# XiaoshuiHuang/GMF

Measured on AMD Instinct MI355X. Metric: correspondences/sec (whole node), higher is better.
Workload: dtype f32 (split-fp16 MFMA operands, fp32 accumulate; the cross products of the attention's two contractions, S = K Q'^T and O = P V, on block-scaled e4m3 operands wherever the device-side score guard allows)

## Files before the change

gmf_amd/_lib.py:

```python
from __future__ import annotations

import collections
import ctypes as C
import os
import threading
from typing import Dict, Optional

_HERE = os.path.dirname(os.path.abspath(__file__))
LIB_PATH = os.path.join(_HERE, "libgmf_hip.so")

_f32p = C.POINTER(C.c_float)
_i32p = C.POINTER(C.c_int)
_vp = C.c_void_p
_ll = C.c_longlong


class EncoderWeights(C.Structure):
    _fields_ = [
        ("num_layers", C.c_int),
        ("f1_ctx_wst", _vp), ("f1_ctx_vec", _vp),
        ("f1_attn_wst", _vp), ("f1_attn_vec", _vp),
        ("f1_ff_wst", _vp), ("f1_ff_vec", _vp),
        ("ctx_wst", _vp), ("ctx_vec", _vp), ("ctx_wst_stride", C.c_int), ("ctx_vec_stride", C.c_int),
        ("attn_wst", _vp), ("attn_vec", _vp), ("attn_wst_stride", C.c_int), ("attn_vec_stride", C.c_int),
        ("ff_wst", _vp), ("ff_vec", _vp), ("ff_wst_stride", C.c_int), ("ff_vec_stride", C.c_int),
        ("front_wst", _vp), ("front_vec", _vp), ("front_wst_stride", C.c_int), ("front_vec_stride", C.c_int),
        ("tail_wst", _vp), ("tail_vec", _vp), ("tail_wst_stride", C.c_int), ("tail_vec_stride", C.c_int),
        ("head_wst", _vp), ("head_vec", _vp),
        ("sigma_d", C.c_float),
        ("front_wst_h2", _vp), ("ctx_wst_h2", _vp), ("attn_wst_h2", _vp), ("ff_wst_h2", _vp),
        ("f1_ctx_wst_h2", _vp), ("f1_attn_wst_h2", _vp), ("f1_ff_wst_h2", _vp),
        ("tail_wst_h2", _vp),
        ("pv_guard", _vp),
    ]


class Tensor(C.Structure):
    _fields_ = [("name", C.c_char_p), ("data", _vp), ("ndim", C.c_int), ("shape", _ll * 4)]


class FusionWeights(C.Structure):
    _fields_ = [("latent_dim", C.c_int), ("d_head", C.c_int), ("pe", C.c_int), ("split_fp16", C.c_int),
                ("max_abs_scaled", C.c_float),
                ("ctx_wst", _vp), ("ctx_vec", _vp), ("attn_wst", _vp), ("attn_vec", _vp), ("ff_wst", _vp), ("ff_vec", _vp),
                ("ctx_wst_h2", _vp), ("attn_wst_h2", _vp), ("ff_wst_h2", _vp)]


GMF_PACK_DEVICE_TENSORS = 1
GMF_PACK_STANDALONE_BLOCK = 2
GMF_PACK_HOST_BLOCK = 4


def tensor_list(sd):
    import torch
    keep, items = [], []
    host = {}
    dev = [(k, v) for k, v in sd.items() if torch.is_tensor(v) and v.is_floating_point() and v.device.type != "cpu" and v.dim() <= 4]
    if dev:
        flat = torch.cat([v.detach().reshape(-1).to(torch.float32) for _, v in dev]).cpu()
        o = 0
        for k, v in dev:
            host[k] = flat[o:o + v.numel()].reshape(v.shape)
            o += v.numel()
    for k, v in sd.items():
        if not (torch.is_tensor(v) and v.is_floating_point()):
            continue
        t = host[k] if k in host else v.detach().to("cpu", torch.float32).contiguous()
        if t.dim() > 4:
            continue
        name = k.encode()
        keep += [t, name]
        e = Tensor()
        e.name, e.data, e.ndim = name, t.data_ptr(), t.dim()
        for d in range(4):
            e.shape[d] = t.shape[d] if d < t.dim() else 1
        items.append(e)
    arr = (Tensor * len(items))(*items)
    return arr, keep


class PoseParams(C.Structure):
    _fields_ = [
        ("num_seeds", C.c_int), ("k", C.c_int), ("num_iterations", C.c_int), ("use_nms", C.c_int),
        ("refine_iters", C.c_int),
        ("sigma", C.c_float), ("sigma_d", C.c_float), ("inlier_threshold", C.c_float),
        ("nms_radius", C.c_float), ("refine_threshold", C.c_float),
    ]


class PoseGraphOptions(C.Structure):
    _fields_ = [("max_iteration", C.c_int), ("max_iteration_lm", C.c_int), ("reference_node", C.c_int),
                ("min_relative_increment", C.c_double), ("min_relative_residual_increment", C.c_double),
                ("min_right_term", C.c_double), ("min_residual", C.c_double),
                ("edge_prune_threshold", C.c_double), ("preference_loop_closure", C.c_double)]


SIGNATURES = {
    "gmf_abi_version": (C.c_int, []),
    "gmf_create": (C.c_int, [C.c_int, C.POINTER(_vp)]),
    "gmf_destroy": (None, [_vp]),
    "gmf_last_error_string": (C.c_char_p, [_vp]),
    "gmf_workspace_bytes": (_ll, [_vp]),
    "gmf_set_workspace": (C.c_int, [_vp, _vp, _ll]),
    "gmf_workspace_wanted": (_ll, [_vp]),
    "gmf_status_read": (C.c_int, [_vp, C.POINTER(C.c_int), C.c_int]),
    "gmf_set_tuning": (C.c_int, [_vp, C.c_char_p, C.c_int]),
    "gmf_get_tuning": (C.c_int, [_vp, C.c_char_p, C.POINTER(C.c_int)]),
    "gmf_set_sigma_device": (C.c_int, [_vp, _vp]),
    "gmf_profile_enable": (C.c_int, [_vp, C.c_int]),
    "gmf_profile_read": (C.c_int, [_vp, C.POINTER(C.c_double), C.POINTER(C.c_int)]),
    "gmf_pack_rows_p32": (C.c_int, [_vp, _vp, _ll, _ll, _ll, C.c_int, C.c_int, C.c_int, _vp, _vp]),
    "gmf_unpack_rows_p32": (C.c_int, [_vp, _vp, C.c_int, C.c_int, C.c_int, _vp, _ll, _ll, _ll, _vp]),
    "gmf_pack_pts8": (C.c_int, [_vp, _vp, _vp, C.c_int, C.c_int, _vp, _vp]),
    "gmf_front_forward": (C.c_int, [_vp, C.c_int, _vp, _vp, _vp, _vp, _vp, _vp, _vp, C.c_int, C.c_int, _vp]),
    "gmf_scattn_forward": (C.c_int, [_vp, _vp, _vp, _vp, _vp, _vp, _vp, _vp, _vp, C.c_int, C.c_int, C.c_float, _vp]),
    "gmf_scattn_forward_dense": (C.c_int, [_vp, _vp, _vp, _vp, _vp, _vp, _vp, _vp, _vp, C.c_int, C.c_int, _vp]),
# ... 294 lines not shown
```

gmf_amd/csrc/encoder_h2.hip:

```cpp
#include <algorithm>
#include <cstdlib>
#include "enc_common.hpp"
#include "enc_ff.hpp"
#include "launchers.hpp"

namespace gmf {

#ifndef GMF_H2_RING
#define GMF_H2_RING 2
#endif
constexpr int kRing = GMF_H2_RING;

template <int MODE>
GMF_DEVINL void front_h2_body(float* lds, const int bx, const int pair, const int zsel_in, const float* __restrict__ in,
                              const float* __restrict__ wst, const float* __restrict__ vecs, float* __restrict__ f_out,
                              float* __restrict__ q_out, float* __restrict__ k_out, float* __restrict__ v_out, int N, int tiles,
                              const PairTab* __restrict__ ptab = nullptr, unsigned* __restrict__ v_scale = nullptr,
                              const PvGuard guard = {}) {
  const int lane = threadIdx.x & 63, h = lane >> 5, i = lane & 31;
  const int wave = __builtin_amdgcn_readfirstlane(threadIdx.x >> 6);
  const size_t row0 = pair_row0(ptab, pair, N);
  N = pair_rows(ptab, pair, N);
  const int tiles_p = ptab ? (N + 31) >> 5 : tiles;
  if (bx * kWavesPerWG >= tiles_p) return;
// ... 512 lines not shown

__global__ void __launch_bounds__(256, 2)
k_small_front_fattn(const float* __restrict__ f_in, const float* __restrict__ front_wst, const float* __restrict__ front_vec,
                    const float* __restrict__ ctx_img, const float* __restrict__ attn_wst, const float* __restrict__ attn_vec,
                    float* __restrict__ q_out, float* __restrict__ k_out, float* __restrict__ v_out, float* __restrict__ x1_out,
                    int N, int tiles, int T, int ttiles, unsigned* __restrict__ v_scale, const PvGuard guard,
                    const PairTab* __restrict__ ptab) {
  __shared__ __attribute__((aligned(16))) float lds[kFattnTileLdsFloats];
  static_assert(kFattnTileLdsFloats >= kFattnLdsFloats, "one buffer serves both forms of the role");
  if (blockIdx.z < 3) {
    front_h2_body<2>(lds, blockIdx.x, blockIdx.y, blockIdx.z, f_in, front_wst, front_vec, nullptr, q_out, k_out, v_out, N, tiles,
                     ptab, v_scale, guard);
    return;
  }
  const int Np = pair_rows(ptab, blockIdx.y, N), tiles_p = ptab ? (Np + 31) >> 5 : tiles;
  if (gridDim.z == 4) {
    if ((int)blockIdx.x * kWavesPerWG >= tiles_p) return;
    fusion_attn_h2_body<true>(lds, blockIdx.x, blockIdx.y, f_in, ctx_img, attn_wst, attn_vec, x1_out, Np, tiles_p, T, ttiles, tiles);
  } else {
    const int tile = (int)blockIdx.x * kWavesPerWG + ((int)blockIdx.z - 3);
    if (tile < tiles_p) fusion_attn_tile_h2_body(lds, tile, blockIdx.y, f_in, ctx_img, attn_wst, attn_vec, x1_out, Np, tiles_p, T, ttiles, tiles);
  }
}

template <bool SPLIT>
__global__ void __launch_bounds__(256, 2)
k_fusion_ff_h2p(const float* __restrict__ x1, const float* __restrict__ wst, const float* __restrict__ vecs,
                float* __restrict__ x2_out, int tiles, float* __restrict__ part) {
  __shared__ __attribute__((aligned(16))) float lds[4 * kStageFloats];
  fusion_ff_h2p_body<SPLIT>(lds, blockIdx.x, blockIdx.y, gridDim.y, blockIdx.z, gridDim.z, x1, wst, vecs, x2_out, tiles, part);
}

__global__ void __launch_bounds__(256, 2)
k_pro_ctx_pts(const int n_a, const int gx_a, const int nb, const float* __restrict__ ctx, const float* __restrict__ wst,
              const float* __restrict__ vecs, float* __restrict__ out, int T, int ttiles,
              const float* __restrict__ src, const float* __restrict__ tgt, float* __restrict__ pts8, int N, int Npad, long total,
              const PairTab* __restrict__ ptab, unsigned* __restrict__ zero_words, int n_zero) {
  __shared__ __attribute__((aligned(16))) float lds[2 * kStageFloats];
  const int id = blockIdx.x;
  if (id < n_a) {
    ctx_prep_h2_body<false, true>(lds, id % gx_a, id / gx_a, 0, nb, ctx, wst, vecs, out, T, ttiles, 0, 0);
    return;
  }
  pack_pts8_body((long)(id - n_a) * 256 + threadIdx.x, src, tgt, pts8, N, Npad, total, ptab, zero_words, n_zero);
}

constexpr int kProBLdsFloats = kFattnLdsFloats > kCompatLdsFloats ? kFattnLdsFloats : kCompatLdsFloats;
__global__ void __launch_bounds__(256, 2)
k_pro_fattn_compat(const int n_a, const int gx_a, const float* __restrict__ xin, const float* __restrict__ ctx_img,
                   const float* __restrict__ wst, const float* __restrict__ vecs, float* __restrict__ x1_out, int T, int ttiles,
                   const float* __restrict__ pts8, float* __restrict__ c_dense, int N, int tiles, int gy, float inv_sig2,
                   const PairTab* __restrict__ ptab) {
  __shared__ __attribute__((aligned(16))) float lds[kProBLdsFloats];
  const int id = blockIdx.x;
  if (id < n_a) {
    fusion_attn_h2_body<false, true>(lds, id % gx_a, id / gx_a, xin, ctx_img, wst, vecs, x1_out, T, ttiles, T, ttiles);
    return;
  }
  const int j = id - n_a, I = j % tiles, rest = j / tiles;
  compat_build_body<0>(lds, I, rest % gy, rest / gy, pts8, c_dense, N, tiles, inv_sig2, ptab);
}

constexpr int kProCLdsFloats = (kRing > 4 ? kRing : 4) * kStageFloats;
template <bool SPLIT, int MINB>
__global__ void __launch_bounds__(256, MINB)
k_pro_ff_front(const int n_a, const int gx_a, const int nb, const int hs, const float* __restrict__ x1, const float* __restrict__ wst,
               const float* __restrict__ vecs, float* __restrict__ x2_out, int ttiles, float* __restrict__ part,
               const int gx_f, const float* __restrict__ in, const float* __restrict__ fwst, const float* __restrict__ fvecs,
               float* __restrict__ f_out, float* __restrict__ q_out, float* __restrict__ k_out, float* __restrict__ v_out, int N,
               int tiles, const PairTab* __restrict__ ptab, const PvGuard guard) {
  __shared__ __attribute__((aligned(16))) float lds[kProCLdsFloats];
  const int id = blockIdx.x;
  if (id < n_a) {
    const int bx = id % gx_a, r = id / gx_a;
    fusion_ff_h2p_body<SPLIT>(lds, bx, r % nb, nb, r / nb, hs, x1, wst, vecs, x2_out, ttiles, part);
    return;
  }
  const int j = id - n_a;
  front_h2_body<3>(lds, j % gx_f, j / gx_f, -1, in, fwst, fvecs, f_out, q_out, k_out, v_out, N, tiles, ptab, nullptr, guard);
}

constexpr int kLinLdsFloats = 4 * kStageFloats + 7 * C + (3 * C + 2 * FFH) + kWavesPerWG * 2 * C + 3 * C;

template <int PART, int NP = 3, bool QSKIP = false>
GMF_DEVINL void linear_h2_body(float* lds, const float* __restrict__ f_in, const float* __restrict__ front_wst,
                               const float* __restrict__ front_vec, const float* __restrict__ ctx_img,
                               const float* __restrict__ attn_wst, const float* __restrict__ attn_vec,
                               const float* __restrict__ ff_wst, const float* __restrict__ ff_vec, float* __restrict__ q_out,
                               float* __restrict__ k_out, float* __restrict__ v_out, float* __restrict__ x2_out, int N, int tiles,
                               int T, int ttiles, const PairTab* __restrict__ ptab = nullptr,
                               unsigned* __restrict__ v_scale = nullptr,
                               const PvGuard guard = {}) {
  const int lane = threadIdx.x & 63, h = lane >> 5, i = lane & 31;
  const int wave = __builtin_amdgcn_readfirstlane(threadIdx.x >> 6);
  const int pair = blockIdx.y;
  if (ptab) N = ptab[pair].n;
  const int tiles_p = ptab ? (N + 31) >> 5 : tiles;
  if ((int)blockIdx.x * kWavesPerWG >= tiles_p) return;
  const int tile_raw = blockIdx.x * kWavesPerWG + wave;
  const bool active = tile_raw < tiles_p;
  const int tile = active ? tile_raw : tiles_p - 1;
  const float* pair_base = f_in + (size_t)pair * tiles * (32 * C);
  const size_t toff = ((size_t)pair * tiles + tile) * (32 * C);

  float* const lvec_a = lds + 4 * kStageFloats;
  float* const lvec_f = lvec_a + 7 * C;
  float* const halo = lvec_f + (3 * C + 2 * FFH) + wave * (2 * C);
  float* const lvec_p = lvec_f + (3 * C + 2 * FFH) + kWavesPerWG * (2 * C);
  if (PART != 2) dma_vec(front_vec + C, lvec_p, 3 * C, wave, kWavesPerWG, lane);
  if (PART != 1) {
    dma_vec(attn_vec, lvec_a, 7 * C, wave, kWavesPerWG, lane);
    dma_vec(ff_vec, lvec_f, 3 * C + 2 * FFH, wave, kWavesPerWG, lane);
    LcpeHalo<CF>::issue(pair_base, tile, tiles_p, halo, lane);
  }
  StageRing<4> ss;
  if (PART == 0) ss.init(lds, wave, lane, front_wst + (QSKIP ? 8 : 4) * kStageFloats, QSKIP ? 8 : 12, attn_wst, 2,
                         ctx_img + (size_t)pair * ttiles * kStageFloats, ttiles, attn_wst + 2 * kStageFloats, 2);
  else if (PART == 1) ss.init(lds, wave, lane, front_wst + 4 * kStageFloats, 12);
  else ss.init(lds, wave, lane, attn_wst, 2, ctx_img + (size_t)pair * ttiles * kStageFloats, ttiles, attn_wst + 2 * kStageFloats, 2);

  float f[CF];
  if (PART != 2) {
    FragH2<8> fx;
    load_frag_p32<CF>(f, f_in + toff, lane);
    fx.set(f);
    ss.prime();
    const bool v8 = pv_planes_on(v_scale, guard, pair);
    unsigned* const sw_tile = v_scale ? v_scale + ((size_t)pair * tiles + tile) * 128 + lane : nullptr;
    unsigned ksw = 0;
#pragma unroll
    for (int which = (QSKIP ? 1 : 0); which < 2; ++which) {
      float* dst = (which == 0 ? q_out : k_out) + toff;
#pragma unroll
      for (int mb = 0; mb < 4; ++mb) {
        constexpr int kYounger[4] = {8, 12, 16, 20};
        const int sidx = 4 * (which - (QSKIP ? 1 : 0)) + mb;
        const f16x8* lw = as_h2(PART == 1 ? ss.acquire()
                                : sidx == 0 ? ss.acquire_counted<kYounger[0]>() : sidx == 1 ? ss.acquire_counted<kYounger[1]>()
                                : sidx == 2 ? ss.acquire_counted<kYounger[2]>() : ss.acquire_counted<kYounger[3]>());
        f32x16 acc = zero16();
        mma_wx_h2n<8, NP>(acc, lw, fx);
        float t[16], bb[16];
        load_vec_block(bb, lvec_p + which * C, mb, h);
#pragma unroll
        for (int r = 0; r < 16; ++r) t[r] = fmaf(acc[r], kH2Inv, bb[r]);
        if (which == 1 && v8) store_block_v8(dst, mb, t, lane, ksw);
        else store_block_h2(dst, mb, t, lane);
      }
    }
    unsigned vsw = 0;
#pragma unroll
    for (int db = 0; db < 4; ++db) {
      const f16x8* lw = as_h2(PART == 1 ? ss.acquire() : ss.acquire_counted<20>());
      f32x16 acc = zero16();
      mma_xw_h2n<8, NP>(acc, lw, fx);
      float t[16];
      const float bvd = lvec_p[2 * C + 32 * db + i];
#pragma unroll
      for (int r = 0; r < 16; ++r) t[r] = fmaf(acc[r], kH2Inv, bvd);
      if (v8) store_block_v8(v_out + toff, db, t, lane, vsw);
      else store_block_h2(v_out + toff, db, t, lane);
    }
    if (v_scale) { sw_tile[0] = vsw; sw_tile[64] = ksw; }
  }

  if (PART == 1) {
    asm volatile("s_waitcnt vmcnt(0)" ::: "memory");
    return;
  }
  if (PART == 2) ss.prime();
  f32x16 x1a[4];
  {
    FragH2<4> qx;
    {
      float xp[CF];
      if (PART == 2) load_frag_p32<CF>(xp, f_in + toff, lane);
      else {
#pragma unroll
        for (int k = 0; k < CF; ++k) xp[k] = f[k];
      }
      if (PART == 2) {
        asm volatile("s_waitcnt vmcnt(0)" ::: "memory");
        __syncthreads();
      }
      LcpeHalo<CF>::apply(xp, halo, lvec_a, tile * 32 + i, N, lane);
      {
        FragH2<8> nx;
        {
          float xn[CF];
          layernorm_frag<CF>(xn, xp, lvec_a + 4 * C, lvec_a + 5 * C, h);
          nx.set(xn);
        }
#pragma unroll
        for (int mb = 0; mb < 2; ++mb) {
          const f16x8* lw = as_h2(ss.acquire());
          f32x16 acc = zero16();
          mma_wx_h2n<8, NP>(acc, lw, nx);
          float t[16];
#pragma unroll
          for (int r = 0; r < 16; ++r) t[r] = acc[r] * kH2Inv;
          qx.set_block(mb, t);
        }
      }
#pragma unroll
      for (int mb = 0; mb < 4; ++mb) {
        float b[16];
        load_vec_block(b, lvec_a + 6 * C, mb, h);
#pragma unroll
        for (int r = 0; r < 16; ++r) x1a[mb][r] = (xp[16 * mb + r] + b[r]) * 256.0f;
      }
    }
    f32x16 oacc[2];
    oacc[0] = zero16(); oacc[1] = zero16();
    float m_run = -INFINITY, l_half = 0.f;
    for (int t = 0; t < ttiles; ++t) {
      const f16x8* lk = as_h2(ss.acquire());
      const f16x8* lv = lk + 2 * 4 * 64;
      f32x16 sc = zero16();
      mma_wx_h2n<4, NP>(sc, lk, qx);
      float x[16];
      float mx = -INFINITY;
      if (t + 1 < ttiles) {
#pragma unroll
        for (int r = 0; r < 16; ++r) { x[r] = sc[r]; mx = fmaxf(mx, sc[r]); }
      } else {
        const int jbase = t * 32 + 4 * h;
#pragma unroll
        for (int r = 0; r < 16; ++r) {
          const int jl = 8 * (r >> 2) + (r & 3);
          x[r] = (jbase + jl < T) ? sc[r] : -INFINITY;
          mx = fmaxf(mx, x[r]);
        }
      }
      mx = xhalf_max(mx);
      const float m_new = fmaxf(m_run, mx);
      const bool moved = m_new > m_run;
      const float alpha = __builtin_amdgcn_exp2f(m_run - m_new);
      m_run = m_new;
      const float m_off = m_new - 10.0f;
      float ls = 0.f;
#pragma unroll
      for (int r = 0; r < 16; ++r) { x[r] = __builtin_amdgcn_exp2f(x[r] - m_off); ls += x[r]; }
      l_half = fmaf(l_half, alpha, ls);
      if (__any(moved)) {
#pragma unroll
        for (int db = 0; db < 2; ++db)
#pragma unroll
          for (int r = 0; r < 16; ++r) oacc[db][r] *= alpha;
      }
#pragma unroll
      for (int s2 = 0; s2 < 2; ++s2) {
        f16x8 ph, pl;
        split8h(&x[8 * s2], ph, pl);
#pragma unroll
        for (int db = 0; db < 2; ++db) {
          const int slot = 2 * db + s2;
          mma_np<NP>(oacc[db], lv[(0 * 4 + slot) * 64], lv[(1 * 4 + slot) * 64], ph, pl);
        }
      }
    }
    FragH2<4> ox;
    {
      const float inv = 1.0f / xhalf_sum(l_half);
#pragma unroll
      for (int db = 0; db < 2; ++db) {
        float t[16];
#pragma unroll
        for (int r = 0; r < 16; ++r) t[r] = oacc[db][r] * inv;
        ox.set_block(db, t);
      }
    }
#pragma unroll
    for (int st = 0; st < 2; ++st) {
      const f16x8* lw = as_h2(ss.acquire());
#pragma unroll
      for (int hb = 0; hb < 2; ++hb) mma_wx_h2n<4, NP>(x1a[2 * st + hb], lw + hb * (2 * 4 * 64), ox);
    }
  }

  FragH2<8> nx;
  f32x16 y[4];
  {
    float x1[CF], xn[CF];
#pragma unroll
    for (int mb = 0; mb < 4; ++mb)
#pragma unroll
      for (int r = 0; r < 16; ++r) x1[16 * mb + r] = x1a[mb][r] * kH2Inv;
    layernorm_frag<CF>(xn, x1, lvec_f, lvec_f + C, h);
    nx.set(xn);
#pragma unroll
    for (int mb = 0; mb < 4; ++mb) {
      float b[16];
      load_vec_block(b, lvec_f + 2 * C + 2 * FFH, mb, h);
#pragma unroll
      for (int r = 0; r < 16; ++r) y[mb][r] = (x1[16 * mb + r] + b[r]) * 256.0f;
    }
  }
  __syncthreads();
  ff_chunks<NP>(nx, y, lds, ff_wst, lvec_f + 2 * C, lvec_f + 2 * C + FFH, wave, lane, h, 0, FFH / 32);
#pragma unroll
  for (int mb = 0; mb < 4; ++mb) {
    float t[16];
#pragma unroll
    for (int r = 0; r < 16; ++r) t[r] = y[mb][r] * kH2Inv;
    if (active) store_block_p32(x2_out + toff, mb, t, lane);
  }
}

template <int NP, bool QSKIP = false>
__global__ void __launch_bounds__(256, 2)
k_linear_h2(const float* __restrict__ f_in, const float* __restrict__ front_wst, const float* __restrict__ front_vec,
            const float* __restrict__ ctx_img, const float* __restrict__ attn_wst, const float* __restrict__ attn_vec,
            const float* __restrict__ ff_wst, const float* __restrict__ ff_vec, float* __restrict__ q_out,
            float* __restrict__ k_out, float* __restrict__ v_out, float* __restrict__ x2_out, int N, int tiles, int T,
            int ttiles, const PairTab* __restrict__ ptab, unsigned* __restrict__ v_scale, const PvGuard guard) {
  __shared__ __attribute__((aligned(16))) float lds[kLinLdsFloats];
  tail_priority(blockIdx.y * gridDim.x + blockIdx.x, gridDim.x * gridDim.y);
  linear_h2_body<0, NP, QSKIP>(lds, f_in, front_wst, front_vec, ctx_img, attn_wst, attn_vec, ff_wst, ff_vec, q_out, k_out, v_out, x2_out, N,
                               tiles, T, ttiles, ptab, v_scale, guard);
}

__global__ void __launch_bounds__(256, 2)
k_linear_roles(const float* __restrict__ f_in, const float* __restrict__ front_wst, const float* __restrict__ front_vec,
               const float* __restrict__ ctx_img, const float* __restrict__ attn_wst, const float* __restrict__ attn_vec,
               const float* __restrict__ ff_wst, const float* __restrict__ ff_vec, float* __restrict__ q_out,
               float* __restrict__ k_out, float* __restrict__ v_out, float* __restrict__ x2_out, int N, int tiles, int T,
               int ttiles, unsigned* __restrict__ v_scale, const PvGuard guard, const PairTab* __restrict__ ptab) {
  __shared__ __attribute__((aligned(16))) float lds[kLinLdsFloats];
  if (blockIdx.z == 0)
    linear_h2_body<1>(lds, f_in, front_wst, front_vec, ctx_img, attn_wst, attn_vec, ff_wst, ff_vec, q_out, k_out, v_out, x2_out, N,
                      tiles, T, ttiles, ptab, v_scale, guard);
  else
    linear_h2_body<2>(lds, f_in, front_wst, front_vec, ctx_img, attn_wst, attn_vec, ff_wst, ff_vec, q_out, k_out, v_out, x2_out, N,
                      tiles, T, ttiles, ptab);
}

__global__ void __launch_bounds__(256)
k_ff_reduce(const float* __restrict__ part, const float* __restrict__ x1, const float* __restrict__ vecs,
            float* __restrict__ x2_out, int tiles, int hs) {
  const int lane = threadIdx.x & 63, h = lane >> 5;
  const int tile = blockIdx.x * kWavesPerWG + (threadIdx.x >> 6);
  if (tile >= tiles) return;
  const int mb = blockIdx.z;
  const size_t n_all = (size_t)gridDim.y * tiles;
  const size_t toff = ((size_t)blockIdx.y * tiles + tile) * (32 * C);
  float b[16], xr[16], p[8][16];
  load_vec_block(b, vecs + 2 * C + 2 * FFH, mb, h);
#pragma unroll
  for (int z = 0; z < 8; ++z)
    if (z < hs) load_block_p32(p[z], part + (size_t)z * n_all * (32 * C) + toff, mb, lane);
  load_block_p32(xr, x1 + toff, mb, lane);
  float t[16];
#pragma unroll
  for (int r = 0; r < 16; ++r) t[r] = p[0][r];
#pragma unroll
  for (int z = 1; z < 8; ++z)
    if (z < hs) {
#pragma unroll
      for (int r = 0; r < 16; ++r) t[r] += p[z][r];
    }
#pragma unroll
  for (int r = 0; r < 16; ++r) t[r] = fmaf(t[r], kH2Inv, b[r]) + xr[r];
  store_block_p32(x2_out + toff, mb, t, lane);
}

static inline dim3 tgrid(int tiles, int B, int sets = 1) { return dim3((tiles + kWavesPerWG - 1) / kWavesPerWG, B, sets); }

hipError_t launch_front_h2(int mode, bool split, const float* in, const float* wst, const float* vecs, float* f, float* q, float* k,
                           float* v, int B, int N, int tiles, hipStream_t s, const PairTab* ptab, unsigned* v_scale, PvGuard guard) {
  dim3 g = tgrid(tiles, B);
  if (split) g.z = 3;
  if (mode == 3) { g.z = 1; hipLaunchKernelGGL(k_front_h2<3>, g, dim3(256), 0, s, in, wst, vecs, f, q, k, v, N, tiles, ptab, v_scale, guard); }
  else if (mode == 1) hipLaunchKernelGGL(k_front_h2<1>, g, dim3(256), 0, s, in, wst, vecs, f, q, k, v, N, tiles, ptab, v_scale, guard);
  else if (mode == 2) hipLaunchKernelGGL(k_front_h2<2>, g, dim3(256), 0, s, in, wst, vecs, f, q, k, v, N, tiles, ptab, v_scale, guard);
  else hipLaunchKernelGGL(k_front_h2<0>, g, dim3(256), 0, s, in, wst, vecs, f, q, k, v, N, tiles, ptab, v_scale, guard);
  return hipGetLastError();
}

hipError_t launch_linear_h2(bool roles, const float* f, const float* front_wst, const float* front_vec, const float* ctx_img,
                            const float* attn_wst, const float* attn_vec, const float* ff_wst, const float* ff_vec, float* q,
                            float* k, float* v, float* x2, int B, int N, int tiles, int T, int ttiles, hipStream_t s,
                            bool one_product, const PairTab* ptab, unsigned* v_scale, PvGuard guard) {
  if (roles)
    hipLaunchKernelGGL(k_linear_roles, tgrid(tiles, B, 2), dim3(256), 0, s, f, front_wst, front_vec, ctx_img, attn_wst, attn_vec,
                       ff_wst, ff_vec, q, k, v, x2, N, tiles, T, ttiles, v_scale, guard, ptab);
  else if (one_product)
    hipLaunchKernelGGL(k_linear_h2<1>, tgrid(tiles, B), dim3(256), 0, s, f, front_wst, front_vec, ctx_img, attn_wst, attn_vec, ff_wst,
                       ff_vec, q, k, v, x2, N, tiles, T, ttiles, ptab, v_scale, guard);
  else if (!q)
    hipLaunchKernelGGL((k_linear_h2<3, true>), tgrid(tiles, B), dim3(256), 0, s, f, front_wst, front_vec, ctx_img, attn_wst, attn_vec, ff_wst,
                       ff_vec, q, k, v, x2, N, tiles, T, ttiles, ptab, v_scale, guard);
  else
    hipLaunchKernelGGL(k_linear_h2<3>, tgrid(tiles, B), dim3(256), 0, s, f, front_wst, front_vec, ctx_img, attn_wst, attn_vec, ff_wst,
                       ff_vec, q, k, v, x2, N, tiles, T, ttiles, ptab, v_scale, guard);
  return hipGetLastError();
}

hipError_t launch_ctx_prep_h2(bool pe, const float* ctx, const float* wst, const float* vecs, float* out, int B, int T,
                              int ttiles, int sets, int wst_stride, int vec_stride, hipStream_t s, bool rowmajor) {
  if (pe) hipLaunchKernelGGL(k_ctx_prep_h2<true>, tgrid(ttiles, B, sets), dim3(256), 0, s, ctx, wst, vecs, out, T, ttiles, wst_stride, vec_stride);
  else if (rowmajor) hipLaunchKernelGGL((k_ctx_prep_h2<false, true>), tgrid(ttiles, B, sets), dim3(256), 0, s, ctx, wst, vecs, out, T, ttiles, wst_stride, vec_stride);
  else hipLaunchKernelGGL(k_ctx_prep_h2<false>, tgrid(ttiles, B, sets), dim3(256), 0, s, ctx, wst, vecs, out, T, ttiles, wst_stride, vec_stride);
  return hipGetLastError();
}

hipError_t launch_fusion_attn_h2(bool pe, const float* x, const float* ctx_img, const float* wst, const float* vecs,
                                 float* x1, int B, int N, int tiles, int T, int ttiles, hipStream_t s, bool rowmajor) {
  if (pe) hipLaunchKernelGGL(k_fusion_attn_h2<true>, tgrid(tiles, B), dim3(256), 0, s, x, ctx_img, wst, vecs, x1, N, tiles, T, ttiles);
  else if (rowmajor) hipLaunchKernelGGL((k_fusion_attn_h2<false, true>), tgrid(tiles, B), dim3(256), 0, s, x, ctx_img, wst, vecs, x1, N, tiles, T, ttiles);
  else hipLaunchKernelGGL(k_fusion_attn_h2<false>, tgrid(tiles, B), dim3(256), 0, s, x, ctx_img, wst, vecs, x1, N, tiles, T, ttiles);
  return hipGetLastError();
}

hipError_t launch_pro_ctx_pts(const float* p_tokens, const float* wst, const float* vecs, float* f1ctx, int B, int T, int ttiles,
                              const float* src, const float* tgt, float* pts8, int N, hipStream_t s, const PairTab* ptab,
                              unsigned* zero_words, int n_zero) {
  const dim3 ga = tgrid(ttiles, B);
  const int Npad = ((N + 31) / 32) * 32;
  const long total = (long)B * Npad;
  const int n_a = (int)(ga.x * ga.y), n_b = (int)((std::max(total, (long)n_zero) + 255) / 256);
  hipLaunchKernelGGL(k_pro_ctx_pts, dim3(n_a + n_b), dim3(256), 0, s, n_a, (int)ga.x, B, p_tokens, wst, vecs, f1ctx, T, ttiles, src, tgt,
                     pts8, N, Npad, total, ptab, zero_words, n_zero);
  return hipGetLastError();
}

hipError_t launch_pro_fattn_compat(const float* q_tokens, const float* f1ctx, const float* wst, const float* vecs, float* x1t, int B,
                                   int T, int ttiles, const float* pts8, float* c_dense, int N, int tiles, float sigma_d,
                                   hipStream_t s, const PairTab* ptab) {
  const dim3 ga = tgrid(ttiles, B);
  const int gy = (tiles + 4 * kJPerWave - 1) / (4 * kJPerWave);
  const int n_a = (int)(ga.x * ga.y);
  const long n_b = (long)tiles * gy * B;
  hipLaunchKernelGGL(k_pro_fattn_compat, dim3((unsigned)(n_a + n_b)), dim3(256), 0, s, n_a, (int)ga.x, q_tokens, f1ctx, wst, vecs, x1t, T,
                     ttiles, pts8, c_dense, N, tiles, gy, 1.0f / (sigma_d * sigma_d), ptab);
  return hipGetLastError();
}

hipError_t launch_pro_ff_front(const float* x1t, const float* wst, const float* vecs, float* imgfeat, int B, int ttiles, float* part,
                               int hs, const float* corr_pos, const float* fwst, const float* fvecs, float* f, float* q, float* k,
                               float* v, int N, int tiles, hipStream_t s, const PairTab* ptab, PvGuard guard) {
  const dim3 ga = tgrid(ttiles, B), gf = tgrid(tiles, B);
  const int n_a = (int)(ga.x * B) * hs, n_b = (int)(gf.x * B);
#define GMF_PRO_C(SPLIT, MINB, HS, PART)                                                                                              \
  hipLaunchKernelGGL((k_pro_ff_front<SPLIT, MINB>), dim3(n_a + n_b), dim3(256), 0, s, n_a, (int)ga.x, B, HS, x1t, wst, vecs, imgfeat, ttiles, \
                     PART, (int)gf.x, corr_pos, fwst, fvecs, f, q, k, v, N, tiles, ptab, guard)
  const bool one_per_cu = n_a + n_b <= 256;
  if (hs > 1) { if (one_per_cu) GMF_PRO_C(true, 1, hs, part); else GMF_PRO_C(true, 2, hs, part); }
  else { if (one_per_cu) GMF_PRO_C(false, 1, 1, (float*)nullptr); else GMF_PRO_C(false, 2, 1, (float*)nullptr); }
#undef GMF_PRO_C
  return hipGetLastError();
}

hipError_t launch_ff_reduce_h2(const float* part, const float* x1, const float* vecs, float* x2, int B, int tiles, int hs, hipStream_t s) {
  const dim3 g = tgrid(tiles, B);
  hipLaunchKernelGGL(k_ff_reduce, dim3(g.x, g.y, 4), dim3(256), 0, s, part, x1, vecs, x2, tiles, hs);
  return hipGetLastError();
}

hipError_t launch_small_front_fattn(const float* f, const float* front_wst, const float* front_vec, const float* ctx_img,
                                    const float* attn_wst, const float* attn_vec, float* q, float* k, float* v, float* x1, int B,
                                    int N, int tiles, int T, int ttiles, hipStream_t s, unsigned* v_scale, PvGuard guard, bool tile_role,
                                    const PairTab* ptab) {
  const bool per_tile = tile_role && ttiles >= 2 && (long)tiles * B <= 256;
  hipLaunchKernelGGL(k_small_front_fattn, tgrid(tiles, B, per_tile ? 7 : 4), dim3(256), 0, s, f, front_wst, front_vec, ctx_img, attn_wst, attn_vec,
                     q, k, v, x1, N, tiles, T, ttiles, v_scale, guard, ptab);
  return hipGetLastError();
}

hipError_t launch_fusion_ff_h2(const float* x1, const float* wst, const float* vecs, float* x2, int B, int tiles, hipStream_t s,
                               float* part, int hs) {
  const dim3 g = tgrid(tiles, B);
  if (hs > 1) {
    hipLaunchKernelGGL(k_fusion_ff_h2p<true>, dim3(g.x, g.y, hs), dim3(256), 0, s, x1, wst, vecs, x2, tiles, part);
    hipLaunchKernelGGL(k_ff_reduce, dim3(g.x, g.y, 4), dim3(256), 0, s, part, x1, vecs, x2, tiles, hs);
  }
  else hipLaunchKernelGGL(k_fusion_ff_h2p<false>, g, dim3(256), 0, s, x1, wst, vecs, x2, tiles, (float*)nullptr);
  return hipGetLastError();
// ... 4 lines not shown
```

gmf_amd/csrc/encoder_kernels.hip:

```cpp
#include <algorithm>
#include <type_traits>
#include "enc_common.hpp"
#include "enc_ff.hpp"

namespace gmf {

template <int MODE>
__global__ void __launch_bounds__(256, 2)
k_front(const float* __restrict__ in, const float* __restrict__ wst, const float* __restrict__ vecs,
        float* __restrict__ f_out, float* __restrict__ q_out, float* __restrict__ k_out,
        float* __restrict__ v_out, int N, int tiles) {
  __shared__ __attribute__((aligned(16))) float lds[2 * kStageFloats];
  const int lane = threadIdx.x & 63, wave = threadIdx.x >> 6, h = lane >> 5, i = lane & 31;
  const int pair = blockIdx.y;
  const int tile_raw = blockIdx.x * kWavesPerWG + wave;
  const bool active = tile_raw < tiles;
  const int tile = active ? tile_raw : tiles - 1;
  const size_t toff = ((size_t)pair * tiles + tile) * (32 * C);

  constexpr bool FIRST = (MODE == 1);
  StageStream ss;
  if (MODE == 2) ss.init(lds, lds + kStageFloats, wave, kWavesPerWG, lane, wst + 4 * kStageFloats, 12);
  else ss.init(lds, lds + kStageFloats, wave, kWavesPerWG, lane, wst, 16);
  ss.prime();
// ... 456 lines not shown

template <bool NEXT_PCN, class Stages, class Fus>
GMF_DEVINL void scattn_epilogue_h2(const float (&o)[CF], const bool active, Stages& ss, const float* __restrict__ vecs,
                                   const Fus& fus_tile, float* __restrict__ out_tile, const int lane, const int h,
                                   const float* __restrict__ next_bias = nullptr,
                                   unsigned* __restrict__ stat_next = nullptr, const int pair = 0, const bool row_valid = false) {
    FragH2<8> ox, featx;
    FragH2<4> m1x, m2x;
    if (active) ox.set(o);
#pragma unroll
    for (int mb = 0; mb < 2; ++mb) {
      const f16x8* lw = as_h2(ss.acquire());
      if (!active) continue;
      f32x16 acc = zero16();
      mma_wx_h2<8>(acc, lw, ox);
      float b[16], t1[16];
      load_vec_block(b, vecs, mb, h);
#pragma unroll
      for (int r = 0; r < 16; ++r) t1[r] = relu_nan(fmaf(acc[r], kH2Inv, b[r]));
      m1x.set_block(mb, t1);
    }
    {
      const f16x8* lw = as_h2(ss.acquire());
#pragma unroll
      for (int mb = 0; mb < 2; ++mb) {
        if (!active) continue;
        f32x16 acc = zero16();
        mma_wx_h2<4>(acc, lw + mb * (2 * 4 * 64), m1x);
        float b[16], t2[16];
        load_vec_block(b, vecs + 64, mb, h);
#pragma unroll
        for (int r = 0; r < 16; ++r) t2[r] = relu_nan(fmaf(acc[r], kH2Inv, b[r]));
        m2x.set_block(mb, t2);
      }
    }
#pragma unroll
    for (int st = 0; st < 2; ++st) {
      const f16x8* lw = as_h2(ss.acquire());
#pragma unroll
      for (int hb = 0; hb < 2; ++hb) {
        if (!active) continue;
        const int mb = 2 * st + hb;
        f32x16 acc = zero16();
        mma_wx_h2<4>(acc, lw + hb * (2 * 4 * 64), m2x);
        float b[16], fz[16], tt[16];
        load_vec_block(b, vecs + 128, mb, h);
        fus_tile.load(fz, mb, lane, h);
#pragma unroll
        for (int r = 0; r < 16; ++r) tt[r] = fmaf(acc[r], kH2Inv, b[r]) + fz[r];
        if (NEXT_PCN) featx.set_block(mb, tt);
        else if (active) store_block_p32(out_tile, mb, tt, lane);
      }
    }
    if (NEXT_PCN) {
      float ssq = 0.f;
#pragma unroll
      for (int mb = 0; mb < 4; ++mb) {
        const f16x8* lw = as_h2(ss.acquire());
        if (!active) continue;
        f32x16 acc = zero16();
        mma_wx_h2<8>(acc, lw, featx);
        float b[16], tt[16];
        load_vec_block(b, next_bias, mb, h);
#pragma unroll
        for (int r = 0; r < 16; ++r) { tt[r] = relu_nan(fmaf(acc[r], kH2Inv, b[r])); ssq = fmaf(tt[r], tt[r], ssq); }
        store_block_p32(out_tile, mb, tt, lane);
      }
      if (stat_next && active) pv_stat_raise(stat_next, pair, ssq, row_valid, lane);
    }
}

struct AttnItem { int item, ks; bool split, valid; };
GMF_DEVINL AttnItem attn_item(int L, int n_items, int n_full, int ksplits) {
  const int chunk = n_items >> 3, rem = n_items & 7, xcd = L & 7, kth = L >> 3;
  const int start = (xcd < rem) ? xcd * (chunk + 1) : rem * (chunk + 1) + (xcd - rem) * chunk;
  const int items = chunk + (xcd < rem ? 1 : 0);
  const int nf = min(n_full, items);
  if (kth < nf) return AttnItem{start + kth, 0, false, true};
  const int j = kth - nf, r = j / ksplits;
  return AttnItem{start + nf + r, j - r * ksplits, true, nf + r < items};
}

constexpr float kInvU16 = 1.0f / 65535.0f;
template <int NPROD = 3, int CFMT = 0, int WAVES = 4, bool PVF8 = false>
GMF_DEVINL void scattn_h2p_body(float* lds, const int bid, const float* __restrict__ q_img, const float* __restrict__ k_img,
                                const float* __restrict__ v_img, const float* __restrict__ fus, const float* __restrict__ wst,
                                const float* __restrict__ vecs, float* out, int N, int tiles, int wgs_per_pair,
                                const float* __restrict__ c_dense, int n_items, int n_full, int ksplits,
                                float* __restrict__ part_o, float* __restrict__ part_ml, const float* __restrict__ next_wst,
                                const float* __restrict__ next_bias, const PairTab* __restrict__ ptab = nullptr,
                                const unsigned* __restrict__ v_scale = nullptr,
                                const float* qf_img = nullptr, const float* __restrict__ qw_wst = nullptr,
                                const float* __restrict__ qw_bias = nullptr,
                                unsigned* __restrict__ stat_next = nullptr) {
  static_assert(!PVF8 || NPROD == 3, "the fp8 cross products belong to the three-product form");
  float* const ldsK = lds;
  float* const ldsV = lds + 2 * kStageFloats;
  const int lane = threadIdx.x & 63, h = lane >> 5;
  const int wave = __builtin_amdgcn_readfirstlane(threadIdx.x >> 6);
  const unsigned lane_off16 = lane * 16;
  const AttnItem it = attn_item(bid, n_items, n_full, ksplits);
  if (!it.valid) return;
  const bool split = it.split;
  const int ks = it.ks;
  const int slot = it.item / wgs_per_pair, qblock = it.item - slot * wgs_per_pair;
  const int pair = ptab ? ptab[slot].ord : slot;
  if (ptab) N = ptab[pair].n;
  const int tiles_p = ptab ? (N + 31) >> 5 : tiles;
  if (qblock * WAVES >= tiles_p) return;
  const int t_begin = split ? (tiles_p * ks) / ksplits : 0;
  const int t_end = split ? (tiles_p * (ks + 1)) / ksplits : tiles_p;
  const int tile_raw = qblock * WAVES + wave;
  const bool active = tile_raw < tiles_p;
  const int tile = active ? tile_raw : tiles_p - 1;
  const size_t pbase = (size_t)pair * tiles;
  const size_t toff = (pbase + tile) * (32 * C);

  f16x8 qh[8], ql[8];
  if (NPROD == 3 && WAVES == 4 && qf_img) {
    FragH2<8> fx;
    {
      float fq[CF];
      load_frag_p32<CF>(fq, qf_img + toff, lane);
      fx.set(fq);
    }
#pragma unroll
    for (int st = 0; st < 4; ++st) dma_4k_s(qw_wst + st * kStageFloats + wave * 1024, lds + st * kStageFloats + wave * 1024, lane_off16);
    asm volatile("s_waitcnt vmcnt(0)" ::: "memory");
    __syncthreads();
#pragma unroll
    for (int mb = 0; mb < 4; ++mb) {
      const f16x8* lw = reinterpret_cast<const f16x8*>(lds + mb * kStageFloats) + lane;
      f32x16 acc = zero16();
      mma_wx_h2n<8, 3>(acc, lw, fx);
      float t[16], bq[16];
      load_vec_block(bq, qw_bias, mb, h);
#pragma unroll
      for (int r = 0; r < 16; ++r) t[r] = fmaf(acc[r], kH2Inv, bq[r]);
      split8h(&t[0], qh[2 * mb], ql[2 * mb]);
      split8h(&t[8], qh[2 * mb + 1], ql[2 * mb + 1]);
    }
    __syncthreads();
  } else {
    const f16x8* qp = reinterpret_cast<const f16x8*>(q_img + (pbase + tile) * (size_t)kStageFloats) + lane;
#pragma unroll
    for (int s = 0; s < 8; ++s) {
      qh[s] = qp[(0 * 8 + s) * 64];
      if (NPROD == 3) ql[s] = qp[(1 * 8 + s) * 64];
    }
  }
  i32x8 qb[4];
  unsigned qsw = 0;
  if (PVF8) {
#pragma unroll
    for (int cb = 0; cb < 4; ++cb) q_planes8(qh[2 * cb], ql[2 * cb], qh[2 * cb + 1], ql[2 * cb + 1], cb, lane, qb[cb], qsw);
  }
  constexpr int kCTile16 = CFMT ? 128 : 256;
  const f32x4* const crow = reinterpret_cast<const f32x4*>(c_dense) + ((pbase + tile) * (size_t)tiles) * kCTile16 + lane;
  float c[16];
  unsigned cw[8];
  const unsigned* const vsrow = PVF8 ? v_scale + pbase * 128 + lane : nullptr;
  unsigned vsw_next = 0, vsw = 0, ksw_next = 0, ksw = 0;
  const int psc = (lane & 32) ? 117 : 129;
  auto fetch_c = [&](int t) {
    const f32x4* ct = crow + (size_t)t * kCTile16;
    if (PVF8) {
      vsw_next = __builtin_nontemporal_load(vsrow + (size_t)t * 128);
      ksw_next = __builtin_nontemporal_load(vsrow + (size_t)min(t + 1, tiles_p - 1) * 128 + 64);
    }
    if (CFMT == 1) {
#pragma unroll
      for (int q2 = 0; q2 < 2; ++q2) {
        const f16x8 hv = __builtin_bit_cast(f16x8, __builtin_nontemporal_load(ct + q2 * 64));
#pragma unroll
        for (int e = 0; e < 8; ++e) c[8 * q2 + e] = (float)hv[e];
      }
    } else if (CFMT >= 2) {
#pragma unroll
      for (int q2 = 0; q2 < 2; ++q2) {
        const f32x4 v = __builtin_nontemporal_load(ct + q2 * 64);
#pragma unroll
        for (int e = 0; e < 4; ++e) cw[4 * q2 + e] = __float_as_uint(v[e]);
      }
    } else {
#pragma unroll
      for (int q = 0; q < 4; ++q) {
        const f32x4 v = __builtin_nontemporal_load(ct + q * 64);
        c[4 * q + 0] = v[0]; c[4 * q + 1] = v[1]; c[4 * q + 2] = v[2]; c[4 * q + 3] = v[3];
      }
    }
  };
  auto score = [&](int r, float sv) -> float {
    if (CFMT == 2) return (float)((r & 1) ? (cw[r >> 1] >> 16) : (cw[r >> 1] & 0xffffu)) * sv;
    return c[r] * sv;
  };
  auto expo = [&](float xv, float m_off) -> float {
    return __builtin_amdgcn_exp2f(CFMT == 2 ? fmaf(xv, kInvU16, -m_off) : xv - m_off);
  };
  auto mma_n = [&](f32x16& acc, f16x8 ah, f16x8 al, f16x8 bh, f16x8 bl) {
    if (NPROD == 3) mma3(acc, ah, al, bh, bl);
    else acc = mfma_h16(ah, bh, acc);
  };
  auto to_planes2 = [&](float x0, float x1, f16x8& hi, f16x8& lo, int j) {
    if (NPROD == 3) split2h(x0, x1, hi, lo, j);
    else { const f32x2 xx = {x0, x1}; const f16x2 hh = __builtin_convertvector(xx, f16x2); hi[j] = hh[0]; hi[j + 1] = hh[1]; }
  };
  auto planes_f8 = [&](const f16x8& hi, const f16x8& lo, const int j, const int kp, i32x8& pb, float& ls_h, float& ls_l) {
    const f16x2 hh = {hi[j], hi[j + 1]}, ll = {lo[j], lo[j + 1]};
    const f16x2 ones = {(_Float16)1.0f, (_Float16)1.0f};
    const int w = kp >> 1;
    if (kp & 1) {
      pb[w] = cvt2_fp8_f16<true>(pb[w], hh, 4.0f);
      pb[4 + w] = cvt2_fp8_f16<true>(pb[4 + w], ll, 0x1p-10f);
      ls_l = __builtin_amdgcn_fdot2(dec2_fp8_f16<true>(pb[4 + w], 0x1p-10f), ones, ls_l, false);
    } else {
      int d0, d1;
      asm("" : "=v"(d0), "=v"(d1));
      pb[w] = cvt2_fp8_f16<false>(d0, hh, 4.0f);
      pb[4 + w] = cvt2_fp8_f16<false>(d1, ll, 0x1p-10f);
      ls_l = __builtin_amdgcn_fdot2(dec2_fp8_f16<false>(pb[4 + w], 0x1p-10f), ones, ls_l, false);
    }
    ls_h = __builtin_amdgcn_fdot2(hh, ones, ls_h, false);
    asm volatile("" : "+v"(ls_h), "+v"(ls_l));
  };
  const float* gk = k_img + pbase * (size_t)kStageFloats;
  const float* gv = v_img + pbase * (size_t)kStageFloats;
  constexpr int kPiecesPerWave = ((NPROD == 3) ? 16 : 8) / WAVES;
  auto issue16k = [&](const float* g, float* l) {
#pragma unroll
    for (int q = 0; q < kPiecesPerWave; ++q) dma_piece_1k_s(g + (wave + WAVES * q) * 256, l + (wave + WAVES * q) * 256, lane_off16);
  };
  auto issueK = [&](int t) { issue16k(gk + (size_t)t * kStageFloats, ldsK + (t & 1) * kStageFloats); };
  auto issueV = [&](int t) { issue16k(gv + (size_t)t * kStageFloats, ldsV + (t & 1) * kStageFloats); };

  f32x16 oacc[4];
#pragma unroll
  for (int db = 0; db < 4; ++db) oacc[db] = zero16();
  float m_run = -INFINITY, l_half = 0.f;

  issueK(t_begin);
  if (t_begin + 1 < t_end) issueK(t_begin + 1);
  issueV(t_begin);
  fetch_c(t_begin);
  asm volatile("s_waitcnt vmcnt(0)" ::: "memory");
  __syncthreads();
  f32x16 s_a = zero16(), s_b;
  auto s_cross8 = [&](f32x16 acc, const f16x8* lkt, const int cb, const unsigned kscale) -> f32x16 {
    const i32x4* l8 = reinterpret_cast<const i32x4*>(lkt);
    const i32x4 a_lo = l8[(1 * 8 + 2 * cb) * 64], a_hi = l8[(1 * 8 + 2 * cb + 1) * 64];
    const i32x8 ka = {a_lo[0], a_lo[1], a_lo[2], a_lo[3], a_hi[0], a_hi[1], a_hi[2], a_hi[3]};
    return mfma_f8s2(ka, qb[cb], acc, cb, (int)kscale, (int)qsw);
  };
  if (active) {
    const f16x8* lk = reinterpret_cast<const f16x8*>(ldsK + (t_begin & 1) * kStageFloats) + lane;
    if (PVF8) {
      const unsigned ks0 = vsrow[(size_t)t_begin * 128 + 64];
#pragma unroll
      for (int s = 0; s < 8; ++s) s_a = mfma_h16(lk[(0 * 8 + s) * 64], qh[s], s_a);
#pragma unroll
      for (int cb = 0; cb < 4; ++cb) s_a = s_cross8(s_a, lk, cb, ks0);
    } else {
#pragma unroll
      for (int s = 0; s < 8; ++s) mma_n(s_a, lk[(0 * 8 + s) * 64], lk[(1 * 8 + s) * 64], qh[s], ql[s]);
    }
  }

  auto tile_top = [&](const int t, const f32x16& s_cur, float (&x)[16], float& mx) {
    asm volatile("s_waitcnt vmcnt(0)" ::: "memory");
    __syncthreads();
    if (PVF8) vsw = vsw_next;
#pragma unroll
    for (int r = 0; r < 16; r += 2) {
      x[r] = score(r, s_cur[r]);
      x[r + 1] = score(r + 1, s_cur[r + 1]);
      mx = __builtin_fmaxf(mx, __builtin_fmaxf(x[r], x[r + 1]));
    }
    __builtin_amdgcn_sched_barrier(0);
    if (t + 1 < t_end) fetch_c(t + 1);
    __builtin_amdgcn_sched_barrier(0);
  };
  auto issue_piece = [&](const int t, const int q) {
    if ((q & 3) >= kPiecesPerWave) return;
    if (q < 4) {
      if (t + 2 < t_end) dma_piece_1k_s(gk + (size_t)(t + 2) * kStageFloats + (wave + WAVES * q) * 256,
                                        ldsK + (t & 1) * kStageFloats + (wave + WAVES * q) * 256, lane_off16);
    } else {
      dma_piece_1k_s(gv + (size_t)(t + 1) * kStageFloats + (wave + WAVES * (q - 4)) * 256,
                     ldsV + ((t + 1) & 1) * kStageFloats + (wave + WAVES * (q - 4)) * 256, lane_off16);
    }
  };
  auto issue_k4 = [&](const int t) {
    if (WAVES == 4 && t + 2 < t_end && (NPROD == 3 || wave < 2))
      dma_4k_s(gk + (size_t)(t + 2) * kStageFloats + wave * 1024, ldsK + (t & 1) * kStageFloats + wave * 1024, lane_off16);
  };
  auto issue_v4 = [&](const int t) {
    if (WAVES == 4 && (NPROD == 3 || wave < 2))
      dma_4k_s(gv + (size_t)(t + 1) * kStageFloats + wave * 1024, ldsV + ((t + 1) & 1) * kStageFloats + wave * 1024, lane_off16);
  };
  auto rescale = [&](const bool moved, const float alpha) {
    if (__any(moved)) {
#pragma unroll
      for (int db = 0; db < 4; ++db)
#pragma unroll
        for (int r = 0; r < 16; ++r) oacc[db][r] *= alpha;
    }
  };
  auto tile_step = [&](const int t, const f32x16& s_cur, f32x16& s_next) {
    float x[16];
    float mx = -INFINITY, m_off = 0.f, alpha = 1.f, ls = 0.f;
    tile_top(t, s_cur, x, mx);
    const f16x8* lv = reinterpret_cast<const f16x8*>(ldsV + (t & 1) * kStageFloats) + lane;
    const f16x8* lk = reinterpret_cast<const f16x8*>(ldsK + ((t + 1) & 1) * kStageFloats) + lane;
    bool moved = false;
    f16x8 ph0, pl0, ph1, pl1;
    {
      mx = xhalf_max_swap(mx);
      if (CFMT == 2) mx *= kInvU16;
      const float m_new = __builtin_fmaxf(m_run, mx);
      moved = m_new > m_run;
      alpha = __builtin_amdgcn_exp2f(m_run - m_new);
      m_run = m_new;
      m_off = m_new - 10.0f;
      rescale(moved, alpha);
    }
    s_next = zero16();
    {
      f16x8 kh = lk[0], kl = kh;
      if (NPROD == 3) kl = lk[8 * 64];
      f16x8 kh_n = kh, kl_n = kl;
#pragma unroll
      for (int u = 0; u < 24; ++u) {
        const int s = u / 3, pr = u % 3;
        if (pr == 0 && s < 7) { kh_n = lk[(0 * 8 + s + 1) * 64]; if (NPROD == 3) kl_n = lk[(1 * 8 + s + 1) * 64]; }
        if (NPROD == 3 || pr == 2) s_next = mma3_part(pr, s_next, kh, kl, qh[s], ql[s]);
        if (pr == 2) { kh = kh_n; kl = kl_n; }
        if (u < 2) {
        } else if (u <= 11) {
          const int r = u - 2;
          x[r] = expo(x[r], m_off);
          ls += x[r];
        } else if (u <= 15) {
          const int j = 2 * (u - 12);
          to_planes2(x[j], x[j + 1], ph0, pl0, j);
        } else if (u <= 21) {
          const int r = u - 6;
          x[r] = expo(x[r], m_off);
          ls += x[r];
        } else {
          const int j = 2 * (u - 22);
          to_planes2(x[8 + j], x[8 + j + 1], ph1, pl1, j);
        }
        __builtin_amdgcn_sched_barrier(0);
      }
    }
    {
      f16x8 vh = lv[0], vl = vh;
      if (NPROD == 3) vl = lv[8 * 64];
      f16x8 vh_n = vh, vl_n = vl;
#pragma unroll
      for (int u = 0; u < 24; ++u) {
        const int s2 = u / 12, db = (u % 12) / 3, pr = u % 3;
        if (pr == 0 && u < 21) {
          const int un = u + 3, slot = 2 * ((un % 12) / 3) + un / 12;
          vh_n = lv[(0 * 8 + slot) * 64]; if (NPROD == 3) vl_n = lv[(1 * 8 + slot) * 64];
        }
        if (NPROD == 3 || pr == 2) oacc[db] = mma3_part(pr, oacc[db], vh, vl, s2 ? ph1 : ph0, s2 ? pl1 : pl0);
        if (pr == 2) { vh = vh_n; vl = vl_n; }
        if (u < 2) {
          const int j = 4 + 2 * u;
          to_planes2(x[8 + j], x[8 + j + 1], ph1, pl1, j);
        }
        if (u >= 3 && u < 11) issue_piece(t, u - 3);
        __builtin_amdgcn_sched_barrier(0);
      }
    }
    l_half = fmaf(l_half, alpha, ls);
  };
  constexpr float kLazy = 5.0f;
  auto tile_step_f8 = [&](const int t, const f32x16& s_cur, f32x16& s_next) {
    float x[16];
    float mx = -INFINITY, m_off = 0.f, alpha = 1.f, ls = 0.f, ls_l = 0.f;
    asm volatile("s_waitcnt vmcnt(0)" ::: "memory");
    __syncthreads();
    vsw = vsw_next;
    ksw = ksw_next;
    const f16x8* lv = reinterpret_cast<const f16x8*>(ldsV + (t & 1) * kStageFloats) + lane;
    const f16x8* lk = reinterpret_cast<const f16x8*>(ldsK + ((t + 1) & 1) * kStageFloats) + lane;
    f16x8 ph0, pl0, ph1, pl1;
    i32x8 pb;
    f16x8 vr[3];
    auto hslot = [](int u) { return (0 * 8 + 2 * (u & 3) + (u >> 2)) * 64; };
    s_next = zero16();
    {
      const i32x4* lk8 = reinterpret_cast<const i32x4*>(lk);
      f16x8 kh = lk[0];
      f16x8 kh_n = kh;
      i32x4 k8a = lk8[(1 * 8) * 64], k8b = lk8[(1 * 8 + 1) * 64];
#pragma unroll
      for (int u = 0; u < 24; ++u) {
        const int s = u / 3, pr = u % 3;
        if (pr == 0 && s < 7) kh_n = lk[(0 * 8 + s + 1) * 64];
        if (pr == 2) s_next = mfma_h16(kh, qh[s], s_next);
        if (pr == 0 && (s & 1)) {
          const int cb = s >> 1;
          const i32x8 ka = {k8a[0], k8a[1], k8a[2], k8a[3], k8b[0], k8b[1], k8b[2], k8b[3]};
          s_next = mfma_f8s2(ka, qb[cb], s_next, cb, (int)ksw, (int)qsw);
          if (cb < 3) { k8a = lk8[(1 * 8 + 2 * cb + 2) * 64]; k8b = lk8[(1 * 8 + 2 * cb + 3) * 64]; }
        }
        if (pr == 2) kh = kh_n;
        if (u < 4) {
#pragma unroll
          for (int r = 4 * u; r < 4 * u + 4; r += 2) {
            x[r] = score(r, s_cur[r]);
            x[r + 1] = score(r + 1, s_cur[r + 1]);
            mx = __builtin_fmaxf(mx, __builtin_fmaxf(x[r], x[r + 1]));
          }
        }
        if (u == 3) {
          __builtin_amdgcn_sched_barrier(0);
          if (t + 1 < t_end) fetch_c(t + 1);
          __builtin_amdgcn_sched_barrier(0);
          mx = xhalf_max_swap(mx);
          if (CFMT == 2) mx *= kInvU16;
          const bool moved = mx > m_run + kLazy;
          const float m_new = moved ? mx : m_run;
          alpha = __builtin_amdgcn_exp2f(m_run - m_new);
          m_run = m_new;
          m_off = m_new - (10.0f - kLazy);
          rescale(moved, alpha);
        }
        if (u >= 4 && u < 20) x[u - 4] = expo(x[u - 4], m_off);
        if (u >= 6 && u <= 18 && (u & 1) == 0) {
          const int k = (u - 6) >> 1;
          if (k < 4) split2h(x[2 * k], x[2 * k + 1], ph0, pl0, 2 * k);
          else split2h(x[2 * k], x[2 * k + 1], ph1, pl1, 2 * k - 8);
        }
        if (u == 20) split2h(x[14], x[15], ph1, pl1, 6);
        if (u == 16) issue_k4(t);
        if (u == 23) issue_v4(t);
        if (u >= 21) vr[u - 21] = lv[hslot(u - 21)];
        __builtin_amdgcn_sched_barrier(0);
      }
    }
    {
      const i32x4* lv8 = reinterpret_cast<const i32x4*>(lv);
      i32x4 fa[2][2];
#pragma unroll
      for (int u = 0; u < 12; ++u) {
        if (u < 8) {
          const int s2 = u >> 2, db = u & 3;
          oacc[db] = mfma_h16(vr[u % 3], s2 ? ph1 : ph0, oacc[db]);
          if (u + 3 < 8) vr[u % 3] = lv[hslot(u + 3)];
          if (u == 4 || u == 6) { const int fd = (u - 4) >> 1; fa[fd][0] = lv8[(1 * 8 + 2 * fd) * 64]; fa[fd][1] = lv8[(1 * 8 + 2 * fd + 1) * 64]; }
          planes_f8(u < 4 ? ph0 : ph1, u < 4 ? pl0 : pl1, 2 * (u & 3), u, pb, ls, ls_l);
        } else {
          const int db = u - 8;
          const i32x4 a_lo = fa[db & 1][0], a_hi = fa[db & 1][1];
          const i32x8 va = {a_lo[0], a_lo[1], a_lo[2], a_lo[3], a_hi[0], a_hi[1], a_hi[2], a_hi[3]};
          oacc[db] = mfma_f8s(va, pb, oacc[db], db, (int)vsw, psc);
          if (db < 2) { fa[db & 1][0] = lv8[(1 * 8 + 2 * db + 4) * 64]; fa[db & 1][1] = lv8[(1 * 8 + 2 * db + 5) * 64]; }
        }
        __builtin_amdgcn_sched_barrier(0);
      }
    }
    l_half = fmaf(l_half, alpha, ls + ls_l);
  };
  auto tile_last = [&](const int t, const f32x16& s_cur) {
    float x[16];
    float mx = -INFINITY, ls = 0.f;
    tile_top(t, s_cur, x, mx);
    const f16x8* lv = reinterpret_cast<const f16x8*>(ldsV + (t & 1) * kStageFloats) + lane;
    const int jbase = t * 32 + 4 * h;
    mx = -INFINITY;
#pragma unroll
    for (int r = 0; r < 16; ++r) {
// ... 39 lines not shown
#pragma unroll
      for (int db = 0; db < 4; ++db) {
        const int slot = 2 * db + s2;
        mma_n(oacc[db], lv[(0 * 8 + slot) * 64], lv[(1 * 8 + slot) * 64], ph, pl);
      }
    }
    }
    l_half = fmaf(l_half, alpha, ls);
  };
  if (!active) {
    for (int t = t_begin; t < t_end; ++t) {
      asm volatile("s_waitcnt vmcnt(0)" ::: "memory");
      __syncthreads();
      if (t + 1 < t_end) {
        if (PVF8) { issue_k4(t); issue_v4(t); }
        else {
#pragma unroll
          for (int q = 0; q < 8; ++q) issue_piece(t, q);
        }
      }
    }
  } else {
    int t = t_begin;
    if (PVF8) {
      for (; t + 2 < t_end; t += 2) {
        tile_step_f8(t, s_a, s_b);
        tile_step_f8(t + 1, s_b, s_a);
      }
      if (t + 1 < t_end) { tile_step_f8(t, s_a, s_b); tile_last(t + 1, s_b); }
      else tile_last(t, s_a);
    } else {
    for (; t + 2 < t_end; t += 2) {
      tile_step(t, s_a, s_b);
      tile_step(t + 1, s_b, s_a);
    }
    if (t + 1 < t_end) { tile_step(t, s_a, s_b); tile_last(t + 1, s_b); }
    else tile_last(t, s_a);
    }
  }
  if (split) {
    if (active) {
      float of[CF];
#pragma unroll
      for (int db = 0; db < 4; ++db)
#pragma unroll
        for (int r = 0; r < 16; ++r) of[16 * db + r] = oacc[db][r];
      const size_t n_tiles_all = (size_t)(n_items / wgs_per_pair) * tiles;
      const size_t pt = (size_t)ks * n_tiles_all + pbase + tile;
      store_frag_p32<CF>(part_o + pt * (32 * C), of, lane);
      const float lsum = xhalf_sum(l_half);
      if (h == 0) { part_ml[(pt * 32 + (lane & 31)) * 2] = m_run; part_ml[(pt * 32 + (lane & 31)) * 2 + 1] = lsum; }
    }
    return;
  }

  float o[CF];
  {
    const float inv = 1.0f / xhalf_sum(l_half);
#pragma unroll
    for (int db = 0; db < 4; ++db)
#pragma unroll
      for (int r = 0; r < 16; ++r) o[16 * db + r] = oacc[db][r] * inv;
  }
  __syncthreads();
  float* const lvec = lds + 2 * kStageFloats;
  stage_tail_vecs(lvec, vecs, next_wst ? next_bias : nullptr, wave, lane);
  StageStream ss;
  ss.init(lds, lds + kStageFloats, wave, WAVES, lane, wst, 5, next_wst, next_wst ? 4 : 0);
  ss.prime();
  const FusTile ft{fus + toff};
  if (next_wst) scattn_epilogue_h2<true>(o, active, ss, lvec, ft, out + toff, lane, h, lvec + 2 * C, stat_next, pair,
                                         tile_raw * 32 + (lane & 31) < N);
  else scattn_epilogue_h2<false>(o, active, ss, lvec, ft, out + toff, lane, h);
}

GMF_DEVINL bool attn_pv_on(const unsigned* __restrict__ v_scale, const PvGuard& guard, int bid, int n_items, int n_full, int ksplits,
                           int wgs_per_pair, const PairTab* __restrict__ ptab = nullptr) {
  if (!guard.stat) return v_scale != nullptr;
  const AttnItem it = attn_item(bid, n_items, n_full, ksplits);
  const int slot = it.valid ? it.item / wgs_per_pair : 0;
  return pv_planes_on(v_scale, guard, ptab ? ptab[slot].ord : slot);
}

template <int NPROD, int CFMT, bool PVF8 = false>
__global__ void __launch_bounds__(256, 2)
k_scattn_h2p(const float* __restrict__ q_img, const float* __restrict__ k_img, const float* __restrict__ v_img,
             const float* __restrict__ fus, const float* __restrict__ wst, const float* __restrict__ vecs,
             float* out, int N, int tiles, int wgs_per_pair, const float* __restrict__ c_dense,
             int n_items, int n_full, int ksplits, float* __restrict__ part_o, float* __restrict__ part_ml,
             const float* __restrict__ next_wst, const float* __restrict__ next_bias, const PairTab* __restrict__ ptab,
             const unsigned* __restrict__ v_scale, const float* qf_img, const float* __restrict__ qw_wst,
             const float* __restrict__ qw_bias, const PvGuard guard) {
  __shared__ __attribute__((aligned(16))) float lds[4 * kStageFloats];
  tail_priority(blockIdx.x, gridDim.x);
  if (!PVF8 || attn_pv_on(v_scale, guard, blockIdx.x, n_items, n_full, ksplits, wgs_per_pair, ptab))
    scattn_h2p_body<NPROD, CFMT, 4, PVF8>(lds, blockIdx.x, q_img, k_img, v_img, fus, wst, vecs, out, N, tiles, wgs_per_pair, c_dense, n_items,
                                          n_full, ksplits, part_o, part_ml, next_wst, next_bias, ptab, v_scale, qf_img, qw_wst, qw_bias,
                                          guard.stat_next);
  else
    scattn_h2p_body<NPROD, CFMT, 4, false>(lds, blockIdx.x, q_img, k_img, v_img, fus, wst, vecs, out, N, tiles, wgs_per_pair, c_dense, n_items,
                                           n_full, ksplits, part_o, part_ml, next_wst, next_bias, ptab, nullptr, qf_img, qw_wst, qw_bias,
                                           guard.stat_next);
}

__global__ void __launch_bounds__(256, 2)
k_scattn_fast(const float* __restrict__ q_img, const float* __restrict__ k_img, const float* __restrict__ v_img,
              const float* __restrict__ fus, const float* __restrict__ wst, const float* __restrict__ vecs,
              float* __restrict__ out, int N, int tiles, int wgs_per_pair, const float* __restrict__ c_half, int n_items,
              const float* __restrict__ next_wst, const float* __restrict__ next_bias) {
  constexpr int WAVES = 4;
  constexpr int kHiFloats = kStageFloats / 2;
  constexpr int kCFloats = 512;
  __shared__ __attribute__((aligned(16))) float lds[6 * kHiFloats + WAVES * 3 * kCFloats];
  float* const ldsK = lds;
  float* const ldsV = lds + 3 * kHiFloats;
  const int lane = threadIdx.x & 63, h = lane >> 5;
  const int wave = __builtin_amdgcn_readfirstlane(threadIdx.x >> 6);
  float* const ldsC = lds + 6 * kHiFloats + wave * 3 * kCFloats;
  const unsigned lane_off16 = lane * 16;
  const AttnItem it = attn_item(blockIdx.x, n_items, 0x7fffffff, 1);
  if (!it.valid) return;
  const int pair = it.item / wgs_per_pair, qblock = it.item - pair * wgs_per_pair;
  const int tile_raw = qblock * WAVES + wave;
  const bool active = tile_raw < tiles;
  const int tile = active ? tile_raw : tiles - 1;
  const size_t pbase = (size_t)pair * tiles;
  const size_t toff = (pbase + tile) * (32 * C);

  f16x8 qh[8];
  {
    const f16x8* qp = reinterpret_cast<const f16x8*>(q_img + (pbase + tile) * (size_t)kStageFloats) + lane;
#pragma unroll
    for (int s = 0; s < 8; ++s) qh[s] = qp[s * 64];
  }
  const float* gc = c_half + ((pbase + tile) * (size_t)tiles) * kCFloats;
  const float* gk = k_img + pbase * (size_t)kStageFloats;
  const float* gv = v_img + pbase * (size_t)kStageFloats;
  auto issue_tile = [&](int t, const int slot) {
    t = min(t, tiles - 1);
#pragma unroll
    for (int q = 0; q < 2; ++q)
      dma_piece_1k_s(gk + (size_t)t * kStageFloats + (wave + WAVES * q) * 256, ldsK + slot * kHiFloats + (wave + WAVES * q) * 256, lane_off16);
#pragma unroll
    for (int q = 0; q < 2; ++q)
      dma_piece_1k_s(gv + (size_t)t * kStageFloats + (wave + WAVES * q) * 256, ldsV + slot * kHiFloats + (wave + WAVES * q) * 256, lane_off16);
#pragma unroll
    for (int q = 0; q < 2; ++q)
      dma_piece_1k_s(gc + (size_t)t * kCFloats + q * 256, ldsC + slot * kCFloats + q * 256, lane_off16);
  };
  auto cfma = [&](const float cdw, const float sv, const float neg_m_off, const bool hi) {
    const f16x2 hv = __builtin_bit_cast(f16x2, cdw);
    return __builtin_fmaf((float)(hi ? hv[1] : hv[0]), sv, neg_m_off);
  };

  f32x16 oacc[4];
#pragma unroll
  for (int db = 0; db < 4; ++db) oacc[db] = zero16();
  float l_half = 0.f;

  constexpr float kSlack = 15.0f;
  float m_off = 0.f;
  auto tile_step = [&](auto last_tag, auto first_tag, const int t, const int slot) {
    constexpr bool LAST = decltype(last_tag)::value;
    constexpr bool FIRST = decltype(first_tag)::value;
    asm volatile("s_waitcnt vmcnt(6)" ::: "memory");
    __syncthreads();
    issue_tile(t + 2, slot == 0 ? 2 : slot - 1);
    if (!active) return;
    const f16x8* lk = reinterpret_cast<const f16x8*>(ldsK + slot * kHiFloats) + lane;
    const f16x8* lv = reinterpret_cast<const f16x8*>(ldsV + slot * kHiFloats) + lane;
    const f32x4* lc = reinterpret_cast<const f32x4*>(ldsC + slot * kCFloats) + lane;
    const f32x4 c0a = lc[0], c0b = lc[64];
    f32x16 sc = zero16();
#pragma unroll
    for (int s = 0; s < 8; ++s) sc = mfma_h16(lk[s * 64], qh[s], sc);
    float x[16];
    const float nm = FIRST ? 0.f : -m_off;
    const int jbase = t * 32 + 4 * h;
#pragma unroll
    for (int r = 0; r < 16; ++r) {
      const float cdw = (r < 8) ? c0a[r >> 1] : c0b[(r - 8) >> 1];
      x[r] = cfma(cdw, sc[r], nm, (r & 1) != 0);
      if (LAST) {
        const int jl = 8 * (r >> 2) + (r & 3);
        x[r] = (jbase + jl < N) ? x[r] : -INFINITY;
// ... 777 lines not shown

__global__ void k_pack_pts8(const float* __restrict__ src, const float* __restrict__ tgt, float* __restrict__ dst,
                            int N, int Npad, long total, const PairTab* __restrict__ ptab, unsigned* __restrict__ zero_words,
                            int n_zero) {
  pack_pts8_body((long)blockIdx.x * blockDim.x + threadIdx.x, src, tgt, dst, N, Npad, total, ptab, zero_words, n_zero);
}

}


#include "launchers.hpp"

namespace gmf {

static inline dim3 tile_grid(int tiles, int B, int sets = 1) { return dim3((tiles + kWavesPerWG - 1) / kWavesPerWG, B, sets); }

hipError_t launch_front(int mode, const float* in, const float* wst, const float* vecs, float* f, float* q, float* k,
                        float* v, int B, int N, int tiles, hipStream_t s) {
  const dim3 g = tile_grid(tiles, B);
  if (mode == 1) hipLaunchKernelGGL(k_front<1>, g, dim3(256), 0, s, in, wst, vecs, f, q, k, v, N, tiles);
  else if (mode == 2) hipLaunchKernelGGL(k_front<2>, g, dim3(256), 0, s, in, wst, vecs, f, q, k, v, N, tiles);
  else hipLaunchKernelGGL(k_front<0>, g, dim3(256), 0, s, in, wst, vecs, f, q, k, v, N, tiles);
  return hipGetLastError();
}

hipError_t launch_compat_build(const float* pts8, float* c_dense, int B, int N, int tiles, float sigma_d, int fmt, hipStream_t s,
                               const PairTab* ptab) {
  const dim3 grid(tiles, (tiles + 4 * kJPerWave - 1) / (4 * kJPerWave), B);
  const float inv = 1.0f / (sigma_d * sigma_d);
  if (fmt == 1) hipLaunchKernelGGL(k_compat_build<1>, grid, dim3(256), 0, s, pts8, c_dense, N, tiles, inv, ptab);
  else if (fmt == 2) hipLaunchKernelGGL(k_compat_build<2>, grid, dim3(256), 0, s, pts8, c_dense, N, tiles, inv, ptab);
  else hipLaunchKernelGGL(k_compat_build<0>, grid, dim3(256), 0, s, pts8, c_dense, N, tiles, inv, ptab);
  return hipGetLastError();
}

hipError_t launch_scattn_fp32(const float* q, const float* k, const float* v, const float* pts8, const float* fus,
                              const float* wst, const float* vecs, float* out, int B, int N, int tiles, float sigma_d,
                              hipStream_t s) {
  hipLaunchKernelGGL(k_scattn<false>, tile_grid(tiles, B), dim3(256), 0, s, q, k, v, pts8, fus, wst, vecs, out, N, tiles,
                     1.0f / (sigma_d * sigma_d));
  return hipGetLastError();
}

hipError_t launch_small_attn_ff_merge(const float* q, const float* k, const float* v, const float* x1, const float* ff_wst,
                                      const float* ff_vecs, float* ff_part, int ff_hs, const float* tail_vecs, float* out, int B,
                                      int N, int tiles, int ksplits, hipStream_t s, const CompatCache* cc, bool tile_merge) {
  const int wpp = (tiles + 3) / 4, W = wpp * B;
  const int per_xcd = (W >> 3) + ((W & 7) ? 1 : 0);
  const int n_attn = 8 * per_xcd * ksplits, n_ff = W * ff_hs;
  if (cc->fmt == 2 && cc->v_scale)
    hipLaunchKernelGGL((k_small_attn_ff<2, true>), dim3(n_attn + n_ff), dim3(256), 0, s, n_attn, q, k, v, cc->tail_wst_h2, tail_vecs, N, tiles, wpp,
                       cc->dense, W, ksplits, cc->part_o, cc->part_ml, x1, ff_wst, ff_vecs, ff_part, B, ff_hs, cc->v_scale, cc->guard, cc->ptab);
  else if (cc->fmt == 2)
    hipLaunchKernelGGL(k_small_attn_ff<2>, dim3(n_attn + n_ff), dim3(256), 0, s, n_attn, q, k, v, cc->tail_wst_h2, tail_vecs, N, tiles, wpp,
                       cc->dense, W, ksplits, cc->part_o, cc->part_ml, x1, ff_wst, ff_vecs, ff_part, B, ff_hs, (const unsigned*)nullptr, PvGuard{}, cc->ptab);
  else if (cc->v_scale)
    hipLaunchKernelGGL((k_small_attn_ff<0, true>), dim3(n_attn + n_ff), dim3(256), 0, s, n_attn, q, k, v, cc->tail_wst_h2, tail_vecs, N, tiles, wpp,
                       cc->dense, W, ksplits, cc->part_o, cc->part_ml, x1, ff_wst, ff_vecs, ff_part, B, ff_hs, cc->v_scale, cc->guard, cc->ptab);
  else
    hipLaunchKernelGGL(k_small_attn_ff<0>, dim3(n_attn + n_ff), dim3(256), 0, s, n_attn, q, k, v, cc->tail_wst_h2, tail_vecs, N, tiles, wpp,
                       cc->dense, W, ksplits, cc->part_o, cc->part_ml, x1, ff_wst, ff_vecs, ff_part, B, ff_hs, (const unsigned*)nullptr, PvGuard{}, cc->ptab);
  if (tile_merge)
    hipLaunchKernelGGL(k_scattn_merge_tile, dim3(tiles, B), dim3(256), 0, s, cc->part_o, cc->part_ml, cc->tail_wst_h2, tail_vecs, out,
                       tiles, ksplits, cc->next_wst_h2, cc->next_bias, (const float*)ff_part, ff_hs, x1, ff_vecs + 2 * C + 2 * FFH,
                       cc->guard.stat_next, N, cc->ptab);
  else
    hipLaunchKernelGGL(k_scattn_merge, dim3(8 * per_xcd), dim3(256), 0, s, cc->part_o, cc->part_ml, x1, cc->tail_wst_h2, tail_vecs, out,
                       tiles, wpp, W, 0, ksplits, cc->next_wst_h2, cc->next_bias, (const float*)ff_part, ff_hs, x1,
                       ff_vecs + 2 * C + 2 * FFH, cc->guard.stat_next, N, cc->ptab);
  return hipGetLastError();
}

hipError_t launch_scattn_h2p(const float* q, const float* k, const float* v, const float* fus, const float* vecs, float* out, int B,
                             int N, int tiles, hipStream_t s, const CompatCache& cc, int n_full, int ksplits) {
  const int wpp = (tiles + 3) / 4, W = wpp * B;
  const int per_xcd = (W >> 3) + ((W & 7) ? 1 : 0);
  const int max_tail = std::max(0, per_xcd - n_full);
  const dim3 grid(8 * (std::min(n_full, per_xcd) + max_tail * ksplits));
  if (cc.half && max_tail == 0)
    hipLaunchKernelGGL(k_scattn_fast, dim3(8 * per_xcd), dim3(256), 0, s, q, k, v, fus, cc.tail_wst_h2, vecs, out, N, tiles, wpp, cc.dense, W,
                       cc.next_wst_h2, cc.next_bias);
  else if (cc.half)
    hipLaunchKernelGGL((k_scattn_h2p<1, 1>), grid, dim3(256), 0, s, q, k, v, fus, cc.tail_wst_h2, vecs, out, N, tiles, wpp, cc.dense, W,
                       n_full, ksplits, cc.part_o, cc.part_ml, cc.next_wst_h2, cc.next_bias, cc.ptab, (const unsigned*)nullptr, (const float*)nullptr, (const float*)nullptr, (const float*)nullptr, PvGuard{});
  else if (cc.fmt == 2 && cc.v_scale)
    hipLaunchKernelGGL((k_scattn_h2p<3, 2, true>), grid, dim3(256), 0, s, q, k, v, fus, cc.tail_wst_h2, vecs, out, N, tiles, wpp, cc.dense,
                       W, n_full, ksplits, cc.part_o, cc.part_ml, cc.next_wst_h2, cc.next_bias, cc.ptab, cc.v_scale, cc.qf_img, cc.qw_wst, cc.qw_bias, cc.guard);
  else if (cc.fmt == 2)
    hipLaunchKernelGGL((k_scattn_h2p<3, 2>), grid, dim3(256), 0, s, q, k, v, fus, cc.tail_wst_h2, vecs, out, N, tiles, wpp, cc.dense,
                       W, n_full, ksplits, cc.part_o, cc.part_ml, cc.next_wst_h2, cc.next_bias, cc.ptab, (const unsigned*)nullptr, cc.qf_img, cc.qw_wst, cc.qw_bias, PvGuard{});
  else if (cc.v_scale)
    hipLaunchKernelGGL((k_scattn_h2p<3, 0, true>), grid, dim3(256), 0, s, q, k, v, fus, cc.tail_wst_h2, vecs, out, N, tiles, wpp, cc.dense,
                       W, n_full, ksplits, cc.part_o, cc.part_ml, cc.next_wst_h2, cc.next_bias, cc.ptab, cc.v_scale, cc.qf_img, cc.qw_wst, cc.qw_bias, cc.guard);
  else
    hipLaunchKernelGGL((k_scattn_h2p<3, 0>), grid, dim3(256), 0, s, q, k, v, fus, cc.tail_wst_h2, vecs, out, N, tiles, wpp, cc.dense,
                       W, n_full, ksplits, cc.part_o, cc.part_ml, cc.next_wst_h2, cc.next_bias, cc.ptab, (const unsigned*)nullptr, cc.qf_img, cc.qw_wst, cc.qw_bias, PvGuard{});
  if (max_tail > 0)
    hipLaunchKernelGGL(k_scattn_merge, dim3(8 * max_tail), dim3(256), 0, s, cc.part_o, cc.part_ml, fus, cc.tail_wst_h2, vecs, out,
                       tiles, wpp, W, n_full, ksplits, cc.next_wst_h2, cc.next_bias, (const float*)nullptr, 0,
                       (const float*)nullptr, (const float*)nullptr, cc.guard.stat_next, N, cc.ptab);
  return hipGetLastError();
}

hipError_t launch_scattn_h2(const float* q, const float* k, const float* v, const float* pts8, const float* fus, const float* wst,
                            const float* vecs, float* out, int B, int N, int tiles, float sigma_d, hipStream_t s, const float* c_dense) {
  const float inv = 1.0f / (sigma_d * sigma_d);
  const int wpp = (tiles + 3) / 4;
  if (c_dense) hipLaunchKernelGGL(k_scattn_h2<true>, dim3(wpp * B), dim3(256), 0, s, q, k, v, pts8, fus, wst, vecs, out, N, tiles, inv, wpp, c_dense);
  else hipLaunchKernelGGL(k_scattn_h2<false>, dim3(wpp * B), dim3(256), 0, s, q, k, v, pts8, fus, wst, vecs, out, N, tiles, inv, wpp, c_dense);
  return hipGetLastError();
}

hipError_t launch_scattn_dense(const float* q, const float* k, const float* v, const float* compat, const float* fus,
                               const float* wst, const float* vecs, float* out, int B, int N, int tiles, hipStream_t s) {
  hipLaunchKernelGGL(k_scattn<true>, tile_grid(tiles, B), dim3(256), 0, s, q, k, v, compat, fus, wst, vecs, out, N, tiles, 0.f);
  return hipGetLastError();
}

hipError_t launch_ctx_prep(bool pe, const float* ctx, const float* wst, const float* vecs, float* out, int B, int T,
                           int ttiles, int sets, int wst_stride, int vec_stride, hipStream_t s) {
  if (pe) hipLaunchKernelGGL(k_ctx_prep<true>, tile_grid(ttiles, B, sets), dim3(256), 0, s, ctx, wst, vecs, out, T, ttiles, wst_stride, vec_stride);
  else hipLaunchKernelGGL(k_ctx_prep<false>, tile_grid(ttiles, B, sets), dim3(256), 0, s, ctx, wst, vecs, out, T, ttiles, wst_stride, vec_stride);
  return hipGetLastError();
}

hipError_t launch_fusion_attn(bool pe, const float* x, const float* ctx_img, const float* wst, const float* vecs,
                              float* x1, int B, int N, int tiles, int T, int ttiles, hipStream_t s) {
  if (pe) hipLaunchKernelGGL(k_fusion_attn<true>, tile_grid(tiles, B), dim3(256), 0, s, x, ctx_img, wst, vecs, x1, N, tiles, T, ttiles);
  else hipLaunchKernelGGL(k_fusion_attn<false>, tile_grid(tiles, B), dim3(256), 0, s, x, ctx_img, wst, vecs, x1, N, tiles, T, ttiles);
  return hipGetLastError();
}

hipError_t launch_fusion_ff(const float* x1, const float* wst, const float* vecs, float* x2, int B, int tiles, hipStream_t s) {
  hipLaunchKernelGGL(k_fusion_ff, tile_grid(tiles, B), dim3(256), 0, s, x1, wst, vecs, x2, tiles);
  return hipGetLastError();
}

hipError_t launch_head(const float* feat_img, const float* wst, const float* vecs, float* logits, float* feat_n,
                       float* feat_rm, int B, int N, int tiles, hipStream_t s, int* status, const PairTab* ptab, const unsigned* pv_stat,
                       const float* pv_thr2, int n_layers) {
  hipLaunchKernelGGL(k_head, tile_grid(tiles, B), dim3(256), 0, s, feat_img, wst, vecs, logits, feat_n, feat_rm, N, tiles, status, ptab,
                     pv_stat, pv_thr2, n_layers);
  return hipGetLastError();
}

hipError_t launch_seed_dist(const float* featn_img, const int* seeds, float* dist, int B, int N, int S, hipStream_t s, const PairTab* ptab) {
  const int tiles = (N + 31) / 32;
  const int sblocks = (S + 127) / 128;
  int chunks = 1;
  while (chunks < 16 && sblocks * B * chunks < 1024 && tiles / (2 * chunks) >= 4) chunks *= 2;
  hipLaunchKernelGGL(k_seed_dist, dim3(sblocks, B * chunks), dim3(256), 0, s, featn_img, seeds, dist, N, tiles, S, chunks, ptab);
  return hipGetLastError();
}

hipError_t launch_pack_p32(const float* src, float* dst, int B, int n_rows, int K, long sb, long sr, long sk, hipStream_t s, const PairTab* ptab) {
  const int tiles = (n_rows + 31) / 32;
  const long total4 = (long)B * tiles * (K / 8) * 64;
  hipLaunchKernelGGL(k_pack_p32, dim3((unsigned)((total4 + 255) / 256)), dim3(256), 0, s, src, dst, n_rows, tiles, K, sb, sr, sk, total4, ptab);
  return hipGetLastError();
}

hipError_t launch_pack_rows_h2(const float* src, float* dst, int B, int n_rows, hipStream_t s, const PairTab* ptab, const float* copy_src,
                               float* copy_dst, long n_copy) {
  const int tiles = (n_rows + 31) / 32;
  const long total = (long)B * tiles * 8 * 64;
  if (!copy_src || !copy_dst) n_copy = 0;
  if (n_copy > total) return hipErrorInvalidValue;
  hipLaunchKernelGGL(k_pack_rows_h2, dim3((unsigned)((total + 255) / 256)), dim3(256), 0, s, src, dst, n_rows, tiles, total, ptab, copy_src,
                     copy_dst, n_copy);
  return hipGetLastError();
}

hipError_t launch_unpack_p32(const float* src, float* dst, int B, int n_rows, int K, long sb, long sr, long sk, hipStream_t s, int* status) {
  const int tiles = (n_rows + 31) / 32;
  const long total4 = (long)B * tiles * (K / 8) * 64;
  hipLaunchKernelGGL(k_unpack_p32, dim3((unsigned)((total4 + 255) / 256)), dim3(256), 0, s, src, dst, n_rows, tiles, K, sb, sr, sk, total4, status);
  return hipGetLastError();
}

// ... 11 lines not shown
```

gmf_amd/csrc/gmf_api.cpp:

```cpp
#include "../../include/gmf_hip.h"

#include <hip/hip_runtime.h>

#include <cmath>
#include <cstdint>
#include <cstdio>
#include <algorithm>
#include <cstring>
#include <new>
#include <string>
#include <utility>
#include <vector>

#include "api_common.hpp"
#include "launchers_pose.hpp"
#include "launchers_solvers.hpp"
#include "launchers_spectral.hpp"
#include "launchers_pointcloud.hpp"
#include "launchers_sparse.hpp"
#include "launchers_dgr_input.hpp"
#include "launchers_correspondence.hpp"
#include "launchers_posegraph.hpp"
#include "launchers_clique.hpp"
#include "launchers_tsdf.hpp"
// ... 190 lines not shown
    return GMF_OK;
  }
  if (std::strcmp(name, "ff_hidden_splits") == 0) {
    GMF_REQUIRE(value == 0 || value == 1 || value == 2 || value == 4 || value == 8, GMF_ERR_BAD_ARG,
                "set_tuning: ff_hidden_splits must be 0, 1, 2, 4 or 8");
    t.ff_split = value;
    return GMF_OK;
  }
  if (std::strcmp(name, "attn_key_splits") == 0) {
    GMF_REQUIRE(value >= 0 && value <= 8, GMF_ERR_BAD_ARG, "set_tuning: attn_key_splits out of range (0..8)");
    t.key_splits = value;
    return GMF_OK;
  }
  if (std::strcmp(name, "attn_tail_split") == 0) {
    GMF_REQUIRE(value == 0 || value == 1, GMF_ERR_BAD_ARG, "set_tuning: attn_tail_split must be 0 or 1");
    t.tail_split = value != 0;
    return GMF_OK;
  }
  if (std::strcmp(name, "small_grid_roles") == 0) {
    GMF_REQUIRE(value == 0 || value == 1, GMF_ERR_BAD_ARG, "set_tuning: small_grid_roles must be 0 or 1");
    t.small_roles = value != 0;
    return GMF_OK;
  }
  if (std::strcmp(name, "fused_linear") == 0) {
    GMF_REQUIRE(value == 0 || value == 1, GMF_ERR_BAD_ARG, "set_tuning: fused_linear must be 0 or 1");
    t.fused_linear = value != 0;
    return GMF_OK;
  }
  if (std::strcmp(name, "compat_cache") == 0) {
    GMF_REQUIRE(value == 0 || value == 1, GMF_ERR_BAD_ARG, "set_tuning: compat_cache must be 0 or 1");
    t.use_cache = value != 0;
    return GMF_OK;
  }
  if (std::strcmp(name, "conv_lds_patch") == 0) {
    GMF_REQUIRE(value >= 0 && value <= 2, GMF_ERR_BAD_ARG, "set_tuning: conv_lds_patch must be 0, 1 or 2");
    t.conv_patch = value;
    return GMF_OK;
  }
  if (std::strcmp(name, "small_fattn_tile") == 0) {
    GMF_REQUIRE(value == 0 || value == 1, GMF_ERR_BAD_ARG, "set_tuning: small_fattn_tile must be 0 or 1");
    t.small_fattn_tile = value != 0;
    return GMF_OK;
  }
  if (std::strcmp(name, "small_prologue_roles") == 0) {
    GMF_REQUIRE(value == 0 || value == 1, GMF_ERR_BAD_ARG, "set_tuning: small_prologue_roles must be 0 or 1");
    t.small_prologue = value != 0;
    return GMF_OK;
  }
  if (std::strcmp(name, "conv_small_grid") == 0) {
    GMF_REQUIRE(value == 0 || value == 1, GMF_ERR_BAD_ARG, "set_tuning: conv_small_grid must be 0 or 1");
    t.conv_small = value != 0;
    return GMF_OK;
  }
  if (std::strcmp(name, "nms_binned") == 0) {
    GMF_REQUIRE(value >= 0 && value <= 2, GMF_ERR_BAD_ARG, "set_tuning: nms_binned must be 0, 1 or 2");
    t.nms_binned = value;
    return GMF_OK;
  }
  if (std::strcmp(name, "topk_select") == 0) {
    GMF_REQUIRE(value == 0 || value == 1, GMF_ERR_BAD_ARG, "set_tuning: topk_select must be 0 or 1");
    t.topk_select = value != 0;
    return GMF_OK;
  }
  if (std::strcmp(name, "wide_attn_tile") == 0) {
    GMF_REQUIRE(value == 0 || value == 1, GMF_ERR_BAD_ARG, "set_tuning: wide_attn_tile must be 0 or 1");
    t.wide_attn_tile = value != 0;
    return GMF_OK;
  }
  if (std::strcmp(name, "small_merge_tile") == 0) {
    GMF_REQUIRE(value == 0 || value == 1, GMF_ERR_BAD_ARG, "set_tuning: small_merge_tile must be 0 or 1");
    t.small_merge_tile = value != 0;
    return GMF_OK;
  }
  if (std::strcmp(name, "mid_grid_roles") == 0) {
    GMF_REQUIRE(value >= 0 && value <= 4096, GMF_ERR_BAD_ARG, "set_tuning: mid_grid_roles out of range (0..4096)");
    t.mid_grid_roles = value;
    return GMF_OK;
  }
  if (std::strcmp(name, "q_in_attention") == 0) {
    GMF_REQUIRE(value == 0 || value == 1, GMF_ERR_BAD_ARG, "set_tuning: q_in_attention must be 0 or 1");
    t.q_in_attention = value != 0;
    return GMF_OK;
  }
  if (std::strcmp(name, "pv_fp8") == 0) {
    GMF_REQUIRE(value >= 0 && value <= 2, GMF_ERR_BAD_ARG, "set_tuning: pv_fp8 must be 0 (three f16 products), 1 (guarded, default) or 2 (always)");
    t.pv_fp8 = value;
    return GMF_OK;
  }
  if (std::strcmp(name, "compat_format") == 0) {
    GMF_REQUIRE(value == 0 || value == 2, GMF_ERR_BAD_ARG, "set_tuning: compat_format must be 0 (fp32) or 2 (16-bit fixed point of c)");
    t.compat_format = value;
    return GMF_OK;
  }
  if (std::strcmp(name, "precision") == 0) {
    GMF_REQUIRE(value >= 0 && value <= 2, GMF_ERR_BAD_ARG, "set_tuning: precision must be 0 (parity), 1 or 2 (throughput numerics)");
    t.precision = value;
    return GMF_OK;
  }
  if (std::strcmp(name, "spectral_col_splits") == 0) {
    GMF_REQUIRE(value >= 0 && value <= gmf::kSmMaxSplits, GMF_ERR_BAD_ARG, "set_tuning: spectral_col_splits out of range (0..32)");
    t.spectral_col_splits = value;
    return GMF_OK;
  }
  if (std::strcmp(name, "clique_local_rows") == 0) {
    GMF_REQUIRE(value >= 0 && value <= gmf::kPmcLocal, GMF_ERR_BAD_ARG, "set_tuning: clique_local_rows out of range (0..384)");
    t.clique_local_rows = value;
    return GMF_OK;
  }
  return fail(h, GMF_ERR_BAD_ARG, std::string("gmf: set_tuning: unknown knob ") + name);
}

int gmf_get_tuning(gmf_handle* h, const char* name, int* value) {
  GMF_REQUIRE(h && name && value, GMF_ERR_BAD_ARG, "get_tuning: null pointer");
  std::lock_guard<std::mutex> lock(h->mu);
  const gmf::Tuning& t = h->tune;
  const struct { const char* name; int v; } tab[] = {
      {"scattn_variant", t.scattn_variant}, {"front_output_split", t.front_split ? 1 : 0}, {"ff_hidden_splits", t.ff_split},
      {"attn_key_splits", t.key_splits}, {"attn_tail_split", t.tail_split ? 1 : 0}, {"small_grid_roles", t.small_roles ? 1 : 0},
      {"fused_linear", t.fused_linear ? 1 : 0}, {"compat_cache", t.use_cache ? 1 : 0}, {"conv_lds_patch", t.conv_patch}, {"conv_small_grid", t.conv_small ? 1 : 0}, {"small_prologue_roles", t.small_prologue ? 1 : 0}, {"small_fattn_tile", t.small_fattn_tile ? 1 : 0},
      {"nms_binned", t.nms_binned}, {"topk_select", t.topk_select ? 1 : 0}, {"wide_attn_tile", t.wide_attn_tile ? 1 : 0},
      {"small_merge_tile", t.small_merge_tile ? 1 : 0}, {"mid_grid_roles", t.mid_grid_roles}, {"pv_fp8", t.pv_fp8}, {"q_in_attention", t.q_in_attention ? 1 : 0},
      {"compat_format", t.compat_format}, {"precision", t.precision}, {"spectral_col_splits", t.spectral_col_splits},
      {"clique_local_rows", t.clique_local_rows}};
  for (const auto& e : tab) {
    if (std::strcmp(name, e.name) == 0) { *value = e.v; return GMF_OK; }
  }
  return fail(h, GMF_ERR_BAD_ARG, std::string("gmf: get_tuning: unknown knob ") + name);
}

int gmf_profile_enable(gmf_handle* h, int on) {
  GMF_REQUIRE(h, GMF_ERR_BAD_ARG, "profile_enable: null handle");
  h->profile = (on != 0);
  h->prof_used = 0;
  return GMF_OK;
}

int gmf_profile_read(gmf_handle* h, double* scattn_ms_total, int* scattn_launches) {
  GMF_REQUIRE(h && scattn_ms_total && scattn_launches, GMF_ERR_BAD_ARG, "profile_read: null pointer");
  SetDevice sd(h);
  double total = 0.0;
  for (size_t i = 0; i < h->prof_used; ++i) {
    GMF_HIP(hipEventSynchronize(h->prof_events[i].second));
    float ms = 0.f;
    GMF_HIP(hipEventElapsedTime(&ms, h->prof_events[i].first, h->prof_events[i].second));
    total += ms;
  }
  *scattn_ms_total = total;
  *scattn_launches = (int)h->prof_used;
  h->prof_used = 0;
  return GMF_OK;
}

void gmf_destroy(gmf_handle* h) {
  if (!h) return;
  for (auto& e : h->prof_events) { (void)hipEventDestroy(e.first); (void)hipEventDestroy(e.second); }
  int prev = -1;
  (void)hipGetDevice(&prev);
  (void)hipSetDevice(h->device);
  if (h->arena && !h->arena_external) (void)hipFree(h->arena);
  if (h->xs_event) (void)hipEventDestroy(h->xs_event);
  for (auto& sl : h->ptab_ring) {
    if (sl.ev) (void)hipEventDestroy(sl.ev);
    if (sl.host) (void)hipHostFree(sl.host);
  }
  for (void* p : h->graph_tables) (void)hipHostFree(p);
  if (h->status_host) (void)hipHostFree(h->status_host);
  if (prev >= 0 && prev != h->device) (void)hipSetDevice(prev);
  delete h;
}

const char* gmf_last_error_string(gmf_handle* h) { return h ? h->err.c_str() : "gmf: null handle"; }

long long gmf_workspace_bytes(gmf_handle* h) { return h ? (long long)h->arena_bytes : 0; }

int gmf_pack_rows_p32(gmf_handle* h, const float* src, long long sb, long long sr, long long sk, int B, int n_rows,
                      int K, float* dst, gmf_stream_t stream) {
  GMF_REQUIRE(h && src && dst, GMF_ERR_BAD_ARG, "pack_rows_p32: null pointer");
  GMF_REQUIRE(B > 0 && n_rows > 0 && K > 0 && K % 8 == 0, GMF_ERR_UNSUPPORTED_SHAPE, "pack_rows_p32: K must be a positive multiple of 8");
  SetDevice sd(h, stream);
  GMF_HIP(gmf::launch_pack_p32(src, dst, B, n_rows, K, sb, sr, sk, S(stream)));
  return GMF_OK;
}

int gmf_unpack_rows_p32(gmf_handle* h, const float* src_img, int B, int n_rows, int K, float* dst, long long sb,
                        long long sr, long long sk, gmf_stream_t stream) {
  GMF_REQUIRE(h && src_img && dst, GMF_ERR_BAD_ARG, "unpack_rows_p32: null pointer");
  GMF_REQUIRE(B > 0 && n_rows > 0 && K > 0 && K % 8 == 0, GMF_ERR_UNSUPPORTED_SHAPE, "unpack_rows_p32: K must be a positive multiple of 8");
  SetDevice sd(h, stream);
  GMF_HIP(gmf::launch_unpack_p32(src_img, dst, B, n_rows, K, sb, sr, sk, S(stream)));
  return GMF_OK;
}

int gmf_pack_pts8(gmf_handle* h, const float* src, const float* tgt, int B, int N, float* dst, gmf_stream_t stream) {
  GMF_REQUIRE(h && src && tgt && dst, GMF_ERR_BAD_ARG, "pack_pts8: null pointer");
  GMF_REQUIRE(B > 0 && N > 0, GMF_ERR_UNSUPPORTED_SHAPE, "pack_pts8: empty input");
  SetDevice sd(h, stream);
  GMF_HIP(gmf::launch_pack_pts8(src, tgt, dst, B, N, S(stream)));
  return GMF_OK;
}

int gmf_front_forward(gmf_handle* h, int first, const float* in, const float* wst, const float* vecs, float* f,
                      float* q, float* k, float* v, int B, int N, gmf_stream_t stream) {
  GMF_REQUIRE(h && in && wst && vecs && f && q && k && v, GMF_ERR_BAD_ARG, "front_forward: null pointer");
  GMF_REQUIRE(B > 0 && N > 0, GMF_ERR_UNSUPPORTED_SHAPE, "front_forward: empty input");
  SetDevice sd(h, stream);
// ... 52 lines not shown
int gmf_classifier_forward(gmf_handle* h, const float* feat_img, const float* wst, const float* vecs, float* logits,
                           float* feat_n, float* feat, int B, int N, gmf_stream_t stream) {
  GMF_REQUIRE(h && feat_img && wst && vecs && logits && feat_n, GMF_ERR_BAD_ARG, "classifier_forward: null pointer");
  GMF_REQUIRE(B > 0 && N > 0, GMF_ERR_UNSUPPORTED_SHAPE, "classifier_forward: empty input");
  SetDevice sd(h, stream);
  GMF_HIP(gmf::launch_head(feat_img, wst, vecs, logits, feat_n, feat, B, N, tiles_of(N), S(stream), h->status_dev));
  return GMF_OK;
}

static int check_weights(gmf_handle* h, const gmf_encoder_weights* w) {
  GMF_REQUIRE(w, GMF_ERR_BAD_ARG, "encoder weights: null");
  GMF_REQUIRE(w->num_layers >= 0 && w->num_layers <= 64, GMF_ERR_BAD_ARG, "encoder weights: bad num_layers");
  GMF_REQUIRE(w->sigma_d > 0.f, GMF_ERR_BAD_ARG, "encoder weights: sigma_d must be positive");
  return GMF_OK;
}

static int cu_count() {
  int dev = 0;
  if (hipGetDevice(&dev) != hipSuccess) return 256;
  static int cached[16] = {0};
  if (dev >= 0 && dev < 16 && cached[dev] > 0) return cached[dev];
  int n = 0;
  if (hipDeviceGetAttribute(&n, hipDeviceAttributeMultiprocessorCount, dev) != hipSuccess || n <= 0) n = 256;
  if (dev >= 0 && dev < 16) cached[dev] = n;
  return n;
}

static void plan_attn_split(const gmf::Tuning& tune, int cus, int W, int tiles, int max_splits, bool ragged, int* n_full_out,
                            int* ksplits_out) {
  const int slots = 2 * cus;
  const int per_xcd = (W >> 3) + ((W & 7) ? 1 : 0);
  int n_full = per_xcd, ksplits = 1;
  if (max_splits > 1 && tiles >= 8) {
    const int cap = std::min(max_splits, std::max(1, tiles / 4));
    if (tune.key_splits > 1) { n_full = 0; ksplits = std::min(tune.key_splits, cap); }
    else if (tune.key_splits == 0) {
      if (W < slots / 2) { n_full = 0; ksplits = std::min(std::max(2, (slots / 2) / W), cap); }
      else if (W < 3 * slots / 4 && tiles >= 64) { n_full = 0; ksplits = std::min(2, cap); }
      else if (W > slots && tune.tail_split && !ragged) {
        const int full = (W / slots) * slots, rest = W - full;
        if (rest > 0 && 2 * rest <= slots && tiles >= 16) { n_full = full / 8; ksplits = std::min(std::min(slots / rest, 4), cap); }
      }
    }
    if (ksplits <= 1) { n_full = per_xcd; ksplits = 1; }
  }
  *n_full_out = n_full;
  *ksplits_out = ksplits;
}

static int plan_ff_split(const gmf::Tuning& tune, int base, int max_parts) {
  int hs = 1;
  if (max_parts >= 2) {
    if (tune.ff_split > 0) hs = tune.ff_split;
    else if (base < 256) hs = base <= 32 ? 8 : base <= 64 ? 4 : 2;
    hs = std::min(hs, max_parts);
    if (hs != 2 && hs != 4 && hs != 8) hs = 1;
  }
  return hs;
}

struct EncoderPlan {
  enum Form {
    kFp32,
    kStages,
    kFusedStages,
    kLinear,
    kSmall3,
  };
  Form form = kFp32;
  bool fused() const { return form >= kFusedStages; }
  bool f1_h2 = false;
  bool prologue = false;
  bool cache = false;
  bool pipelined = false;
  int fmt = 0;
  bool half = false;
  bool one_product = false;
  bool front_split = false;
  int max_splits = 0;
  int attn_nf = 0, attn_ks = 1;
  int ff_hs = 1, f1_ff_hs = 1;
  bool roles = false;
  bool q_in_attn = false;
  bool v_fp8 = false;
  bool guard = false;
  bool clear_stats = false;
  size_t act = 0, tok = 0, cache_floats = 0;
};

static EncoderPlan plan_encoder(const gmf::Tuning& t, const gmf_encoder_weights* w, int B, int N, int T, int L, int min_tiles, int cus,
                                bool dense = false) {
  EncoderPlan p;
  const int tiles = tiles_of(N), tt = tiles_of(T);
  const int W = ((tiles + 3) / 4) * B;
  const bool ragged = min_tiles > 0;
  p.act = (size_t)B * tiles * kTileFloats;
  p.tok = (size_t)B * tt * kTileFloats;
  const bool h2 = !dense && t.scattn_variant >= 9 && w->front_wst_h2 && w->ctx_wst_h2 && w->attn_wst_h2 && w->ff_wst_h2 && w->tail_wst_h2;
  const bool fusable = h2 && t.fused_linear && t.scattn_variant == 18;
  const bool half = t.precision >= 1 && fusable && W >= 256 && !ragged;
  const int fmt = half ? 1 : t.scattn_variant == 18 ? t.compat_format : 0;
  const size_t cache_floats = (size_t)B * tiles * tiles * (fmt ? 512 : 1024);
  p.cache = h2 && L > 1 && t.use_cache && cache_floats * 4 <= ((size_t)96 << 30);
  const bool fused = fusable && p.cache;
  if (p.cache) { p.cache_floats = cache_floats; p.fmt = fmt; p.half = half; }
  p.one_product = p.half && t.precision == 2;
  p.pipelined = p.cache && t.scattn_variant == 18;
  p.front_split = t.front_split && W < 128;
  p.max_splits = (p.cache && tiles >= 8) ? (W < 384 ? 8 : 4) : 0;
  plan_attn_split(t, cus, W, ragged ? min_tiles : tiles, p.max_splits, ragged, &p.attn_nf, &p.attn_ks);
  p.ff_hs = plan_ff_split(t, W, p.max_splits);
  p.f1_ff_hs = tt <= tiles ? plan_ff_split(t, ((tt + 3) / 4) * B, p.max_splits) : 1;
  if (!h2) p.form = EncoderPlan::kFp32;
  else if (!fused) p.form = EncoderPlan::kStages;
  else if (W < 256 && t.small_roles && p.attn_nf == 0 && p.attn_ks > 1 && p.ff_hs > 1 && p.max_splits == 8) p.form = EncoderPlan::kSmall3;
  else p.form = (W >= 256 || ragged) ? EncoderPlan::kLinear : EncoderPlan::kFusedStages;
  p.roles = p.form == EncoderPlan::kLinear && t.mid_grid_roles > 0 && W < t.mid_grid_roles;
  p.q_in_attn = p.form == EncoderPlan::kLinear && t.q_in_attention && !p.half && !p.roles;
  p.v_fp8 = fused && !p.half && (t.pv_fp8 == 2 || (t.pv_fp8 == 1 && w->pv_guard));
  p.clear_stats = fused && t.pv_fp8 == 1 && w->pv_guard;
  p.guard = p.clear_stats && !p.half;
  p.f1_h2 = h2 && w->f1_ctx_wst_h2 && w->f1_attn_wst_h2 && w->f1_ff_wst_h2;
  p.prologue = t.small_prologue && fused && p.f1_h2 && p.fmt == 0 && W < 256;
  return p;
}

static int prof_begin(gmf_handle* h, hipStream_t st, hipEvent_t* ev0, hipEvent_t* ev1) {
  *ev0 = *ev1 = nullptr;
  if (!h->profile) return GMF_OK;
  if (h->prof_used == h->prof_events.size()) {
    hipEvent_t a, b;
    GMF_HIP(hipEventCreate(&a));
    GMF_HIP(hipEventCreate(&b));
    h->prof_events.emplace_back(a, b);
  }
  *ev0 = h->prof_events[h->prof_used].first;
  *ev1 = h->prof_events[h->prof_used].second;
  ++h->prof_used;
  GMF_HIP(hipEventRecord(*ev0, st));
  return GMF_OK;
}

static int run_scattn(gmf_handle* h, const gmf_encoder_weights* w, const EncoderPlan& p, int l, const float* q, const float* k,
                      const float* v, const float* pts8, const float* x2, float* out, int B, int N, hipStream_t st,
                      const float* dense_compat, const gmf::CompatCache& cc) {
  const int tiles = tiles_of(N);
  const float* wst = w->tail_wst + (size_t)l * w->tail_wst_stride;
  const float* vecs = w->tail_vec + (size_t)l * w->tail_vec_stride;
  hipEvent_t ev0 = nullptr, ev1 = nullptr;
  if (int rc = prof_begin(h, st, &ev0, &ev1)) return rc;
  if (dense_compat) GMF_HIP(gmf::launch_scattn_dense(q, k, v, dense_compat, x2, wst, vecs, out, B, N, tiles, st));
  else if (p.pipelined) GMF_HIP(gmf::launch_scattn_h2p(q, k, v, x2, vecs, out, B, N, tiles, st, cc, p.attn_nf, p.attn_ks));
  else if (p.form == EncoderPlan::kStages)
    GMF_HIP(gmf::launch_scattn_h2(q, k, v, pts8, x2, wst, vecs, out, B, N, tiles, w->sigma_d, st, cc.dense));
  else GMF_HIP(gmf::launch_scattn_fp32(q, k, v, pts8, x2, wst, vecs, out, B, N, tiles, w->sigma_d, st));
  if (ev1) GMF_HIP(hipEventRecord(ev1, st));
  return GMF_OK;
}

static int run_block_tail(gmf_handle* h, const gmf_encoder_weights* w, const EncoderPlan& p, int l, const float* f, const float* q,
                          const float* k, const float* v, const float* pts8, const float* ctx_l, float* x1, float* x2,
                          float* out, int B, int N, int T, hipStream_t st, const float* dense_compat, const gmf::CompatCache& cc) {
  const int tiles = tiles_of(N), tt = tiles_of(T);
  if (p.form == EncoderPlan::kStages) {
    GMF_HIP(gmf::launch_fusion_attn_h2(true, f, ctx_l, w->attn_wst_h2 + (size_t)l * w->attn_wst_stride,
                                       w->attn_vec + (size_t)l * w->attn_vec_stride, x1, B, N, tiles, T, tt, st));
    GMF_HIP(gmf::launch_fusion_ff_h2(x1, w->ff_wst_h2 + (size_t)l * w->ff_wst_stride, w->ff_vec + (size_t)l * w->ff_vec_stride, x2, B,
                                     tiles, st, cc.part_o, p.ff_hs));
  } else {
    GMF_HIP(gmf::launch_fusion_attn(true, f, ctx_l, w->attn_wst + (size_t)l * w->attn_wst_stride,
                                    w->attn_vec + (size_t)l * w->attn_vec_stride, x1, B, N, tiles, T, tt, st));
    GMF_HIP(gmf::launch_fusion_ff(x1, w->ff_wst + (size_t)l * w->ff_wst_stride, w->ff_vec + (size_t)l * w->ff_vec_stride,
                                  x2, B, tiles, st));
  }
  return run_scattn(h, w, p, l, q, k, v, pts8, x2, out, B, N, st, dense_compat, cc);
}

static int check_ragged_sizes(gmf_handle* h, const int* n_points, int B) {
  const gmf::PairPlanStatus bad = gmf::check_pair_sizes(n_points, B);
  GMF_REQUIRE(bad != gmf::kPairPlanEmptyPair, GMF_ERR_UNSUPPORTED_SHAPE, "ragged batch: every pair needs at least one correspondence");
  GMF_REQUIRE(bad != gmf::kPairPlanTooManyRows, GMF_ERR_UNSUPPORTED_SHAPE, "ragged batch: more than 2^31 rows");
  return GMF_OK;
}

static int encoder_forward_impl(gmf_handle* h, const gmf_encoder_weights* w, const float* corr_pos, const float* src_keypts,
                                const float* tgt_keypts, const float* p_tokens, const float* q_tokens, int B, int N, int T,
                                float* logits, float* feat_n, float* feat, gmf_stream_t stream, const int* n_points);

int gmf_encoder_forward(gmf_handle* h, const gmf_encoder_weights* w, const float* corr_pos, const float* src_keypts,
                        const float* tgt_keypts, const float* p_tokens, const float* q_tokens, int B, int N, int T,
                        float* logits, float* feat_n, float* feat, gmf_stream_t stream) {
  GMF_REQUIRE(h, GMF_ERR_BAD_ARG, "encoder_forward: null handle");
  GMF_REQUIRE(B > 0 && N > 0 && T > 0, GMF_ERR_UNSUPPORTED_SHAPE, "encoder_forward: empty input");
  return encoder_forward_impl(h, w, corr_pos, src_keypts, tgt_keypts, p_tokens, q_tokens, B, N, T, logits, feat_n, feat, stream, nullptr);
}

int gmf_encoder_forward_ragged(gmf_handle* h, const gmf_encoder_weights* w, const float* corr_pos, const float* src_keypts,
                               const float* tgt_keypts, const float* p_tokens, const float* q_tokens, const int* n_points, int B,
                               int T, float* logits, float* feat_n, float* feat, gmf_stream_t stream) {
  GMF_REQUIRE(h, GMF_ERR_BAD_ARG, "encoder_forward_ragged: null handle");
  GMF_REQUIRE(n_points, GMF_ERR_BAD_ARG, "encoder_forward_ragged: null n_points");
  GMF_REQUIRE(B > 0 && T > 0, GMF_ERR_UNSUPPORTED_SHAPE, "encoder_forward_ragged: empty input");
  return encoder_forward_impl(h, w, corr_pos, src_keypts, tgt_keypts, p_tokens, q_tokens, B, 0, T, logits, feat_n, feat, stream, n_points);
}

static int encoder_forward_impl(gmf_handle* h, const gmf_encoder_weights* w, const float* corr_pos, const float* src_keypts,
                                const float* tgt_keypts, const float* p_tokens, const float* q_tokens, int B, int N, int T,
                                float* logits, float* feat_n, float* feat, gmf_stream_t stream, const int* n_points) {
  if (int rc = check_weights(h, w)) return rc;
  GMF_REQUIRE(corr_pos && src_keypts && tgt_keypts && p_tokens && q_tokens && logits && feat_n, GMF_ERR_BAD_ARG,
              "encoder_forward: null pointer");
  SetDevice sd(h, stream);
  hipStream_t st = S(stream);
  const bool ragged = n_points != nullptr;
  int min_tiles = 0;
  HostTable tab;
  const HostPart<gmf::PairTab> pairs = tab.add<gmf::PairTab>(ragged ? (size_t)B : 0);
  RingTaken ring;
  if (ragged) {
    long long n_sum = 0;
    if (int rc = check_ragged_sizes(h, n_points, B)) return rc;
    if (int rc = ring_take(h, tab, &ring)) return rc;
    gmf::plan_pair_table(n_points, B, -1.0, 0, pairs.host(ring.host), &N, &n_sum, nullptr);
    min_tiles = tiles_of(*std::min_element(n_points, n_points + B));
  }
  const int L = w->num_layers;
  const int tiles = tiles_of(N), tt = tiles_of(T);
  const EncoderPlan p = plan_encoder(h->tune, w, B, N, T, L, min_tiles, cu_count());
  GMF_REQUIRE(p.fused() || !ragged, GMF_ERR_UNSUPPORTED_SHAPE,
              "encoder_forward_ragged: ragged batches run on the default path only (split-fp16 weight images, at least two layers, the "
              "compat cache, \"fused_linear\" = 1, \"scattn_variant\" = 18)");
  const size_t act = p.act, tok = p.tok;
  char* dtab;
  float *featA, *featB, *f, *q, *k, *v, *x1, *x2, *pts8, *pimg, *qimg, *f1ctx, *x1t, *imgfeat, *ctxall, *c_dense, *ff_part, *part_o,
      *part_ml;
  unsigned *v_scale, *fstat;
  if (int rc = arena_carve(h, {arena_buf(dtab, tab.bytes()), arena_buf(featA, act), arena_buf(featB, act), arena_buf(f, act),
                               arena_buf(q, act), arena_buf(k, act), arena_buf(v, act), arena_buf(x1, act), arena_buf(x2, act),
                               arena_buf(pts8, (size_t)B * tiles * 32 * 8), arena_buf(pimg, tok), arena_buf(qimg, tok),
                               arena_buf(f1ctx, tok), arena_buf(x1t, tok), arena_buf(imgfeat, tok),
                               arena_buf(ctxall, (size_t)(L > 0 ? L : 1) * tok),
                               arena_buf(v_scale, (size_t)B * tiles * 128),
                               arena_buf(fstat, (size_t)(L + 1) * B * gmf::kPvStatStride),
                               arena_buf(c_dense, p.cache_floats),
                               arena_buf(ff_part, p.max_splits == 8 ? 8 * act : 0),
                               arena_buf(part_o, p.max_splits * act),
                               arena_buf(part_ml, (size_t)p.max_splits * B * tiles * 64)}))
    return rc;
  if (int rc = ragged ? ring_upload(h, ring, dtab, st) : GMF_OK) return rc;
  const gmf::PairTab* const ptab = ragged ? pairs.dev(dtab) : nullptr;
  gmf::CompatCache cc{c_dense, nullptr, part_o, part_ml};
  cc.half = p.half;
  cc.fmt = p.fmt;
  cc.ptab = ptab;
  cc.v_scale = p.v_fp8 ? v_scale : nullptr;
  unsigned* const zero_words = p.clear_stats ? fstat : nullptr;
  const int n_zero = p.clear_stats ? (L + 1) * B * gmf::kPvStatStride : 0;
  if (p.prologue) {
    GMF_HIP(gmf::launch_pro_ctx_pts(p_tokens, w->f1_ctx_wst_h2, w->f1_ctx_vec, f1ctx, B, T, tt, src_keypts, tgt_keypts, pts8, N, st, ptab,
                                    zero_words, n_zero));
    GMF_HIP(gmf::launch_pro_fattn_compat(q_tokens, f1ctx, w->f1_attn_wst_h2, w->f1_attn_vec, x1t, B, T, tt, pts8, c_dense, N, tiles,
                                         w->sigma_d, st, ptab));
    gmf::PvGuard g0;
    if (p.guard) g0.stat_next = fstat;
    GMF_HIP(gmf::launch_pro_ff_front(x1t, w->f1_ff_wst_h2, w->f1_ff_vec, imgfeat, B, tt, part_o, p.f1_ff_hs, corr_pos, w->front_wst_h2,
                                     w->front_vec, f, q, k, v, N, tiles, st, ptab, g0));
    if (p.f1_ff_hs > 1) GMF_HIP(gmf::launch_ff_reduce_h2(part_o, x1t, w->f1_ff_vec, imgfeat, B, tt, p.f1_ff_hs, st));
    GMF_HIP(gmf::launch_ctx_prep_h2(true, imgfeat, w->ctx_wst_h2, w->ctx_vec, ctxall, B, T, tt, L, w->ctx_wst_stride, w->ctx_vec_stride, st));
  } else {
    if (p.f1_h2) {
      GMF_HIP(gmf::launch_ctx_prep_h2(false, p_tokens, w->f1_ctx_wst_h2, w->f1_ctx_vec, f1ctx, B, T, tt, 1, 0, 0, st, true));
      GMF_HIP(gmf::launch_fusion_attn_h2(false, q_tokens, f1ctx, w->f1_attn_wst_h2, w->f1_attn_vec, x1t, B, T, tt, T, tt, st, true));
      GMF_HIP(gmf::launch_fusion_ff_h2(x1t, w->f1_ff_wst_h2, w->f1_ff_vec, imgfeat, B, tt, st, part_o, p.f1_ff_hs));
    } else {
      GMF_HIP(gmf::launch_pack_p32(p_tokens, pimg, B, T, kC, (long)T * kC, kC, 1, st));
      GMF_HIP(gmf::launch_pack_p32(q_tokens, qimg, B, T, kC, (long)T * kC, kC, 1, st));
      GMF_HIP(gmf::launch_ctx_prep(false, pimg, w->f1_ctx_wst, w->f1_ctx_vec, f1ctx, B, T, tt, 1, 0, 0, st));
      GMF_HIP(gmf::launch_fusion_attn(false, qimg, f1ctx, w->f1_attn_wst, w->f1_attn_vec, x1t, B, T, tt, T, tt, st));
      GMF_HIP(gmf::launch_fusion_ff(x1t, w->f1_ff_wst, w->f1_ff_vec, imgfeat, B, tt, st));
    }
    if (L > 0) {
      if (p.form != EncoderPlan::kFp32) GMF_HIP(gmf::launch_ctx_prep_h2(true, imgfeat, w->ctx_wst_h2, w->ctx_vec, ctxall, B, T, tt, L,
                                                                         w->ctx_wst_stride, w->ctx_vec_stride, st));
      else GMF_HIP(gmf::launch_ctx_prep(true, imgfeat, w->ctx_wst, w->ctx_vec, ctxall, B, T, tt, L, w->ctx_wst_stride,
                                        w->ctx_vec_stride, st));
    }
    GMF_HIP(gmf::launch_pack_pts8(src_keypts, tgt_keypts, pts8, B, N, st, ptab, zero_words, n_zero));
    if (p.cache) GMF_HIP(gmf::launch_compat_build(pts8, c_dense, B, N, tiles, w->sigma_d, p.fmt, st, ptab));
  }

  float* cur = featA;
  float* nxt = featB;
  if (p.fused()) {
    if (!p.prologue) {
      gmf::PvGuard g0;
      if (p.guard) g0.stat_next = fstat;
      GMF_HIP(gmf::launch_front_h2(3, p.front_split, corr_pos, w->front_wst_h2, w->front_vec, f, q, k, v, B, N, tiles, st, ptab, nullptr, g0));
    }
    for (int l = 0; l < L; ++l) {
      cc.guard = gmf::PvGuard{};
      if (p.guard) cc.guard = gmf::PvGuard{fstat + (size_t)l * B * gmf::kPvStatStride, w->pv_guard + l, fstat + (size_t)(l + 1) * B * gmf::kPvStatStride};
      const float* fw = w->front_wst_h2 + (size_t)l * w->front_wst_stride;
      const float* fv = w->front_vec + (size_t)l * w->front_vec_stride;
      const float* aw = w->attn_wst_h2 + (size_t)l * w->attn_wst_stride;
      const float* av = w->attn_vec + (size_t)l * w->attn_vec_stride;
      const float* ffw = w->ff_wst_h2 + (size_t)l * w->ff_wst_stride;
      const float* ffv = w->ff_vec + (size_t)l * w->ff_vec_stride;
      const float* ctx_l = ctxall + (size_t)l * tok;
      const bool last = (l + 1 == L);
      cc.tail_wst_h2 = w->tail_wst_h2 + (size_t)l * w->tail_wst_stride;
      cc.next_wst_h2 = last ? nullptr : w->front_wst_h2 + (size_t)(l + 1) * w->front_wst_stride;
      cc.next_bias = last ? nullptr : w->front_vec + (size_t)(l + 1) * w->front_vec_stride;
      if (p.form == EncoderPlan::kLinear) {
        cc.qf_img = p.q_in_attn ? f : nullptr;
        cc.qw_wst = p.q_in_attn ? fw + 4 * kTileFloats : nullptr;
        cc.qw_bias = p.q_in_attn ? fv + kC : nullptr;
        GMF_HIP(gmf::launch_linear_h2(p.roles, f, fw, fv, ctx_l, aw, av, ffw, ffv, p.q_in_attn ? nullptr : q, k, v, x2, B, N, tiles, T, tt,
                                      st, p.one_product, ptab, cc.v_scale, cc.guard));
      } else if (p.form == EncoderPlan::kSmall3) {
        GMF_HIP(gmf::launch_small_front_fattn(f, fw, fv, ctx_l, aw, av, q, k, v, x1, B, N, tiles, T, tt, st, cc.v_scale, cc.guard,
                                              h->tune.small_fattn_tile, ptab));
        hipEvent_t e0 = nullptr, e1 = nullptr;
        if (int rc = prof_begin(h, st, &e0, &e1)) return rc;
        GMF_HIP(gmf::launch_small_attn_ff_merge(q, k, v, x1, ffw, ffv, ff_part, p.ff_hs, w->tail_vec + (size_t)l * w->tail_vec_stride,
                                                last ? cur : f, B, N, tiles, p.attn_ks, st, &cc, h->tune.small_merge_tile));
        if (e1) GMF_HIP(hipEventRecord(e1, st));
        continue;
      } else {
        GMF_HIP(gmf::launch_front_h2(2, p.front_split, f, fw, fv, f, q, k, v, B, N, tiles, st, nullptr, cc.v_scale, cc.guard));
        GMF_HIP(gmf::launch_fusion_attn_h2(true, f, ctx_l, aw, av, x1, B, N, tiles, T, tt, st));
        GMF_HIP(gmf::launch_fusion_ff_h2(x1, ffw, ffv, x2, B, tiles, st, part_o, p.ff_hs));
      }
      if (int rc = run_scattn(h, w, p, l, q, k, v, pts8, x2, last ? cur : f, B, N, st, nullptr, cc)) return rc;
    }
    GMF_HIP(gmf::launch_head(cur, w->head_wst, w->head_vec, logits, feat_n, feat, B, N, tiles, st, h->status_dev, ptab,
                             p.guard ? fstat : nullptr, p.guard ? w->pv_guard : nullptr, L));
    return GMF_OK;
  }
  if (L == 0) {
    GMF_HIP(gmf::launch_front(1, corr_pos, w->front_wst, w->front_vec, cur, q, k, v, B, N, tiles, st));
  }
  for (int l = 0; l < L; ++l) {
    const float* in = (l == 0) ? corr_pos : cur;
    if (p.form == EncoderPlan::kStages)
      GMF_HIP(gmf::launch_front_h2(l == 0 ? 1 : 0, p.front_split, in, w->front_wst_h2 + (size_t)l * w->front_wst_stride,
                                   w->front_vec + (size_t)l * w->front_vec_stride, f, q, k, v, B, N, tiles, st));
    else GMF_HIP(gmf::launch_front(l == 0 ? 1 : 0, in, w->front_wst + (size_t)l * w->front_wst_stride,
                                   w->front_vec + (size_t)l * w->front_vec_stride, f, q, k, v, B, N, tiles, st));
    cc.tail_wst_h2 = w->tail_wst_h2 ? w->tail_wst_h2 + (size_t)l * w->tail_wst_stride : nullptr;
    if (int rc = run_block_tail(h, w, p, l, f, q, k, v, pts8, ctxall + (size_t)l * tok, x1, x2, nxt, B, N, T, st, nullptr, cc)) return rc;
    float* t = cur; cur = nxt; nxt = t;
  }
  GMF_HIP(gmf::launch_head(cur, w->head_wst, w->head_vec, logits, feat_n, feat, B, N, tiles, st, h->status_dev));
  return GMF_OK;
}

int gmf_nonlocal_block_forward(gmf_handle* h, const gmf_encoder_weights* w, int layer, int apply_pointcn,
                               const float* feat_img, const float* pts8, const float* attention,
                               const float* image_feat_img, float* out_img, int B, int N, int T, gmf_stream_t stream) {
  GMF_REQUIRE(h, GMF_ERR_BAD_ARG, "nonlocal_block_forward: null handle");
  if (int rc = check_weights(h, w)) return rc;
  GMF_REQUIRE(feat_img && image_feat_img && out_img, GMF_ERR_BAD_ARG, "nonlocal_block_forward: null pointer");
  GMF_REQUIRE((pts8 != nullptr) != (attention != nullptr), GMF_ERR_BAD_ARG, "nonlocal_block_forward: pass exactly one of pts8 / attention");
  GMF_REQUIRE(layer >= 0 && layer < w->num_layers, GMF_ERR_BAD_ARG, "nonlocal_block_forward: layer out of range");
  GMF_REQUIRE(B > 0 && N > 0 && T > 0, GMF_ERR_UNSUPPORTED_SHAPE, "nonlocal_block_forward: empty input");
  GMF_REQUIRE(apply_pointcn == 0 || apply_pointcn == 1, GMF_ERR_BAD_ARG, "nonlocal_block_forward: bad flag");
  SetDevice sd(h, stream);
  hipStream_t st = S(stream);
  const int tiles = tiles_of(N), tt = tiles_of(T);
  const EncoderPlan p = plan_encoder(h->tune, w, B, N, T, 1, 0, cu_count(), attention != nullptr);
  float *f, *q, *k, *v, *x1, *x2, *ctx;
  if (int rc = arena_carve(h, {arena_buf(f, p.act), arena_buf(q, p.act), arena_buf(k, p.act), arena_buf(v, p.act), arena_buf(x1, p.act),
                               arena_buf(x2, p.act), arena_buf(ctx, p.tok)}))
    return rc;
  if (p.form == EncoderPlan::kStages) {
    GMF_HIP(gmf::launch_front_h2(apply_pointcn ? 0 : 2, p.front_split, feat_img, w->front_wst_h2 + (size_t)layer * w->front_wst_stride,
                                 w->front_vec + (size_t)layer * w->front_vec_stride, f, q, k, v, B, N, tiles, st));
    GMF_HIP(gmf::launch_ctx_prep_h2(true, image_feat_img, w->ctx_wst_h2 + (size_t)layer * w->ctx_wst_stride,
                                    w->ctx_vec + (size_t)layer * w->ctx_vec_stride, ctx, B, T, tt, 1, 0, 0, st));
  } else {
    GMF_HIP(gmf::launch_front(apply_pointcn ? 0 : 2, feat_img, w->front_wst + (size_t)layer * w->front_wst_stride,
                              w->front_vec + (size_t)layer * w->front_vec_stride, f, q, k, v, B, N, tiles, st));
    GMF_HIP(gmf::launch_ctx_prep(true, image_feat_img, w->ctx_wst + (size_t)layer * w->ctx_wst_stride,
                                 w->ctx_vec + (size_t)layer * w->ctx_vec_stride, ctx, B, T, tt, 1, 0, 0, st));
  }
  gmf::CompatCache cc{nullptr, w->tail_wst_h2 ? w->tail_wst_h2 + (size_t)layer * w->tail_wst_stride : nullptr, nullptr, nullptr};
  return run_block_tail(h, w, p, layer, f, q, k, v, pts8, ctx, x1, x2, out_img, B, N, T, st, attention, cc);
}

int gmf_fusion_layer_forward(gmf_handle* h, int pe, int latent_dim, int d_head, const float* ctx_wst, const float* ctx_vec,
                             const float* attn_wst, const float* attn_vec, const float* ff_wst, const float* ff_vec,
                             const float* data, const float* queries, long long q_sb, long long q_sr, long long q_sk,
                             float* out, long long o_sb, long long o_sr, long long o_sk, int B, int N, int T,
                             gmf_stream_t stream, const float* ff_wst_h2, const float* ctx_wst_h2, const float* attn_wst_h2) {
  GMF_REQUIRE(h && ctx_wst && ctx_vec && attn_wst && attn_vec && ff_wst && ff_vec && data && queries && out,
              GMF_ERR_BAD_ARG, "fusion_layer_forward: null pointer");
  GMF_REQUIRE((ctx_wst_h2 == nullptr) == (attn_wst_h2 == nullptr), GMF_ERR_BAD_ARG,
              "fusion_layer_forward: ctx_wst_h2 and attn_wst_h2 go together (the attention reads the context image the "
              "context kernel of the same kind writes)");
  GMF_REQUIRE(B > 0 && N > 0 && T > 0, GMF_ERR_UNSUPPORTED_SHAPE, "fusion_layer_forward: empty input");
  const bool narrow = (latent_dim == 128 && d_head == 64), wide = (latent_dim == 256 && d_head == 128);
  GMF_REQUIRE(narrow || wide, GMF_ERR_UNSUPPORTED_SHAPE,
              "fusion_layer_forward: kernels exist for (latent_dim, d_head) = (128, 64) and (256, 128), context dim 128");
  SetDevice sd(h, stream);
  hipStream_t st = S(stream);
  const int tiles = tiles_of(N), tt = tiles_of(T);
  const size_t act = (size_t)B * tiles * 32 * latent_dim;
  const size_t tok = (size_t)B * tt * kTileFloats;
  const size_t ctxsz = wide ? 2 * tok : tok;
  const int ff_hs_w = (wide && ff_wst_h2 && h->tune.ff_split != 1) ?
                          (h->tune.ff_split > 1 ? h->tune.ff_split : gmf::plan_ff_split_w(((tiles + 3) / 4) * B)) : 1;
  float *xin, *x1, *x2, *cimg, *ctx, *ff_part_w;
  if (int rc = arena_carve(h, {arena_buf(xin, act), arena_buf(x1, act), arena_buf(x2, act), arena_buf(cimg, tok), arena_buf(ctx, ctxsz),
                               arena_buf(ff_part_w, ff_hs_w > 1 ? (size_t)ff_hs_w * act : 0)}))
    return rc;
  const bool wide_direct = wide && attn_wst_h2 != nullptr;
// ... 1215 lines not shown
```

gmf_amd/csrc/gmf_pack.cpp:

```cpp
#include "../../include/gmf_hip.h"

#include <hip/hip_runtime.h>

#include <algorithm>
#include <cmath>
#include <cstdint>
#include <cstring>
#include <map>
#include <new>
#include <string>
#include <vector>

#include "api_common.hpp"

#pragma clang fp contract(off)

namespace {

constexpr int kCw = 128;
constexpr double kLog2e = 1.4426950408889634;
constexpr float kFp16Max = 65504.0f;

struct Mat {
  int M = 0, K = 0;
// ... 197 lines not shown
  const Mat Wk = mat_of(sd, n + "projection_k.weight", kCw, kCw), Wv = mat_of(sd, n + "projection_v.weight", kCw, kCw);
  cx.img(wst, Wp, kind);
  cx.img(wst, Wq, kind);
  cx.img(wst, Wk, kind);
  cx.img(wst, Wv, kind);
  if (!vec) return;
  append(*vec, bp);
  append(*vec, bq);
  append(*vec, vec_of(sd, n + "projection_k.bias", kCw));
  append(*vec, vec_of(sd, n + "projection_v.bias", kCw));
  if (with_layer0) {
    const Mat W0 = mat_of(sd, "encoder.layer0.weight", kCw);
    if (W0.K > 8) throw PackError{GMF_ERR_UNSUPPORTED_SHAPE, "gmf: pack: in_dim > 8 is not supported by the layer0 MFMA prologue"};
    Mat W0p(kCw, 8);
    for (int r = 0; r < kCw; ++r)
      for (int c = 0; c < W0.K; ++c) W0p.at(r, c) = W0.at(r, c);
    append(*vec, vec_of(sd, "encoder.layer0.bias", kCw));
    p32(*vec, W0p);
  } else {
    append_zeros(*vec, kCw + 1024);
  }
}

constexpr double kPvGuardScore = 1024.0;
double spectral_norm(const Mat& W) {
  std::vector<double> x((size_t)W.K), y((size_t)W.M);
  for (int c = 0; c < W.K; ++c) x[c] = 1.0 + 0.01 * ((c * 37) % 17);
  double sigma = 0.0;
  for (int it = 0; it < 96; ++it) {
    double nx = 0.0;
    for (int c = 0; c < W.K; ++c) nx += x[c] * x[c];
    nx = std::sqrt(nx);
    if (!(nx > 0.0) || !std::isfinite(nx)) return nx > 0.0 ? nx : 0.0;
    for (int c = 0; c < W.K; ++c) x[c] /= nx;
    double ny = 0.0;
    for (int r = 0; r < W.M; ++r) {
      double a = 0.0;
      for (int c = 0; c < W.K; ++c) a += (double)W.at(r, c) * x[c];
      y[r] = a;
      ny += a * a;
    }
    sigma = std::sqrt(ny);
    for (int c = 0; c < W.K; ++c) {
      double a = 0.0;
      for (int r = 0; r < W.M; ++r) a += (double)W.at(r, c) * y[r];
      x[c] = a;
    }
  }
  return sigma * 1.02;
}
float pv_guard_threshold(const StateDict& sd, int layer) {
  const std::string n = "encoder.blocks.NonLocal_layer_" + std::to_string(layer) + ".";
  const Mat Wq = mat_of(sd, n + "projection_q.weight", kCw, kCw), Wk = mat_of(sd, n + "projection_k.weight", kCw, kCw);
  const std::vector<float> bq = vec_of(sd, n + "projection_q.bias", kCw), bk = vec_of(sd, n + "projection_k.bias", kCw);
  double nq = 0.0, nk = 0.0;
  for (float v : bq) nq += (double)v * v;
  for (float v : bk) nk += (double)v * v;
  nq = std::sqrt(nq); nk = std::sqrt(nk);
  const double sq = spectral_norm(Wq), sk = spectral_norm(Wk), Z = kPvGuardScore * std::sqrt((double)kCw);
  if (!std::isfinite(sq) || !std::isfinite(sk) || !std::isfinite(nq) || !std::isfinite(nk)) return -1.0f;
  const double a = sq * sk, b = sq * nk + sk * nq, c = nq * nk - Z;
  if (c >= 0.0) return -1.0f;
  if (!(a > 0.0)) return b > 0.0 ? (float)std::min(1e30, (-c / b) * (-c / b)) : 1e30f;
  const double F = (-b + std::sqrt(b * b - 4.0 * a * c)) / (2.0 * a);
  return (float)std::min(1e30, F * F);
}

void pack_tail(const StateDict& sd, int layer, Img kind, Ctx& cx, std::vector<float>& wst, std::vector<float>* vec) {
  const std::string p = "encoder.blocks.NonLocal_layer_" + std::to_string(layer) + ".fc_message.";
  Mat Wa = mat_of(sd, p + "0.weight", 64, kCw), Wb = mat_of(sd, p + "3.weight", 64, 64);
  const Mat Wc = mat_of(sd, p + "6.weight", kCw, 64);
  std::vector<float> ba = vec_of(sd, p + "0.bias", 64), bb = vec_of(sd, p + "3.bias", 64);
  fold_bn(Wa, ba, sd, p + "1.");
  fold_bn(Wb, bb, sd, p + "4.");
  cx.img(wst, Wa, kind);
  cx.img(wst, Wb, kind);
  cx.img(wst, Wc, kind);
  if (!vec) return;
  append(*vec, ba);
  append(*vec, bb);
  append(*vec, vec_of(sd, p + "6.bias", kCw));
}

void pack_head(const StateDict& sd, std::vector<float>& wst, std::vector<float>& vec) {
  p32(wst, mat_of(sd, "classification.0.weight", 32, kCw));
  p32(wst, mat_of(sd, "classification.2.weight", 32, 32));
  append_zeros(wst, 8192 - 4096 - 1024);
  append(vec, vec_of(sd, "classification.0.bias", 32));
  append(vec, vec_of(sd, "classification.2.bias", 32));
  append(vec, vec_of(sd, "classification.4.weight", 32));
  append(vec, vec_of(sd, "classification.4.bias", 1));
  append_zeros(vec, 128 - 97);
}

int read_state(gmf_handle* h, const gmf_tensor* ts, int n, int on_device, StateDict& sd, std::string& err) {
  for (int i = 0; i < n; ++i) {
    const gmf_tensor& t = ts[i];
    if (!t.name || !t.data || t.ndim < 0 || t.ndim > 4) { err = "gmf: pack: tensor " + std::to_string(i) + " has no name / data or a bad rank"; return GMF_ERR_BAD_ARG; }
    Tensor e{t.data, t.ndim, {1, 1, 1, 1}, 1};
    for (int d = 0; d < t.ndim; ++d) {
      if (t.shape[d] < 0) { err = std::string("gmf: pack: negative extent in `") + t.name + "`"; return GMF_ERR_BAD_ARG; }
      e.shape[d] = t.shape[d];
      e.numel *= t.shape[d];
    }
    if (on_device) {
      if (!h) { err = "gmf: pack: device tensors need a handle"; return GMF_ERR_BAD_ARG; }
      SetDevice sdv(h);
      sd.staged.emplace_back((size_t)e.numel);
      hipError_t rc = hipMemcpy(sd.staged.back().data(), t.data, (size_t)e.numel * sizeof(float), hipMemcpyDeviceToHost);
      if (rc != hipSuccess) { err = std::string("gmf: pack: hipMemcpy(`") + t.name + "`): " + hipGetErrorString(rc); return GMF_ERR_HIP; }
      e.data = sd.staged.back().data();
    }
    sd.t[t.name] = e;
  }
  return GMF_OK;
}

struct Block {
  std::vector<float> host;
  size_t add(const std::vector<float>& v) {
    const size_t off = (host.size() + 63) / 64 * 64;
    host.resize(off);
    host.insert(host.end(), v.begin(), v.end());
    return off;
  }
};

}

struct gmf_packed_encoder {
  gmf_encoder_weights w{};
  float sigma = 1.0f;
  int split_fp16 = 0;
  float amax = 0.f;
  float* device_block = nullptr;
  int device = -1;
  std::vector<float> host_block;
  const float* placed = nullptr;
};

struct gmf_packed_fusion {
  gmf_fusion_weights w{};
  float* device_block = nullptr;
  int device = -1;
  std::vector<float> host_block;
  const float* placed = nullptr;
};

namespace {

int place(gmf_handle* h, Block& blk, std::vector<float>& host_keep, float** device_block, int* device, const float** base, std::string& err,
          bool host_only = false) {
  if (!h || host_only) {
    host_keep.swap(blk.host);
    *base = host_keep.data();
    return GMF_OK;
  }
  SetDevice sd(h);
  void* d = nullptr;
  hipError_t rc = hipMalloc(&d, blk.host.size() * sizeof(float));
  if (rc != hipSuccess) { err = std::string("gmf: pack: hipMalloc: ") + hipGetErrorString(rc); return GMF_ERR_OOM; }
  rc = hipMemcpy(d, blk.host.data(), blk.host.size() * sizeof(float), hipMemcpyHostToDevice);
  if (rc != hipSuccess) { (void)hipFree(d); err = std::string("gmf: pack: hipMemcpy: ") + hipGetErrorString(rc); return GMF_ERR_HIP; }
  *device_block = static_cast<float*>(d);
  *device = h->device;
  *base = *device_block;
  return GMF_OK;
}

}

extern "C" {

int gmf_encoder_pack_weights(gmf_handle* h, const gmf_tensor* tensors, int n_tensors, int num_layers, int flags,
                             gmf_packed_encoder** out) {
  if (!out) return GMF_ERR_BAD_ARG;
  *out = nullptr;
  std::string err;
  auto bail = [&](int code, const std::string& m) { if (h) h->err = m; return code; };
  if (!tensors || n_tensors <= 0 || num_layers < 0 || num_layers > 64) return bail(GMF_ERR_BAD_ARG, "gmf: encoder_pack_weights: bad arguments");
  const bool on_device = (flags & GMF_PACK_DEVICE_TENSORS) != 0, standalone = (flags & GMF_PACK_STANDALONE_BLOCK) != 0;
  gmf_packed_encoder* p = new (std::nothrow) gmf_packed_encoder();
  if (!p) return GMF_ERR_OOM;
  try {
    StateDict sd;
    if (int rc = read_state(h, tensors, n_tensors, on_device, sd, err)) { delete p; return bail(rc, err); }
    const int L = num_layers;
    const bool has_f1 = sd.has("encoder.fusion_layer_1.cross_attend_blocks.0.fn.to_q.weight");
    const bool has_l0 = sd.has("encoder.layer0.weight");
    const bool has_head = sd.has("classification.0.weight");
    Block blk;
    struct Off { size_t v = 0; bool set = false; };
    auto put = [&](Off& o, const std::vector<float>& v) { o.v = blk.add(v); o.set = true; };
    Off f1[6], f1h[3], ctx[2], attn[2], ff[2], front[2], tail[2], head[2], ctxh, attnh, ffh, fronth, tailh, pvgo;
    Ctx c32, ch2;
    if (has_f1) {
      FusionBlobs b = pack_fusion(sd, "encoder.fusion_layer_1.", false, Img::F32, c32);
      if (b.lat != 128) throw PackError{GMF_ERR_UNSUPPORTED_SHAPE, "gmf: pack: fusion_layer_1 must be 128 wide"};
      put(f1[0], b.ctx_wst); put(f1[1], b.ctx_vec); put(f1[2], b.attn_wst); put(f1[3], b.attn_vec); put(f1[4], b.ff_wst); put(f1[5], b.ff_vec);
      FusionBlobs bh = pack_fusion(sd, "encoder.fusion_layer_1.", false, Img::H2S, ch2);
      put(f1h[0], bh.ctx_wst); put(f1h[1], bh.attn_wst); put(f1h[2], bh.ff_wst);
    }
    if (L > 0) {
      std::vector<float> cw, cv, aw, av, fw, fv, cwh, awh, fwh, frw, frv, frwh, tw, tv, twh, pvg;
      for (int l = 0; l < L; ++l) {
        const std::string pre = "encoder.blocks.NonLocal_layer_" + std::to_string(l) + ".fusion_layer_2.";
        FusionBlobs b = pack_fusion(sd, pre, true, Img::F32, c32);
        if (b.lat != 128) throw PackError{GMF_ERR_UNSUPPORTED_SHAPE, "gmf: pack: fusion_layer_2 must be 128 wide"};
        append(cw, b.ctx_wst); append(cv, b.ctx_vec); append(aw, b.attn_wst); append(av, b.attn_vec); append(fw, b.ff_wst); append(fv, b.ff_vec);
        FusionBlobs bh = pack_fusion(sd, pre, true, Img::H2S, ch2);
        append(cwh, bh.ctx_wst); append(awh, bh.attn_wst); append(fwh, bh.ff_wst);
        pack_front(sd, l, l == 0 && has_l0, standalone, Img::F32, c32, frw, &frv);
        pack_front(sd, l, l == 0 && has_l0, standalone, Img::H2S, ch2, frwh, nullptr);
        pack_tail(sd, l, Img::F32, c32, tw, &tv);
        pack_tail(sd, l, Img::H2S, ch2, twh, nullptr);
        pvg.push_back(pv_guard_threshold(sd, l));
      }
      put(ctx[0], cw); put(ctx[1], cv); put(attn[0], aw); put(attn[1], av); put(ff[0], fw); put(ff[1], fv);
      put(front[0], frw); put(front[1], frv); put(tail[0], tw); put(tail[1], tv);
      put(ctxh, cwh); put(attnh, awh); put(ffh, fwh); put(fronth, frwh); put(tailh, twh); put(pvgo, pvg);
    }
    if (has_head) {
      std::vector<float> hw, hv;
      pack_head(sd, hw, hv);
      put(head[0], hw); put(head[1], hv);
    }
    p->split_fp16 = ch2.ok ? 1 : 0;
    p->amax = ch2.amax;
    p->sigma = sd.has("sigma") ? need(sd, "sigma").data[0] : 1.0f;
    const float sigma_d = sd.has("sigma_spat") ? need(sd, "sigma_spat").data[0] : 0.1f;
    const float* base = nullptr;
    if (int rc = place(h, blk, p->host_block, &p->device_block, &p->device, &base, err, (flags & GMF_PACK_HOST_BLOCK) != 0)) { delete p; return bail(rc, err); }
    auto at = [&](const Off& o) -> const float* { return o.set ? base + o.v : nullptr; };
    gmf_encoder_weights& w = p->w;
    w.num_layers = L;
    w.f1_ctx_wst = at(f1[0]); w.f1_ctx_vec = at(f1[1]); w.f1_attn_wst = at(f1[2]); w.f1_attn_vec = at(f1[3]);
    w.f1_ff_wst = at(f1[4]); w.f1_ff_vec = at(f1[5]);
    w.ctx_wst = at(ctx[0]); w.ctx_vec = at(ctx[1]); w.ctx_wst_stride = 16384; w.ctx_vec_stride = 768;
    w.attn_wst = at(attn[0]); w.attn_vec = at(attn[1]); w.attn_wst_stride = 16384; w.attn_vec_stride = 896;
    w.ff_wst = at(ff[0]); w.ff_vec = at(ff[1]); w.ff_wst_stride = 196608; w.ff_vec_stride = 1408;
    w.front_wst = at(front[0]); w.front_vec = at(front[1]); w.front_wst_stride = 65536; w.front_vec_stride = 1664;
    w.tail_wst = at(tail[0]); w.tail_vec = at(tail[1]); w.tail_wst_stride = 20480; w.tail_vec_stride = 256;
    w.head_wst = at(head[0]); w.head_vec = at(head[1]);
    w.sigma_d = sigma_d;
    w.pv_guard = at(pvgo);
    if (ch2.ok) {
      w.front_wst_h2 = at(fronth); w.ctx_wst_h2 = at(ctxh); w.attn_wst_h2 = at(attnh); w.ff_wst_h2 = at(ffh);
      w.f1_ctx_wst_h2 = at(f1h[0]); w.f1_attn_wst_h2 = at(f1h[1]); w.f1_ff_wst_h2 = at(f1h[2]);
      w.tail_wst_h2 = at(tailh);
    }
  } catch (const PackError& e) {
    delete p;
    return bail(e.code, e.msg);
  } catch (const std::bad_alloc&) {
    delete p;
    return bail(GMF_ERR_OOM, "gmf: pack: out of host memory");
  }
  *out = p;
  return GMF_OK;
}

const gmf_encoder_weights* gmf_packed_encoder_weights(const gmf_packed_encoder* p) { return p ? &p->w : nullptr; }

int gmf_packed_encoder_info(const gmf_packed_encoder* p, float* sigma, float* sigma_d, int* split_fp16, float* max_abs_scaled) {
  if (!p) return GMF_ERR_BAD_ARG;
  if (sigma) *sigma = p->sigma;
  if (sigma_d) *sigma_d = p->w.sigma_d;
  if (split_fp16) *split_fp16 = p->split_fp16;
  if (max_abs_scaled) *max_abs_scaled = p->amax;
  return GMF_OK;
}

void gmf_packed_encoder_free(gmf_packed_encoder* p) {
  if (!p) return;
  if (p->device_block) {
    int prev = -1;
    (void)hipGetDevice(&prev);
    (void)hipSetDevice(p->device);
    (void)hipFree(p->device_block);
    if (prev >= 0 && prev != p->device) (void)hipSetDevice(prev);
  }
  delete p;
}

int gmf_fusion_pack_weights(gmf_handle* h, const gmf_tensor* tensors, int n_tensors, const char* prefix, int pe, int flags,
                            gmf_packed_fusion** out) {
  if (!out) return GMF_ERR_BAD_ARG;
  *out = nullptr;
  std::string err;
  auto bail = [&](int code, const std::string& m) { if (h) h->err = m; return code; };
  if (!tensors || n_tensors <= 0) return bail(GMF_ERR_BAD_ARG, "gmf: fusion_pack_weights: bad arguments");
  gmf_packed_fusion* p = new (std::nothrow) gmf_packed_fusion();
  if (!p) return GMF_ERR_OOM;
  try {
    StateDict sd;
    if (int rc = read_state(h, tensors, n_tensors, (flags & GMF_PACK_DEVICE_TENSORS) != 0, sd, err)) { delete p; return bail(rc, err); }
    const std::string pre = prefix ? prefix : "";
    Ctx c32, ch2;
    FusionBlobs b = pack_fusion(sd, pre, pe != 0, Img::F32, c32);
    FusionBlobs bh = pack_fusion(sd, pre, pe != 0, Img::H2S, ch2);
    Block blk;
    const size_t o0 = blk.add(b.ctx_wst), o1 = blk.add(b.ctx_vec), o2 = blk.add(b.attn_wst), o3 = blk.add(b.attn_vec), o4 = blk.add(b.ff_wst),
                 o5 = blk.add(b.ff_vec), o6 = blk.add(bh.ctx_wst), o7 = blk.add(bh.attn_wst), o8 = blk.add(bh.ff_wst);
    const float* base = nullptr;
    if (int rc = place(h, blk, p->host_block, &p->device_block, &p->device, &base, err, (flags & GMF_PACK_HOST_BLOCK) != 0)) { delete p; return bail(rc, err); }
    gmf_fusion_weights& w = p->w;
    w.latent_dim = b.lat; w.d_head = b.dh; w.pe = pe != 0;
    w.ctx_wst = base + o0; w.ctx_vec = base + o1; w.attn_wst = base + o2; w.attn_vec = base + o3; w.ff_wst = base + o4; w.ff_vec = base + o5;
    if (ch2.ok) { w.ctx_wst_h2 = base + o6; w.attn_wst_h2 = base + o7; w.ff_wst_h2 = base + o8; }
    w.split_fp16 = ch2.ok ? 1 : 0;
    w.max_abs_scaled = ch2.amax;
  } catch (const PackError& e) {
    delete p;
    return bail(e.code, e.msg);
  } catch (const std::bad_alloc&) {
    delete p;
    return bail(GMF_ERR_OOM, "gmf: pack: out of host memory");
  }
  *out = p;
  return GMF_OK;
}

const gmf_fusion_weights* gmf_packed_fusion_weights(const gmf_packed_fusion* p) { return p ? &p->w : nullptr; }

void gmf_packed_fusion_free(gmf_packed_fusion* p) {
  if (!p) return;
  if (p->device_block) {
    int prev = -1;
    (void)hipGetDevice(&prev);
    (void)hipSetDevice(p->device);
    (void)hipFree(p->device_block);
    if (prev >= 0 && prev != p->device) (void)hipSetDevice(prev);
  }
  delete p;
}

}

namespace {
inline void rebase_ptr(const float*& ptr, const float* from, size_t n, const float* to) {
  if (ptr && ptr >= from && ptr < from + n) ptr = to + (ptr - from);
}
int place_into(gmf_handle* h, const std::vector<float>& host_block, void* device_dst, long long bytes, gmf_stream_t stream, const char* what) {
  if (!h || !device_dst) return GMF_ERR_BAD_ARG;
  if (host_block.empty()) { h->err = std::string("gmf: ") + what + ": the object was not packed with a NULL handle (its block is not in host memory)"; return GMF_ERR_BAD_ARG; }
  if ((size_t)bytes < host_block.size() * sizeof(float) || ((uintptr_t)device_dst & 255u)) {
    h->err = std::string("gmf: ") + what + ": the destination must be 256-byte aligned and hold " + std::to_string(host_block.size() * sizeof(float)) + " B";
    return GMF_ERR_BAD_ARG;
  }
  SetDevice sd(h, stream);
  hipStream_t st = reinterpret_cast<hipStream_t>(stream);
  hipError_t rc = hipMemcpyAsync(device_dst, host_block.data(), host_block.size() * sizeof(float), hipMemcpyHostToDevice, st);
  if (rc == hipSuccess) rc = hipStreamSynchronize(st);
  if (rc != hipSuccess) { h->err = std::string("gmf: ") + what + ": copy to the device: " + hipGetErrorString(rc); return GMF_ERR_HIP; }
  return GMF_OK;
}
}

extern "C" {

long long gmf_packed_encoder_bytes(const gmf_packed_encoder* p) {
  return p ? (long long)(p->host_block.size() * sizeof(float)) : 0;
}

int gmf_packed_encoder_place(gmf_handle* h, gmf_packed_encoder* p, void* device_dst, long long bytes, gmf_stream_t stream) {
  if (!h || !p) return GMF_ERR_BAD_ARG;
  if (int rc = place_into(h, p->host_block, device_dst, bytes, stream, "packed_encoder_place")) return rc;
  const float* from = p->placed ? p->placed : p->host_block.data();
  const float* to = static_cast<const float*>(device_dst);
  const size_t n = p->host_block.size();
  gmf_encoder_weights& w = p->w;
  const float** ptrs[] = {&w.f1_ctx_wst, &w.f1_ctx_vec, &w.f1_attn_wst, &w.f1_attn_vec, &w.f1_ff_wst, &w.f1_ff_vec, &w.ctx_wst, &w.ctx_vec,
                          &w.attn_wst, &w.attn_vec, &w.ff_wst, &w.ff_vec, &w.front_wst, &w.front_vec, &w.tail_wst, &w.tail_vec, &w.head_wst,
                          &w.head_vec, &w.front_wst_h2, &w.ctx_wst_h2, &w.attn_wst_h2, &w.ff_wst_h2, &w.f1_ctx_wst_h2, &w.f1_attn_wst_h2,
                          &w.f1_ff_wst_h2, &w.tail_wst_h2, &w.pv_guard};
  for (const float** q : ptrs) rebase_ptr(*q, from, n, to);
  p->placed = to;
  return GMF_OK;
}

long long gmf_packed_fusion_bytes(const gmf_packed_fusion* p) {
  return p ? (long long)(p->host_block.size() * sizeof(float)) : 0;
}

int gmf_packed_fusion_place(gmf_handle* h, gmf_packed_fusion* p, void* device_dst, long long bytes, gmf_stream_t stream) {
  if (!h || !p) return GMF_ERR_BAD_ARG;
  if (int rc = place_into(h, p->host_block, device_dst, bytes, stream, "packed_fusion_place")) return rc;
  const float* from = p->placed ? p->placed : p->host_block.data();
  const float* to = static_cast<const float*>(device_dst);
  const size_t n = p->host_block.size();
  gmf_fusion_weights& w = p->w;
  const float** ptrs[] = {&w.ctx_wst, &w.ctx_vec, &w.attn_wst, &w.attn_vec, &w.ff_wst, &w.ff_vec, &w.ctx_wst_h2, &w.attn_wst_h2, &w.ff_wst_h2};
  for (const float** q : ptrs) rebase_ptr(*q, from, n, to);
  p->placed = to;
  return GMF_OK;
}

}
```

gmf_amd/csrc/launchers.hpp:

```cpp
#pragma once
#include <hip/hip_runtime.h>

#include "pair_plan.hpp"

namespace gmf {


constexpr int kPvStatStride = 32;
struct PvGuard {
  const unsigned* stat = nullptr;
  const float* thr2 = nullptr;
  unsigned* stat_next = nullptr;
};

struct CompatCache {
  const float* dense;
  const float* tail_wst_h2;
  float* part_o;
  float* part_ml;
  const float* next_wst_h2 = nullptr;
  const float* next_bias = nullptr;
  bool half = false;
  const PairTab* ptab = nullptr;
  int fmt = 0;
  unsigned* v_scale = nullptr;
  const float* qf_img = nullptr;
  const float* qw_wst = nullptr;
  const float* qw_bias = nullptr;
  PvGuard guard;
};

struct Tuning {
  int scattn_variant = 18;
  bool use_cache = true;
  int key_splits = 0;
  bool tail_split = false;
  int ff_split = 0;
  bool front_split = true;
  bool wide_attn_tile = true;
  bool small_merge_tile = true;
  bool small_fattn_tile = true;
  bool small_roles = true;
  bool fused_linear = true;
  int conv_patch = 1;
  bool small_prologue = true;
  bool conv_small = true;
  int nms_binned = 1;
  bool topk_select = true;
  int mid_grid_roles = 512;
  bool q_in_attention = true;
  int pv_fp8 = 1;
  int compat_format = 0;
  int precision = 0;
  int spectral_col_splits = 0;
  int clique_local_rows = 384;
};

hipError_t launch_compat_build(const float* pts8, float* c_dense, int B, int N, int tiles, float sigma_d, int fmt, hipStream_t s,
                               const PairTab* ptab = nullptr);
hipError_t launch_front(int mode, const float* in, const float* wst, const float* vecs, float* f, float* q, float* k,
                        float* v, int B, int N, int tiles, hipStream_t s);
hipError_t launch_scattn_fp32(const float* q, const float* k, const float* v, const float* pts8, const float* fus,
                              const float* wst, const float* vecs, float* out, int B, int N, int tiles, float sigma_d,
                              hipStream_t s);
hipError_t launch_scattn_h2(const float* q, const float* k, const float* v, const float* pts8, const float* fus, const float* wst,
                            const float* vecs, float* out, int B, int N, int tiles, float sigma_d, hipStream_t s, const float* c_dense);
hipError_t launch_scattn_h2p(const float* q, const float* k, const float* v, const float* fus, const float* vecs, float* out, int B,
                             int N, int tiles, hipStream_t s, const CompatCache& cc, int n_full, int ksplits);
hipError_t launch_scattn_dense(const float* q, const float* k, const float* v, const float* compat, const float* fus,
                               const float* wst, const float* vecs, float* out, int B, int N, int tiles, hipStream_t s);
hipError_t launch_ctx_prep(bool pe, const float* ctx, const float* wst, const float* vecs, float* out, int B, int T,
                           int ttiles, int sets, int wst_stride, int vec_stride, hipStream_t s);
hipError_t launch_fusion_attn(bool pe, const float* x, const float* ctx_img, const float* wst, const float* vecs,
                              float* x1, int B, int N, int tiles, int T, int ttiles, hipStream_t s);
hipError_t launch_fusion_ff(const float* x1, const float* wst, const float* vecs, float* x2, int B, int tiles, hipStream_t s);
hipError_t launch_head(const float* feat_img, const float* wst, const float* vecs, float* logits, float* feat_n,
                       float* feat_rm, int B, int N, int tiles, hipStream_t s, int* status = nullptr, const PairTab* ptab = nullptr,
                       const unsigned* pv_stat = nullptr, const float* pv_thr2 = nullptr, int n_layers = 0);
hipError_t launch_ctx_prep_w(bool pe, const float* ctx, const float* wst, const float* vecs, float* out, int B, int T,
                             int ttiles, hipStream_t s);
hipError_t launch_fusion_attn_w(bool pe, const float* x, const float* ctx_img, const float* wst, const float* vecs,
                                float* x1, int B, int N, int tiles, int T, int ttiles, hipStream_t s);
hipError_t launch_fusion_ff_w(const float* x1, const float* wst, const float* vecs, float* x2, int B, int tiles, hipStream_t s);
hipError_t launch_ctx_prep_w_h2(bool pe, const float* ctx, const float* wst_h2, const float* vecs, float* out, int B, int T,
                                int ttiles, hipStream_t s, bool rowmajor = false);
hipError_t launch_fusion_attn_w_h2(bool pe, const float* x, const float* ctx_img, const float* wst_h2, const float* vecs,
                                   float* x1, int B, int N, int tiles, int T, int ttiles, hipStream_t s, bool tile_form = true);
hipError_t launch_fusion_ff_w_h2(const float* x1, const float* wst_h2, const float* vecs, float* x2, int B, int tiles, hipStream_t s,
                                 float* part = nullptr, int hs = 1, float* out_rm = nullptr, long o_sb = 0, long o_sr = 0,
                                 long o_sk = 0, int n_rows = 0, int* status = nullptr);
int plan_ff_split_w(int base_wgs);
hipError_t launch_front_h2(int mode, bool split, const float* in, const float* wst, const float* vecs, float* f, float* q, float* k,
                           float* v, int B, int N, int tiles, hipStream_t s, const PairTab* ptab = nullptr, unsigned* v_scale = nullptr,
                           PvGuard guard = {});
hipError_t launch_linear_h2(bool roles, const float* f, const float* front_wst, const float* front_vec, const float* ctx_img,
                            const float* attn_wst, const float* attn_vec, const float* ff_wst, const float* ff_vec, float* q,
                            float* k, float* v, float* x2, int B, int N, int tiles, int T, int ttiles, hipStream_t s, bool one_product = false,
                            const PairTab* ptab = nullptr, unsigned* v_scale = nullptr, PvGuard guard = {});
hipError_t launch_small_front_fattn(const float* f, const float* front_wst, const float* front_vec, const float* ctx_img,
                                    const float* attn_wst, const float* attn_vec, float* q, float* k, float* v, float* x1, int B,
                                    int N, int tiles, int T, int ttiles, hipStream_t s, unsigned* v_scale = nullptr, PvGuard guard = {},
                                    bool tile_role = true, const PairTab* ptab = nullptr);
hipError_t launch_small_attn_ff_merge(const float* q, const float* k, const float* v, const float* x1, const float* ff_wst,
                                      const float* ff_vecs, float* ff_part, int ff_hs, const float* tail_vecs, float* out, int B,
                                      int N, int tiles, int ksplits, hipStream_t s, const CompatCache* cc, bool tile_merge = true);
hipError_t launch_ctx_prep_h2(bool pe, const float* ctx, const float* wst, const float* vecs, float* out, int B, int T,
                              int ttiles, int sets, int wst_stride, int vec_stride, hipStream_t s, bool rowmajor = false);
hipError_t launch_fusion_attn_h2(bool pe, const float* x, const float* ctx_img, const float* wst, const float* vecs,
                                 float* x1, int B, int N, int tiles, int T, int ttiles, hipStream_t s, bool rowmajor = false);
hipError_t launch_pro_ctx_pts(const float* p_tokens, const float* wst, const float* vecs, float* f1ctx, int B, int T, int ttiles,
                              const float* src, const float* tgt, float* pts8, int N, hipStream_t s, const PairTab* ptab,
                              unsigned* zero_words, int n_zero);
hipError_t launch_pro_fattn_compat(const float* q_tokens, const float* f1ctx, const float* wst, const float* vecs, float* x1t, int B,
                                   int T, int ttiles, const float* pts8, float* c_dense, int N, int tiles, float sigma_d,
                                   hipStream_t s, const PairTab* ptab);
hipError_t launch_pro_ff_front(const float* x1t, const float* wst, const float* vecs, float* imgfeat, int B, int ttiles, float* part,
                               int hs, const float* corr_pos, const float* fwst, const float* fvecs, float* f, float* q, float* k,
                               float* v, int N, int tiles, hipStream_t s, const PairTab* ptab, PvGuard guard);
hipError_t launch_ff_reduce_h2(const float* part, const float* x1, const float* vecs, float* x2, int B, int tiles, int hs, hipStream_t s);
hipError_t launch_fusion_ff_h2(const float* x1, const float* wst, const float* vecs, float* x2, int B, int tiles, hipStream_t s,
                               float* part = nullptr, int hs = 1);
int padded_desc_width(int d);
hipError_t launch_nn_match(const float* F0, const float* F1, float* f0_img, float* f1_img, float* norm2, unsigned long long* best, int* idx,
                           float* dist, int N0, int N1, int d, int mode, hipStream_t s);
struct MatchPair { int row0, n0, key0, n1, tile0, stage0, stages, wg0, wgx, ks, pad0, pad1; };
static_assert(sizeof(MatchPair) == 48, "tests/abi_cpp/host_table_host.cpp lays the correspondence table out with a 48-byte stand-in");
struct MatchTotals { long tiles0, stages, wgs, rows0; int tps; };
bool plan_nn_match_batched(const int* off0, const int* off1, int B, int K, MatchPair* tab, MatchTotals* tot);
hipError_t launch_nn_match_batched(const float* F0, const float* F1, float* f0_img, float* f1_img, float* norm2, unsigned long long* best,
                                   const MatchPair* tab, int B, const MatchTotals& tot, int d, int mode, int global_index, int* idx,
                                   float* dist, hipStream_t s);
hipError_t launch_seed_dist(const float* featn_img, const int* seeds, float* dist, int B, int N, int S, hipStream_t s, const PairTab* ptab = nullptr);
hipError_t launch_pack_p32(const float* src, float* dst, int B, int n_rows, int K, long sb, long sr, long sk, hipStream_t s, const PairTab* ptab = nullptr);
hipError_t launch_pack_rows_h2(const float* src, float* dst, int B, int n_rows, hipStream_t s, const PairTab* ptab = nullptr,
                               const float* copy_src = nullptr, float* copy_dst = nullptr, long n_copy = 0);
hipError_t launch_unpack_p32(const float* src, float* dst, int B, int n_rows, int K, long sb, long sr, long sk, hipStream_t s, int* status = nullptr);
hipError_t launch_pack_pts8(const float* src, const float* tgt, float* dst, int B, int N, hipStream_t s, const PairTab* ptab = nullptr,
                            unsigned* zero_words = nullptr, int n_zero = 0);

size_t similarity_image_floats(int B, int N);
int sm_fused_parts_per_pair(int B, int N);
int sm_parts_per_pair(int B, int N);
int classification_parts(int B, int N);
int transformation_slices(int B, int N);
hipError_t launch_similarity_matrix(const float* feat_n, float* img, float* M, int B, int N, int ldm, float sigma,
                                    hipStream_t s, const float* sigma_dev = nullptr);
hipError_t launch_sm_loss_fused(const float* feat_n, const float* gt, float* img, double* part, double* pair_loss, int B,
                                int N, float sigma, int balanced, float* out, hipStream_t s, const float* sigma_dev = nullptr);
hipError_t launch_sm_loss(const float* M, int ldm, const float* gt, double* part, double* pair_loss, int B, int N,
                          int balanced, float* out, hipStream_t s);
int sm_backward_parts(int B, int N);
hipError_t launch_sm_backward(const float* feat_n, const float* gt, float* img, float* timg, float* consts, double* dsig_part,
                              int B, int N, float sigma, int balanced, float* dF, float* dsigma, hipStream_t s,
                              const float* sigma_dev = nullptr);
hipError_t launch_classification_loss(const float* pred, const float* gt, const float* weight, double* part, int B, int N,
                                      int balanced, float* out, hipStream_t s);
hipError_t launch_transformation_loss(const float* trans, const float* gt_trans, const float* src, const float* tgt,
                                      const float* probs, double* part, int B, int N, float re_thre, float te_thre,
                                      float* out, hipStream_t s);

int gemm_ksplits(bool ta, bool tb, const float* A, const float* B, int M, int N, int K, long lda, long ldb, long sA, long sB,
                 int batch);
hipError_t launch_gemm_f32(bool ta, bool tb, const float* A, const float* B, float* C, const float* bias, const float* R, int M, int N,
                           int K, long lda, long ldb, long ldc, long sA, long sB, long sC, int batch, float alpha, float* part,
                           int ksplits, int relu, hipStream_t s);
hipError_t launch_lcpe(bool backward, const float* x, const float* w, const float* bias, float* y, int rows, int L, int C, hipStream_t s);
hipError_t launch_ln_fwd(const float* x, const float* gamma, const float* beta, float* y, float* mean, float* rstd, long rows, int C,
                         hipStream_t s);
hipError_t launch_ln_bwd(const float* dy, const float* x, const float* gamma, const float* mean, const float* rstd, const float* dx_add,
                         float* dx, long rows, int C, hipStream_t s);
hipError_t launch_softmax(bool backward, const float* a, const float* b, const float* mul, float* out, long rows, int T, float scale,
                          hipStream_t s);
hipError_t launch_geglu(bool backward, const float* hdn, const float* dg, float* out, long rows, int H, hipStream_t s);
int colsum_chunks(long rows);
hipError_t launch_colsum(const float* x, const float* y, const float* mean, const float* rstd, const float* cmean, const float* crstd,
                         int center_x, int shift, int L, long rows, int C, float* part, float* out, hipStream_t s,
                         const float* relu_y = nullptr, bool dual = false, float* out2 = nullptr);
hipError_t launch_bn_finish(const float* sum, const float* sumsq, float* mean, float* rstd, float* run_mean, float* run_var, int C,
                            long rows, float eps, float momentum, hipStream_t s);
hipError_t launch_bn_apply(const float* x, const float* mean, const float* rstd, const float* gamma, const float* beta, float* y,
                           long rows, int C, int relu, const float* residual, hipStream_t s);
// ... 20 lines not shown
```

include/gmf_hip.h:

```cpp
#ifndef GMF_HIP_H_
#define GMF_HIP_H_

#ifdef __cplusplus
extern "C" {
#endif

typedef struct gmf_handle gmf_handle;
typedef void* gmf_stream_t;

enum {
  GMF_OK = 0,
  GMF_ERR_BAD_ARG = -1,
  GMF_ERR_UNSUPPORTED_SHAPE = -2,
  GMF_ERR_HIP = -3,
  GMF_ERR_NO_DEVICE = -4,
  GMF_ERR_OOM = -5,
  GMF_ERR_WORKSPACE = -6
};

#define GMF_ABI_VERSION 5

int gmf_abi_version(void);
int gmf_create(int device, gmf_handle** out);
void gmf_destroy(gmf_handle* h);
const char* gmf_last_error_string(gmf_handle* h);
long long gmf_workspace_bytes(gmf_handle* h);
int gmf_set_workspace(gmf_handle* h, void* device_ptr, long long bytes);
long long gmf_workspace_wanted(gmf_handle* h);

#define GMF_STATUS_NONFINITE 1
#define GMF_STATUS_PV_GUARDED 2
#define GMF_STATUS_SPARSE_DUPLICATE 4
#define GMF_STATUS_BATCHNORM_ROWS 8
#define GMF_STATUS_POSEGRAPH_PIVOT 16
int gmf_status_read(gmf_handle* h, int* flags, int clear);

int gmf_set_sigma_device(gmf_handle* h, const float* sigma_dev);

int gmf_set_tuning(gmf_handle* h, const char* name, int value);
int gmf_get_tuning(gmf_handle* h, const char* name, int* value);

int gmf_profile_enable(gmf_handle* h, int on);
int gmf_profile_read(gmf_handle* h, double* scattn_ms_total, int* scattn_launches);

int gmf_pack_rows_p32(gmf_handle* h, const float* src, long long sb, long long sr, long long sk, int B, int n_rows,
                      int K, float* dst, gmf_stream_t stream);
int gmf_unpack_rows_p32(gmf_handle* h, const float* src_img, int B, int n_rows, int K, float* dst, long long sb,
                        long long sr, long long sk, gmf_stream_t stream);
int gmf_pack_pts8(gmf_handle* h, const float* src, const float* tgt, int B, int N, float* dst, gmf_stream_t stream);

int gmf_front_forward(gmf_handle* h, int first, const float* in, const float* wst, const float* vecs, float* f,
                      float* q, float* k, float* v, int B, int N, gmf_stream_t stream);
int gmf_scattn_forward(gmf_handle* h, const float* q, const float* k, const float* v, const float* pts8,
                       const float* fusion2_out, const float* wst, const float* vecs, float* out, int B, int N,
                       float sigma_d, gmf_stream_t stream);
int gmf_scattn_forward_dense(gmf_handle* h, const float* q, const float* k, const float* v, const float* attention,
                             const float* fusion2_out, const float* wst, const float* vecs, float* out, int B, int N,
                             gmf_stream_t stream);
int gmf_fusion_ctx_prepare(gmf_handle* h, int pe, const float* ctx, const float* wst, const float* vecs, float* out,
                           int B, int T, int sets, int wst_stride, int vec_stride, gmf_stream_t stream);
int gmf_fusion_attn_forward(gmf_handle* h, int pe, const float* x, const float* ctx_img, const float* wst,
                            const float* vecs, float* x1, int B, int N, int T, gmf_stream_t stream);
int gmf_fusion_ff_forward(gmf_handle* h, const float* x1, const float* wst, const float* vecs, float* x2, int B,
                          int N, gmf_stream_t stream);
int gmf_classifier_forward(gmf_handle* h, const float* feat_img, const float* wst, const float* vecs, float* logits,
                           float* feat_n, float* feat, int B, int N, gmf_stream_t stream);

typedef struct gmf_encoder_weights {
  int num_layers;
  const float* f1_ctx_wst;  const float* f1_ctx_vec;
  const float* f1_attn_wst; const float* f1_attn_vec;
  const float* f1_ff_wst;   const float* f1_ff_vec;
  const float* ctx_wst;     const float* ctx_vec;   int ctx_wst_stride,   ctx_vec_stride;
  const float* attn_wst;    const float* attn_vec;  int attn_wst_stride,  attn_vec_stride;
  const float* ff_wst;      const float* ff_vec;    int ff_wst_stride,    ff_vec_stride;
  const float* front_wst;   const float* front_vec; int front_wst_stride, front_vec_stride;
  const float* tail_wst;    const float* tail_vec;  int tail_wst_stride,  tail_vec_stride;
  const float* head_wst;    const float* head_vec;
  float sigma_d;
  const float* front_wst_h2; const float* ctx_wst_h2; const float* attn_wst_h2; const float* ff_wst_h2;
  const float* f1_ctx_wst_h2; const float* f1_attn_wst_h2; const float* f1_ff_wst_h2;
  const float* tail_wst_h2;
  const float* pv_guard;
} gmf_encoder_weights;

typedef struct gmf_tensor {
  const char* name;
  const float* data;
  int ndim;
  long long shape[4];
} gmf_tensor;
#define GMF_PACK_DEVICE_TENSORS 1
#define GMF_PACK_STANDALONE_BLOCK 2
#define GMF_PACK_HOST_BLOCK 4
typedef struct gmf_packed_encoder gmf_packed_encoder;
int gmf_encoder_pack_weights(gmf_handle* h, const gmf_tensor* tensors, int n_tensors, int num_layers, int flags,
                             gmf_packed_encoder** out);
const struct gmf_encoder_weights* gmf_packed_encoder_weights(const gmf_packed_encoder* p);
int gmf_packed_encoder_info(const gmf_packed_encoder* p, float* sigma, float* sigma_d, int* split_fp16, float* max_abs_scaled);
void gmf_packed_encoder_free(gmf_packed_encoder* p);
long long gmf_packed_encoder_bytes(const gmf_packed_encoder* p);
int gmf_packed_encoder_place(gmf_handle* h, gmf_packed_encoder* p, void* device_dst, long long bytes, gmf_stream_t stream);

typedef struct gmf_fusion_weights {
  int latent_dim, d_head, pe, split_fp16;
  float max_abs_scaled;
  const float *ctx_wst, *ctx_vec, *attn_wst, *attn_vec, *ff_wst, *ff_vec;
  const float *ctx_wst_h2, *attn_wst_h2, *ff_wst_h2;
} gmf_fusion_weights;
typedef struct gmf_packed_fusion gmf_packed_fusion;
int gmf_fusion_pack_weights(gmf_handle* h, const gmf_tensor* tensors, int n_tensors, const char* prefix, int pe, int flags,
                            gmf_packed_fusion** out);
const gmf_fusion_weights* gmf_packed_fusion_weights(const gmf_packed_fusion* p);
void gmf_packed_fusion_free(gmf_packed_fusion* p);
long long gmf_packed_fusion_bytes(const gmf_packed_fusion* p);
int gmf_packed_fusion_place(gmf_handle* h, gmf_packed_fusion* p, void* device_dst, long long bytes, gmf_stream_t stream);

int gmf_encoder_forward(gmf_handle* h, const gmf_encoder_weights* w, const float* corr_pos, const float* src_keypts,
                        const float* tgt_keypts, const float* p_tokens, const float* q_tokens, int B, int N, int T,
                        float* logits, float* feat_n, float* feat, gmf_stream_t stream);

int gmf_encoder_forward_ragged(gmf_handle* h, const gmf_encoder_weights* w, const float* corr_pos, const float* src_keypts,
                               const float* tgt_keypts, const float* p_tokens, const float* q_tokens, const int* n_points, int B,
                               int T, float* logits, float* feat_n, float* feat, gmf_stream_t stream);

int gmf_nonlocal_block_forward(gmf_handle* h, const gmf_encoder_weights* w, int layer, int apply_pointcn,
                               const float* feat_img, const float* pts8, const float* attention,
                               const float* image_feat_img, float* out_img, int B, int N, int T, gmf_stream_t stream);

int gmf_fusion_layer_forward(gmf_handle* h, int pe, int latent_dim, int d_head, const float* ctx_wst, const float* ctx_vec,
                             const float* attn_wst, const float* attn_vec, const float* ff_wst, const float* ff_vec,
                             const float* data, const float* queries, long long q_sb, long long q_sr, long long q_sk,
                             float* out, long long o_sb, long long o_sr, long long o_sk, int B, int N, int T,
                             gmf_stream_t stream, const float* ff_wst_h2, const float* ctx_wst_h2, const float* attn_wst_h2);

typedef struct gmf_pose_params {
  int num_seeds;
  int k;
  int num_iterations;
  int use_nms;
  int refine_iters;
  float sigma;
  float sigma_d;
  float inlier_threshold;
  float nms_radius;
  float refine_threshold;
} gmf_pose_params;

int gmf_pose_head(gmf_handle* h, const gmf_pose_params* p, const float* feat_n, const float* src_keypts,
                  const float* tgt_keypts, const float* logits, const int* seeds_in, int B, int N, float* final_trans,
                  float* final_labels, int* seeds_out, int* knn_out, float* seed_trans, float* fitness,
                  gmf_stream_t stream);

int gmf_pose_head_ragged(gmf_handle* h, const gmf_pose_params* p, double ratio, const float* feat_n, const float* src_keypts,
                         const float* tgt_keypts, const float* logits, const int* n_points, int B, float* final_trans,
                         float* final_labels, int* seeds_out, int* knn_out, float* seed_trans, float* fitness,
                         gmf_stream_t stream);

int gmf_pick_seeds(gmf_handle* h, const float* src_keypts, const float* scores, int B, int N, float nms_radius,
                   int use_nms, int num_seeds, int* seeds_out, gmf_stream_t stream);

int gmf_knn_rows(gmf_handle* h, const float* feat_n, const int* rows, int B, int N, int S, int k, int* knn_out,
                 gmf_stream_t stream);

int gmf_knn_from_distances(gmf_handle* h, const float* dist, int B, int N, int S, int k, int* knn_out, gmf_stream_t stream);

int gmf_nn_match(gmf_handle* h, const float* F0, const float* F1, int N0, int N1, int d, int mode, int* idx_out,
// ... 260 lines not shown
```

Measured before the change: 9.842 million.

## Fold K and V projections into Q-side and output weights for attention

Precomputes at pack time a folded Q weight (Wk^T Wq), bias terms, and a folded message weight (Wa·Wv), so the linear kernel writes the raw features directly as K and V (V through an LDS transpose) instead of running two projection GEMMs. The attention kernel adds a per-row beta bias into the score accumulator to account for the folded key bias. This removes per-point K/V matmuls at the cost of an extra packed weight block, an LDS transpose, and numerics that now depend on the folded fp16-split weights.

Result: faster. 10.08 million (median of 6 runs) (+2.5%).

```diff
diff --git a/gmf_amd/_lib.py b/gmf_amd/_lib.py
--- a/gmf_amd/_lib.py
+++ b/gmf_amd/_lib.py
@@ -32,6 +32,7 @@
         ("f1_ctx_wst_h2", _vp), ("f1_attn_wst_h2", _vp), ("f1_ff_wst_h2", _vp),
         ("tail_wst_h2", _vp),
         ("pv_guard", _vp),
+        ("kv_fold", _vp),
     ]
 
 
diff --git a/gmf_amd/csrc/encoder_h2.hip b/gmf_amd/csrc/encoder_h2.hip
--- a/gmf_amd/csrc/encoder_h2.hip
+++ b/gmf_amd/csrc/encoder_h2.hip
@@ -618,7 +618,7 @@
 
 constexpr int kLinLdsFloats = 4 * kStageFloats + 7 * C + (3 * C + 2 * FFH) + kWavesPerWG * 2 * C + 3 * C;
 
-template <int PART, int NP = 3, bool QSKIP = false>
+template <int PART, int NP = 3, bool QSKIP = false, bool KVF = false>
 GMF_DEVINL void linear_h2_body(float* lds, const float* __restrict__ f_in, const float* __restrict__ front_wst,
                                const float* __restrict__ front_vec, const float* __restrict__ ctx_img,
                                const float* __restrict__ attn_wst, const float* __restrict__ attn_vec,
@@ -626,7 +626,9 @@
                                float* __restrict__ k_out, float* __restrict__ v_out, float* __restrict__ x2_out, int N, int tiles,
                                int T, int ttiles, const PairTab* __restrict__ ptab = nullptr,
                                unsigned* __restrict__ v_scale = nullptr,
-                               const PvGuard guard = {}) {
+                               const PvGuard guard = {},
+                               const float* __restrict__ kvf_wst = nullptr, const float* __restrict__ kvf_bias = nullptr) {
+  static_assert(!KVF || (NP == 3 && PART != 2), "the folded form: parity numerics, the kernel or its projection role");
   const int lane = threadIdx.x & 63, h = lane >> 5, i = lane & 31;
   const int wave = __builtin_amdgcn_readfirstlane(threadIdx.x >> 6);
   const int pair = blockIdx.y;
@@ -643,14 +645,18 @@
   float* const lvec_f = lvec_a + 7 * C;
   float* const halo = lvec_f + (3 * C + 2 * FFH) + wave * (2 * C);
   float* const lvec_p = lvec_f + (3 * C + 2 * FFH) + kWavesPerWG * (2 * C);
-  if (PART != 2) dma_vec(front_vec + C, lvec_p, 3 * C, wave, kWavesPerWG, lane);
+  if (PART != 2 && KVF) { if (!QSKIP) dma_vec(kvf_bias, lvec_p, C, wave, kWavesPerWG, lane); }
+  else if (PART != 2) dma_vec(front_vec + C, lvec_p, 3 * C, wave, kWavesPerWG, lane);
   if (PART != 1) {
     dma_vec(attn_vec, lvec_a, 7 * C, wave, kWavesPerWG, lane);
     dma_vec(ff_vec, lvec_f, 3 * C + 2 * FFH, wave, kWavesPerWG, lane);
     LcpeHalo<CF>::issue(pair_base, tile, tiles_p, halo, lane);
   }
   StageRing<4> ss;
-  if (PART == 0) ss.init(lds, wave, lane, front_wst + (QSKIP ? 8 : 4) * kStageFloats, QSKIP ? 8 : 12, attn_wst, 2,
+  if (KVF && PART == 1) ss.init(lds, wave, lane, kvf_wst, 4);
+  else if (KVF && QSKIP) ss.init(lds, wave, lane, attn_wst, 2, ctx_img + (size_t)pair * ttiles * kStageFloats, ttiles, attn_wst + 2 * kStageFloats, 2);
+  else if (KVF) ss.init(lds, wave, lane, kvf_wst, 4, attn_wst, 2, ctx_img + (size_t)pair * ttiles * kStageFloats, ttiles, attn_wst + 2 * kStageFloats, 2);
+  else if (PART == 0) ss.init(lds, wave, lane, front_wst + (QSKIP ? 8 : 4) * kStageFloats, QSKIP ? 8 : 12, attn_wst, 2,
                          ctx_img + (size_t)pair * ttiles * kStageFloats, ttiles, attn_wst + 2 * kStageFloats, 2);
   else if (PART == 1) ss.init(lds, wave, lane, front_wst + 4 * kStageFloats, 12);
   else ss.init(lds, wave, lane, attn_wst, 2, ctx_img + (size_t)pair * ttiles * kStageFloats, ttiles, attn_wst + 2 * kStageFloats, 2);
@@ -663,9 +669,44 @@
     ss.prime();
     const bool v8 = pv_planes_on(v_scale, guard, pair);
     unsigned* const sw_tile = v_scale ? v_scale + ((size_t)pair * tiles + tile) * 128 + lane : nullptr;
-    unsigned ksw = 0;
-#pragma unroll
-    for (int which = (QSKIP ? 1 : 0); which < 2; ++which) {
+    unsigned ksw = 0, vsw = 0;
+    if (KVF) {
+      asm volatile("s_waitcnt vmcnt(12)" ::: "memory");
+      __syncthreads();
+      float* const mt = lds + 3 * kStageFloats + wave * 1024;
+#pragma unroll
+      for (int mb = 0; mb < 4; ++mb) {
+        float t[16], td[16];
+#pragma unroll
+        for (int r = 0; r < 16; ++r) t[r] = f[16 * mb + r];
+        if (v8) store_block_v8(k_out + toff, mb, t, lane, ksw);
+        else store_block_h2(k_out + toff, mb, t, lane);
+#pragma unroll
+        for (int r = 0; r < 16; ++r) mt[i * 32 + (frag_feature(r, h) ^ i)] = t[r];
+        asm volatile("s_waitcnt lgkmcnt(0)" ::: "memory");
+#pragma unroll
+        for (int r = 0; r < 16; ++r) { const int kk = frag_feature(r, h); td[r] = mt[kk * 32 + (i ^ kk)]; }
+        asm volatile("s_waitcnt lgkmcnt(0)" ::: "memory");
+        if (v8) store_block_v8(v_out + toff, mb, td, lane, vsw);
+        else store_block_h2(v_out + toff, mb, td, lane);
+      }
+      if (v_scale) { sw_tile[0] = vsw; sw_tile[64] = ksw; }
+      if (!QSKIP) {
+#pragma unroll
+        for (int mb = 0; mb < 4; ++mb) {
+          const f16x8* lw = as_h2(ss.acquire());
+          f32x16 acc = zero16();
+          mma_wx_h2n<8, NP>(acc, lw, fx);
+          float t[16], bb[16];
+          load_vec_block(bb, lvec_p, mb, h);
+#pragma unroll
+          for (int r = 0; r < 16; ++r) t[r] = fmaf(acc[r], kH2Inv, bb[r]);
+          store_block_h2(q_out + toff, mb, t, lane);
+        }
+      }
+    }
+#pragma unroll
+    for (int which = (KVF ? 2 : QSKIP ? 1 : 0); which < 2; ++which) {
       float* dst = (which == 0 ? q_out : k_out) + toff;
 #pragma unroll
       for (int mb = 0; mb < 4; ++mb) {
@@ -684,9 +725,8 @@
         else store_block_h2(dst, mb, t, lane);
       }
     }
-    unsigned vsw = 0;
-#pragma unroll
-    for (int db = 0; db < 4; ++db) {
+#pragma unroll
+    for (int db = (KVF ? 4 : 0); db < 4; ++db) {
       const f16x8* lw = as_h2(PART == 1 ? ss.acquire() : ss.acquire_counted<20>());
       f32x16 acc = zero16();
       mma_xw_h2n<8, NP>(acc, lw, fx);
@@ -697,7 +737,7 @@
       if (v8) store_block_v8(v_out + toff, db, t, lane, vsw);
       else store_block_h2(v_out + toff, db, t, lane);
     }
-    if (v_scale) { sw_tile[0] = vsw; sw_tile[64] = ksw; }
+    if (v_scale && !KVF) { sw_tile[0] = vsw; sw_tile[64] = ksw; }
   }
 
   if (PART == 1) {
@@ -729,7 +769,7 @@
         }
 #pragma unroll
         for (int mb = 0; mb < 2; ++mb) {
-          const f16x8* lw = as_h2(ss.acquire());
+          const f16x8* lw = as_h2((KVF && QSKIP && PART == 0) ? ss.acquire_counted<40>() : ss.acquire());
           f32x16 acc = zero16();
           mma_wx_h2n<8, NP>(acc, lw, nx);
           float t[16];
@@ -843,29 +883,32 @@
   }
 }
 
-template <int NP, bool QSKIP = false>
+template <int NP, bool QSKIP = false, bool KVF = false>
 __global__ void __launch_bounds__(256, 2)
 k_linear_h2(const float* __restrict__ f_in, const float* __restrict__ front_wst, const float* __restrict__ front_vec,
             const float* __restrict__ ctx_img, const float* __restrict__ attn_wst, const float* __restrict__ attn_vec,
             const float* __restrict__ ff_wst, const float* __restrict__ ff_vec, float* __restrict__ q_out,
             float* __restrict__ k_out, float* __restrict__ v_out, float* __restrict__ x2_out, int N, int tiles, int T,
-            int ttiles, const PairTab* __restrict__ ptab, unsigned* __restrict__ v_scale, const PvGuard guard) {
+            int ttiles, const PairTab* __restrict__ ptab, unsigned* __restrict__ v_scale, const PvGuard guard,
+            const float* __restrict__ kvf_wst, const float* __restrict__ kvf_bias) {
   __shared__ __attribute__((aligned(16))) float lds[kLinLdsFloats];
   tail_priority(blockIdx.y * gridDim.x + blockIdx.x, gridDim.x * gridDim.y);
-  linear_h2_body<0, NP, QSKIP>(lds, f_in, front_wst, front_vec, ctx_img, attn_wst, attn_vec, ff_wst, ff_vec, q_out, k_out, v_out, x2_out, N,
-                               tiles, T, ttiles, ptab, v_scale, guard);
-}
-
+  linear_h2_body<0, NP, QSKIP, KVF>(lds, f_in, front_wst, front_vec, ctx_img, attn_wst, attn_vec, ff_wst, ff_vec, q_out, k_out, v_out, x2_out, N,
+                                    tiles, T, ttiles, ptab, v_scale, guard, kvf_wst, kvf_bias);
+}
+
+template <bool KVF>
 __global__ void __launch_bounds__(256, 2)
 k_linear_roles(const float* __restrict__ f_in, const float* __restrict__ front_wst, const float* __restrict__ front_vec,
                const float* __restrict__ ctx_img, const float* __restrict__ attn_wst, const float* __restrict__ attn_vec,
                const float* __restrict__ ff_wst, const float* __restrict__ ff_vec, float* __restrict__ q_out,
                float* __restrict__ k_out, float* __restrict__ v_out, float* __restrict__ x2_out, int N, int tiles, int T,
-               int ttiles, unsigned* __restrict__ v_scale, const PvGuard guard, const PairTab* __restrict__ ptab) {
+               int ttiles, unsigned* __restrict__ v_scale, const PvGuard guard, const PairTab* __restrict__ ptab,
+               const float* __restrict__ kvf_wst, const float* __restrict__ kvf_bias) {
   __shared__ __attribute__((aligned(16))) float lds[kLinLdsFloats];
   if (blockIdx.z == 0)
-    linear_h2_body<1>(lds, f_in, front_wst, front_vec, ctx_img, attn_wst, attn_vec, ff_wst, ff_vec, q_out, k_out, v_out, x2_out, N,
-                      tiles, T, ttiles, ptab, v_scale, guard);
+    linear_h2_body<1, 3, false, KVF>(lds, f_in, front_wst, front_vec, ctx_img, attn_wst, attn_vec, ff_wst, ff_vec, q_out, k_out, v_out, x2_out, N,
+                                     tiles, T, ttiles, ptab, v_scale, guard, kvf_wst, kvf_bias);
   else
     linear_h2_body<2>(lds, f_in, front_wst, front_vec, ctx_img, attn_wst, attn_vec, ff_wst, ff_vec, q_out, k_out, v_out, x2_out, N,
                       tiles, T, ttiles, ptab);
@@ -916,19 +959,30 @@
 hipError_t launch_linear_h2(bool roles, const float* f, const float* front_wst, const float* front_vec, const float* ctx_img,
                             const float* attn_wst, const float* attn_vec, const float* ff_wst, const float* ff_vec, float* q,
                             float* k, float* v, float* x2, int B, int N, int tiles, int T, int ttiles, hipStream_t s,
-                            bool one_product, const PairTab* ptab, unsigned* v_scale, PvGuard guard) {
-  if (roles)
-    hipLaunchKernelGGL(k_linear_roles, tgrid(tiles, B, 2), dim3(256), 0, s, f, front_wst, front_vec, ctx_img, attn_wst, attn_vec,
-                       ff_wst, ff_vec, q, k, v, x2, N, tiles, T, ttiles, v_scale, guard, ptab);
+                            bool one_product, const PairTab* ptab, unsigned* v_scale, PvGuard guard, const float* kvf_wst,
+                            const float* kvf_bias) {
+  const float* const none = nullptr;
+  if (roles && kvf_wst)
+    hipLaunchKernelGGL(k_linear_roles<true>, tgrid(tiles, B, 2), dim3(256), 0, s, f, front_wst, front_vec, ctx_img, attn_wst, attn_vec,
+                       ff_wst, ff_vec, q, k, v, x2, N, tiles, T, ttiles, v_scale, guard, ptab, kvf_wst, kvf_bias);
+  else if (roles)
+    hipLaunchKernelGGL(k_linear_roles<false>, tgrid(tiles, B, 2), dim3(256), 0, s, f, front_wst, front_vec, ctx_img, attn_wst, attn_vec,
+                       ff_wst, ff_vec, q, k, v, x2, N, tiles, T, ttiles, v_scale, guard, ptab, none, none);
+  else if (kvf_wst && !q)
+    hipLaunchKernelGGL((k_linear_h2<3, true, true>), tgrid(tiles, B), dim3(256), 0, s, f, front_wst, front_vec, ctx_img, attn_wst, attn_vec, ff_wst,
+                       ff_vec, q, k, v, x2, N, tiles, T, ttiles, ptab, v_scale, guard, kvf_wst, kvf_bias);
+  else if (kvf_wst)
+    hipLaunchKernelGGL((k_linear_h2<3, false, true>), tgrid(tiles, B), dim3(256), 0, s, f, front_wst, front_vec, ctx_img, attn_wst, attn_vec, ff_wst,
+                       ff_vec, q, k, v, x2, N, tiles, T, ttiles, ptab, v_scale, guard, kvf_wst, kvf_bias);
   else if (one_product)
     hipLaunchKernelGGL(k_linear_h2<1>, tgrid(tiles, B), dim3(256), 0, s, f, front_wst, front_vec, ctx_img, attn_wst, attn_vec, ff_wst,
-                       ff_vec, q, k, v, x2, N, tiles, T, ttiles, ptab, v_scale, guard);
+                       ff_vec, q, k, v, x2, N, tiles, T, ttiles, ptab, v_scale, guard, none, none);
   else if (!q)
     hipLaunchKernelGGL((k_linear_h2<3, true>), tgrid(tiles, B), dim3(256), 0, s, f, front_wst, front_vec, ctx_img, attn_wst, attn_vec, ff_wst,
-                       ff_vec, q, k, v, x2, N, tiles, T, ttiles, ptab, v_scale, guard);
+                       ff_vec, q, k, v, x2, N, tiles, T, ttiles, ptab, v_scale, guard, none, none);
   else
     hipLaunchKernelGGL(k_linear_h2<3>, tgrid(tiles, B), dim3(256), 0, s, f, front_wst, front_vec, ctx_img, attn_wst, attn_vec, ff_wst,
-                       ff_vec, q, k, v, x2, N, tiles, T, ttiles, ptab, v_scale, guard);
+                       ff_vec, q, k, v, x2, N, tiles, T, ttiles, ptab, v_scale, guard, none, none);
   return hipGetLastError();
 }
 
diff --git a/gmf_amd/csrc/encoder_kernels.hip b/gmf_amd/csrc/encoder_kernels.hip
--- a/gmf_amd/csrc/encoder_kernels.hip
+++ b/gmf_amd/csrc/encoder_kernels.hip
@@ -562,7 +562,7 @@
 }
 
 constexpr float kInvU16 = 1.0f / 65535.0f;
-template <int NPROD = 3, int CFMT = 0, int WAVES = 4, bool PVF8 = false>
+template <int NPROD = 3, int CFMT = 0, int WAVES = 4, bool PVF8 = false, bool FOLD = false>
 GMF_DEVINL void scattn_h2p_body(float* lds, const int bid, const float* __restrict__ q_img, const float* __restrict__ k_img,
                                 const float* __restrict__ v_img, const float* __restrict__ fus, const float* __restrict__ wst,
                                 const float* __restrict__ vecs, float* out, int N, int tiles, int wgs_per_pair,
@@ -572,8 +572,10 @@
                                 const unsigned* __restrict__ v_scale = nullptr,
                                 const float* qf_img = nullptr, const float* __restrict__ qw_wst = nullptr,
                                 const float* __restrict__ qw_bias = nullptr,
-                                unsigned* __restrict__ stat_next = nullptr) {
+                                unsigned* __restrict__ stat_next = nullptr,
+                                const float* __restrict__ kvf_vec = nullptr) {
   static_assert(!PVF8 || NPROD == 3, "the fp8 cross products belong to the three-product form");
+  static_assert(!FOLD || (NPROD == 3 && WAVES == 4), "the folded form belongs to the parity kernels");
   float* const ldsK = lds;
   float* const ldsV = lds + 2 * kStageFloats;
   const int lane = threadIdx.x & 63, h = lane >> 5;
@@ -597,12 +599,21 @@
   const size_t toff = (pbase + tile) * (32 * C);
 
   f16x8 qh[8], ql[8];
-  if (NPROD == 3 && WAVES == 4 && qf_img) {
+  float beta = 0.f;
+  auto fold_beta = [&](const float (&fq)[CF]) {
+    float uv[CF], bs = 0.f;
+    load_vec_frag<CF>(uv, kvf_vec, h);
+#pragma unroll
+    for (int e = 0; e < CF; ++e) bs = fmaf(fq[e], uv[e], bs);
+    beta = xhalf_sum(bs) + kvf_vec[C];
+  };
+  if (NPROD == 3 && WAVES == 4 && qw_wst) {
     FragH2<8> fx;
     {
       float fq[CF];
       load_frag_p32<CF>(fq, qf_img + toff, lane);
       fx.set(fq);
+      if (FOLD) fold_beta(fq);
     }
 #pragma unroll
     for (int st = 0; st < 4; ++st) dma_4k_s(qw_wst + st * kStageFloats + wave * 1024, lds + st * kStageFloats + wave * 1024, lane_off16);
@@ -628,7 +639,22 @@
       qh[s] = qp[(0 * 8 + s) * 64];
       if (NPROD == 3) ql[s] = qp[(1 * 8 + s) * 64];
     }
-  }
+    if (FOLD) {
+      float fq[CF];
+      load_frag_p32<CF>(fq, qf_img + toff, lane);
+      fold_beta(fq);
+    }
+  }
+  auto s_start = [&]() -> f32x16 {
+    f32x16 z = zero16();
+    if (FOLD) {
+      float b = beta;
+      asm volatile("" : "+v"(b));
+#pragma unroll
+      for (int r = 0; r < 16; ++r) z[r] = b;
+    }
+    return z;
+  };
   i32x8 qb[4];
   unsigned qsw = 0;
   if (PVF8) {
@@ -724,7 +750,7 @@
   fetch_c(t_begin);
   asm volatile("s_waitcnt vmcnt(0)" ::: "memory");
   __syncthreads();
-  f32x16 s_a = zero16(), s_b;
+  f32x16 s_a = s_start(), s_b;
   auto s_cross8 = [&](f32x16 acc, const f16x8* lkt, const int cb, const unsigned kscale) -> f32x16 {
     const i32x4* l8 = reinterpret_cast<const i32x4*>(lkt);
     const i32x4 a_lo = l8[(1 * 8 + 2 * cb) * 64], a_hi = l8[(1 * 8 + 2 * cb + 1) * 64];
@@ -803,7 +829,7 @@
       m_off = m_new - 10.0f;
       rescale(moved, alpha);
     }
-    s_next = zero16();
+    s_next = s_start();
     {
       f16x8 kh = lk[0], kl = kh;
       if (NPROD == 3) kl = lk[8 * 64];
@@ -870,7 +896,7 @@
     i32x8 pb;
     f16x8 vr[3];
     auto hslot = [](int u) { return (0 * 8 + 2 * (u & 3) + (u >> 2)) * 64; };
-    s_next = zero16();
+    s_next = s_start();
     {
       const i32x4* lk8 = reinterpret_cast<const i32x4*>(lk);
       f16x8 kh = lk[0];
@@ -1076,7 +1102,7 @@
   return pv_planes_on(v_scale, guard, ptab ? ptab[slot].ord : slot);
 }
 
-template <int NPROD, int CFMT, bool PVF8 = false>
+template <int NPROD, int CFMT, bool PVF8 = false, bool FOLD = false>
 __global__ void __launch_bounds__(256, 2)
 k_scattn_h2p(const float* __restrict__ q_img, const float* __restrict__ k_img, const float* __restrict__ v_img,
              const float* __restrict__ fus, const float* __restrict__ wst, const float* __restrict__ vecs,
@@ -1084,17 +1110,17 @@
              int n_items, int n_full, int ksplits, float* __restrict__ part_o, float* __restrict__ part_ml,
              const float* __restrict__ next_wst, const float* __restrict__ next_bias, const PairTab* __restrict__ ptab,
              const unsigned* __restrict__ v_scale, const float* qf_img, const float* __restrict__ qw_wst,
-             const float* __restrict__ qw_bias, const PvGuard guard) {
+             const float* __restrict__ qw_bias, const PvGuard guard, const float* __restrict__ kvf_vec) {
   __shared__ __attribute__((aligned(16))) float lds[4 * kStageFloats];
   tail_priority(blockIdx.x, gridDim.x);
   if (!PVF8 || attn_pv_on(v_scale, guard, blockIdx.x, n_items, n_full, ksplits, wgs_per_pair, ptab))
-    scattn_h2p_body<NPROD, CFMT, 4, PVF8>(lds, blockIdx.x, q_img, k_img, v_img, fus, wst, vecs, out, N, tiles, wgs_per_pair, c_dense, n_items,
-                                          n_full, ksplits, part_o, part_ml, next_wst, next_bias, ptab, v_scale, qf_img, qw_wst, qw_bias,
-                                          guard.stat_next);
+    scattn_h2p_body<NPROD, CFMT, 4, PVF8, FOLD>(lds, blockIdx.x, q_img, k_img, v_img, fus, wst, vecs, out, N, tiles, wgs_per_pair, c_dense, n_items,
+                                                n_full, ksplits, part_o, part_ml, next_wst, next_bias, ptab, v_scale, qf_img, qw_wst, qw_bias,
+                                                guard.stat_next, kvf_vec);
   else
-    scattn_h2p_body<NPROD, CFMT, 4, false>(lds, blockIdx.x, q_img, k_img, v_img, fus, wst, vecs, out, N, tiles, wgs_per_pair, c_dense, n_items,
-                                           n_full, ksplits, part_o, part_ml, next_wst, next_bias, ptab, nullptr, qf_img, qw_wst, qw_bias,
-                                           guard.stat_next);
+    scattn_h2p_body<NPROD, CFMT, 4, false, FOLD>(lds, blockIdx.x, q_img, k_img, v_img, fus, wst, vecs, out, N, tiles, wgs_per_pair, c_dense, n_items,
+                                                 n_full, ksplits, part_o, part_ml, next_wst, next_bias, ptab, nullptr, qf_img, qw_wst, qw_bias,
+                                                 guard.stat_next, kvf_vec);
 }
 
 __global__ void __launch_bounds__(256, 2)
@@ -2038,19 +2064,25 @@
                        cc.next_wst_h2, cc.next_bias);
   else if (cc.half)
     hipLaunchKernelGGL((k_scattn_h2p<1, 1>), grid, dim3(256), 0, s, q, k, v, fus, cc.tail_wst_h2, vecs, out, N, tiles, wpp, cc.dense, W,
-                       n_full, ksplits, cc.part_o, cc.part_ml, cc.next_wst_h2, cc.next_bias, cc.ptab, (const unsigned*)nullptr, (const float*)nullptr, (const float*)nullptr, (const float*)nullptr, PvGuard{});
+                       n_full, ksplits, cc.part_o, cc.part_ml, cc.next_wst_h2, cc.next_bias, cc.ptab, (const unsigned*)nullptr, (const float*)nullptr, (const float*)nullptr, (const float*)nullptr, PvGuard{}, (const float*)nullptr);
   else if (cc.fmt == 2 && cc.v_scale)
     hipLaunchKernelGGL((k_scattn_h2p<3, 2, true>), grid, dim3(256), 0, s, q, k, v, fus, cc.tail_wst_h2, vecs, out, N, tiles, wpp, cc.dense,
-                       W, n_full, ksplits, cc.part_o, cc.part_ml, cc.next_wst_h2, cc.next_bias, cc.ptab, cc.v_scale, cc.qf_img, cc.qw_wst, cc.qw_bias, cc.guard);
+                       W, n_full, ksplits, cc.part_o, cc.part_ml, cc.next_wst_h2, cc.next_bias, cc.ptab, cc.v_scale, cc.qf_img, cc.qw_wst, cc.qw_bias, cc.guard, (const float*)nullptr);
   else if (cc.fmt == 2)
     hipLaunchKernelGGL((k_scattn_h2p<3, 2>), grid, dim3(256), 0, s, q, k, v, fus, cc.tail_wst_h2, vecs, out, N, tiles, wpp, cc.dense,
-                       W, n_full, ksplits, cc.part_o, cc.part_ml, cc.next_wst_h2, cc.next_bias, cc.ptab, (const unsigned*)nullptr, cc.qf_img, cc.qw_wst, cc.qw_bias, PvGuard{});
+                       W, n_full, ksplits, cc.part_o, cc.part_ml, cc.next_wst_h2, cc.next_bias, cc.ptab, (const unsigned*)nullptr, cc.qf_img, cc.qw_wst, cc.qw_bias, PvGuard{}, (const float*)nullptr);
+  else if (cc.kvf_vec && cc.v_scale)
+    hipLaunchKernelGGL((k_scattn_h2p<3, 0, true, true>), grid, dim3(256), 0, s, q, k, v, fus, cc.tail_wst_h2, vecs, out, N, tiles, wpp, cc.dense,
+                       W, n_full, ksplits, cc.part_o, cc.part_ml, cc.next_wst_h2, cc.next_bias, cc.ptab, cc.v_scale, cc.qf_img, cc.qw_wst, cc.qw_bias, cc.guard, cc.kvf_vec);
+  else if (cc.kvf_vec)
+    hipLaunchKernelGGL((k_scattn_h2p<3, 0, false, true>), grid, dim3(256), 0, s, q, k, v, fus, cc.tail_wst_h2, vecs, out, N, tiles, wpp, cc.dense,
+                       W, n_full, ksplits, cc.part_o, cc.part_ml, cc.next_wst_h2, cc.next_bias, cc.ptab, (const unsigned*)nullptr, cc.qf_img, cc.qw_wst, cc.qw_bias, PvGuard{}, cc.kvf_vec);
   else if (cc.v_scale)
     hipLaunchKernelGGL((k_scattn_h2p<3, 0, true>), grid, dim3(256), 0, s, q, k, v, fus, cc.tail_wst_h2, vecs, out, N, tiles, wpp, cc.dense,
-                       W, n_full, ksplits, cc.part_o, cc.part_ml, cc.next_wst_h2, cc.next_bias, cc.ptab, cc.v_scale, cc.qf_img, cc.qw_wst, cc.qw_bias, cc.guard);
+                       W, n_full, ksplits, cc.part_o, cc.part_ml, cc.next_wst_h2, cc.next_bias, cc.ptab, cc.v_scale, cc.qf_img, cc.qw_wst, cc.qw_bias, cc.guard, (const float*)nullptr);
   else
     hipLaunchKernelGGL((k_scattn_h2p<3, 0>), grid, dim3(256), 0, s, q, k, v, fus, cc.tail_wst_h2, vecs, out, N, tiles, wpp, cc.dense,
-                       W, n_full, ksplits, cc.part_o, cc.part_ml, cc.next_wst_h2, cc.next_bias, cc.ptab, (const unsigned*)nullptr, cc.qf_img, cc.qw_wst, cc.qw_bias, PvGuard{});
+                       W, n_full, ksplits, cc.part_o, cc.part_ml, cc.next_wst_h2, cc.next_bias, cc.ptab, (const unsigned*)nullptr, cc.qf_img, cc.qw_wst, cc.qw_bias, PvGuard{}, (const float*)nullptr);
   if (max_tail > 0)
     hipLaunchKernelGGL(k_scattn_merge, dim3(8 * max_tail), dim3(256), 0, s, cc.part_o, cc.part_ml, fus, cc.tail_wst_h2, vecs, out,
                        tiles, wpp, W, n_full, ksplits, cc.next_wst_h2, cc.next_bias, (const float*)nullptr, 0,
diff --git a/gmf_amd/csrc/gmf_api.cpp b/gmf_amd/csrc/gmf_api.cpp
--- a/gmf_amd/csrc/gmf_api.cpp
+++ b/gmf_amd/csrc/gmf_api.cpp
@@ -296,6 +296,11 @@
     t.q_in_attention = value != 0;
     return GMF_OK;
   }
+  if (std::strcmp(name, "kv_fold") == 0) {
+    GMF_REQUIRE(value == 0 || value == 1, GMF_ERR_BAD_ARG, "set_tuning: kv_fold must be 0 or 1");
+    t.kv_fold = value != 0;
+    return GMF_OK;
+  }
   if (std::strcmp(name, "pv_fp8") == 0) {
     GMF_REQUIRE(value >= 0 && value <= 2, GMF_ERR_BAD_ARG, "set_tuning: pv_fp8 must be 0 (three f16 products), 1 (guarded, default) or 2 (always)");
     t.pv_fp8 = value;
@@ -334,7 +339,7 @@
       {"fused_linear", t.fused_linear ? 1 : 0}, {"compat_cache", t.use_cache ? 1 : 0}, {"conv_lds_patch", t.conv_patch}, {"conv_small_grid", t.conv_small ? 1 : 0}, {"small_prologue_roles", t.small_prologue ? 1 : 0}, {"small_fattn_tile", t.small_fattn_tile ? 1 : 0},
       {"nms_binned", t.nms_binned}, {"topk_select", t.topk_select ? 1 : 0}, {"wide_attn_tile", t.wide_attn_tile ? 1 : 0},
       {"small_merge_tile", t.small_merge_tile ? 1 : 0}, {"mid_grid_roles", t.mid_grid_roles}, {"pv_fp8", t.pv_fp8}, {"q_in_attention", t.q_in_attention ? 1 : 0},
-      {"compat_format", t.compat_format}, {"precision", t.precision}, {"spectral_col_splits", t.spectral_col_splits},
+      {"kv_fold", t.kv_fold ? 1 : 0}, {"compat_format", t.compat_format}, {"precision", t.precision}, {"spectral_col_splits", t.spectral_col_splits},
       {"clique_local_rows", t.clique_local_rows}};
   for (const auto& e : tab) {
     if (std::strcmp(name, e.name) == 0) { *value = e.v; return GMF_OK; }
@@ -553,6 +558,7 @@
   int ff_hs = 1, f1_ff_hs = 1;
   bool roles = false;
   bool q_in_attn = false;
+  bool kv_fold = false;
   bool v_fp8 = false;
   bool guard = false;
   bool clear_stats = false;
@@ -588,6 +594,7 @@
   else p.form = (W >= 256 || ragged) ? EncoderPlan::kLinear : EncoderPlan::kFusedStages;
   p.roles = p.form == EncoderPlan::kLinear && t.mid_grid_roles > 0 && W < t.mid_grid_roles;
   p.q_in_attn = p.form == EncoderPlan::kLinear && t.q_in_attention && !p.half && !p.roles;
+  p.kv_fold = t.kv_fold && p.form == EncoderPlan::kLinear && p.pipelined && !p.half && p.fmt == 0 && w->kv_fold != nullptr;
   p.v_fp8 = fused && !p.half && (t.pv_fp8 == 2 || (t.pv_fp8 == 1 && w->pv_guard));
   p.clear_stats = fused && t.pv_fp8 == 1 && w->pv_guard;
   p.guard = p.clear_stats && !p.half;
@@ -614,10 +621,10 @@
 
 static int run_scattn(gmf_handle* h, const gmf_encoder_weights* w, const EncoderPlan& p, int l, const float* q, const float* k,
                       const float* v, const float* pts8, const float* x2, float* out, int B, int N, hipStream_t st,
-                      const float* dense_compat, const gmf::CompatCache& cc) {
+                      const float* dense_compat, const gmf::CompatCache& cc, const float* tail_vecs = nullptr) {
   const int tiles = tiles_of(N);
   const float* wst = w->tail_wst + (size_t)l * w->tail_wst_stride;
-  const float* vecs = w->tail_vec + (size_t)l * w->tail_vec_stride;
+  const float* vecs = tail_vecs ? tail_vecs : w->tail_vec + (size_t)l * w->tail_vec_stride;
   hipEvent_t ev0 = nullptr, ev1 = nullptr;
   if (int rc = prof_begin(h, st, &ev0, &ev1)) return rc;
   if (dense_compat) GMF_HIP(gmf::launch_scattn_dense(q, k, v, dense_compat, x2, wst, vecs, out, B, N, tiles, st));
@@ -779,6 +786,7 @@
       const float* ffv = w->ff_vec + (size_t)l * w->ff_vec_stride;
       const float* ctx_l = ctxall + (size_t)l * tok;
       const bool last = (l + 1 == L);
+      const float* tail_vecs = nullptr;
       cc.tail_wst_h2 = w->tail_wst_h2 + (size_t)l * w->tail_wst_stride;
       cc.next_wst_h2 = last ? nullptr : w->front_wst_h2 + (size_t)(l + 1) * w->front_wst_stride;
       cc.next_bias = last ? nullptr : w->front_vec + (size_t)(l + 1) * w->front_vec_stride;
@@ -786,8 +794,18 @@
         cc.qf_img = p.q_in_attn ? f : nullptr;
         cc.qw_wst = p.q_in_attn ? fw + 4 * kTileFloats : nullptr;
         cc.qw_bias = p.q_in_attn ? fv + kC : nullptr;
+        const float* kvf = p.kv_fold ? w->kv_fold + (size_t)l * GMF_KV_FOLD_STRIDE : nullptr;
+        const float* kvf_vecs = kvf ? kvf + 9 * kTileFloats : nullptr;
+        if (kvf) {
+          cc.qf_img = f;
+          cc.qw_wst = p.q_in_attn ? kvf : nullptr;
+          cc.qw_bias = p.q_in_attn ? kvf_vecs : nullptr;
+          cc.tail_wst_h2 = kvf + 4 * kTileFloats;
+          cc.kvf_vec = kvf_vecs + kC;
+          tail_vecs = kvf_vecs + 3 * kC;
+        }
         GMF_HIP(gmf::launch_linear_h2(p.roles, f, fw, fv, ctx_l, aw, av, ffw, ffv, p.q_in_attn ? nullptr : q, k, v, x2, B, N, tiles, T, tt,
-                                      st, p.one_product, ptab, cc.v_scale, cc.guard));
+                                      st, p.one_product, ptab, cc.v_scale, cc.guard, kvf, kvf_vecs));
       } else if (p.form == EncoderPlan::kSmall3) {
         GMF_HIP(gmf::launch_small_front_fattn(f, fw, fv, ctx_l, aw, av, q, k, v, x1, B, N, tiles, T, tt, st, cc.v_scale, cc.guard,
                                               h->tune.small_fattn_tile, ptab));
@@ -802,7 +820,7 @@
         GMF_HIP(gmf::launch_fusion_attn_h2(true, f, ctx_l, aw, av, x1, B, N, tiles, T, tt, st));
         GMF_HIP(gmf::launch_fusion_ff_h2(x1, ffw, ffv, x2, B, tiles, st, part_o, p.ff_hs));
       }
-      if (int rc = run_scattn(h, w, p, l, q, k, v, pts8, x2, last ? cur : f, B, N, st, nullptr, cc)) return rc;
+      if (int rc = run_scattn(h, w, p, l, q, k, v, pts8, x2, last ? cur : f, B, N, st, nullptr, cc, tail_vecs)) return rc;
     }
     GMF_HIP(gmf::launch_head(cur, w->head_wst, w->head_vec, logits, feat_n, feat, B, N, tiles, st, h->status_dev, ptab,
                              p.guard ? fstat : nullptr, p.guard ? w->pv_guard : nullptr, L));
diff --git a/gmf_amd/csrc/gmf_pack.cpp b/gmf_amd/csrc/gmf_pack.cpp
--- a/gmf_amd/csrc/gmf_pack.cpp
+++ b/gmf_amd/csrc/gmf_pack.cpp
@@ -303,6 +303,59 @@
   append(*vec, vec_of(sd, p + "6.bias", kCw));
 }
 
+void pack_kv_fold(const StateDict& sd, int layer, Ctx& cx, std::vector<float>& out) {
+  const std::string n = "encoder.blocks.NonLocal_layer_" + std::to_string(layer) + ".";
+  const size_t base = out.size();
+  const float cq = (float)(kLog2e / std::sqrt((double)kCw));
+  const Mat Wq = scaled(mat_of(sd, n + "projection_q.weight", kCw, kCw), cq);
+  std::vector<float> bq = vec_of(sd, n + "projection_q.bias", kCw);
+  for (float& x : bq) x = x * cq;
+  const Mat Wk = mat_of(sd, n + "projection_k.weight", kCw, kCw), Wv = mat_of(sd, n + "projection_v.weight", kCw, kCw);
+  const std::vector<float> bk = vec_of(sd, n + "projection_k.bias", kCw), bv = vec_of(sd, n + "projection_v.bias", kCw);
+  Mat Wa = mat_of(sd, n + "fc_message.0.weight", 64, kCw);
+  std::vector<float> ba = vec_of(sd, n + "fc_message.0.bias", 64);
+  fold_bn(Wa, ba, sd, n + "fc_message.1.");
+  Mat Wqf(kCw, kCw), Waf(64, kCw);
+  std::vector<float> bqf(kCw), u(kCw), baf(64);
+  double b0 = 0.0;
+  for (int c = 0; c < kCw; ++c) {
+    for (int j = 0; j < kCw; ++j) {
+      double a = 0.0;
+      for (int m = 0; m < kCw; ++m) a += (double)Wk.at(m, c) * (double)Wq.at(m, j);
+      Wqf.at(c, j) = (float)a;
+    }
+    double a = 0.0, b = 0.0;
+    for (int m = 0; m < kCw; ++m) { a += (double)Wk.at(m, c) * (double)bq[m]; b += (double)bk[m] * (double)Wq.at(m, c); }
+    bqf[c] = (float)a;
+    u[c] = (float)b;
+    b0 += (double)bk[c] * (double)bq[c];
+  }
+  for (int r = 0; r < 64; ++r) {
+    for (int j = 0; j < kCw; ++j) {
+      double a = 0.0;
+      for (int m = 0; m < kCw; ++m) a += (double)Wa.at(r, m) * (double)Wv.at(m, j);
+      Waf.at(r, j) = (float)a;
+    }
+    double a = (double)ba[r];
+    for (int m = 0; m < kCw; ++m) a += (double)Wa.at(r, m) * (double)bv[m];
+    baf[r] = (float)a;
+  }
+  cx.img(out, Wqf, Img::H2S);
+  cx.img(out, Waf, Img::H2S);
+  Ctx copy;
+  std::vector<float> tw, tv;
+  pack_tail(sd, layer, Img::H2S, copy, tw, &tv);
+  if (!copy.ok) cx.ok = false;
+  out.insert(out.end(), tw.begin() + 2 * 4096, tw.end());
+  append(out, bqf);
+  append(out, u);
+  out.push_back((float)b0);
+  append_zeros(out, kCw - 1);
+  append(out, baf);
+  out.insert(out.end(), tv.begin() + 64, tv.end());
+  if (out.size() - base != (size_t)GMF_KV_FOLD_STRIDE) throw PackError{GMF_ERR_BAD_ARG, "gmf: pack: kv_fold block size"};
+}
+
 void pack_head(const StateDict& sd, std::vector<float>& wst, std::vector<float>& vec) {
   p32(wst, mat_of(sd, "classification.0.weight", 32, kCw));
   p32(wst, mat_of(sd, "classification.2.weight", 32, 32));
@@ -413,8 +466,8 @@
     Block blk;
     struct Off { size_t v = 0; bool set = false; };
     auto put = [&](Off& o, const std::vector<float>& v) { o.v = blk.add(v); o.set = true; };
-    Off f1[6], f1h[3], ctx[2], attn[2], ff[2], front[2], tail[2], head[2], ctxh, attnh, ffh, fronth, tailh, pvgo;
-    Ctx c32, ch2;
+    Off f1[6], f1h[3], ctx[2], attn[2], ff[2], front[2], tail[2], head[2], ctxh, attnh, ffh, fronth, tailh, pvgo, kvfo;
+    Ctx c32, ch2, ckv;
     if (has_f1) {
       FusionBlobs b = pack_fusion(sd, "encoder.fusion_layer_1.", false, Img::F32, c32);
       if (b.lat != 128) throw PackError{GMF_ERR_UNSUPPORTED_SHAPE, "gmf: pack: fusion_layer_1 must be 128 wide"};
@@ -423,7 +476,7 @@
       put(f1h[0], bh.ctx_wst); put(f1h[1], bh.attn_wst); put(f1h[2], bh.ff_wst);
     }
     if (L > 0) {
-      std::vector<float> cw, cv, aw, av, fw, fv, cwh, awh, fwh, frw, frv, frwh, tw, tv, twh, pvg;
+      std::vector<float> cw, cv, aw, av, fw, fv, cwh, awh, fwh, frw, frv, frwh, tw, tv, twh, pvg, kvf;
       for (int l = 0; l < L; ++l) {
         const std::string pre = "encoder.blocks.NonLocal_layer_" + std::to_string(l) + ".fusion_layer_2.";
         FusionBlobs b = pack_fusion(sd, pre, true, Img::F32, c32);
@@ -436,10 +489,11 @@
         pack_tail(sd, l, Img::F32, c32, tw, &tv);
         pack_tail(sd, l, Img::H2S, ch2, twh, nullptr);
         pvg.push_back(pv_guard_threshold(sd, l));
+        pack_kv_fold(sd, l, ckv, kvf);
       }
       put(ctx[0], cw); put(ctx[1], cv); put(attn[0], aw); put(attn[1], av); put(ff[0], fw); put(ff[1], fv);
       put(front[0], frw); put(front[1], frv); put(tail[0], tw); put(tail[1], tv);
-      put(ctxh, cwh); put(attnh, awh); put(ffh, fwh); put(fronth, frwh); put(tailh, twh); put(pvgo, pvg);
+      put(ctxh, cwh); put(attnh, awh); put(ffh, fwh); put(fronth, frwh); put(tailh, twh); put(pvgo, pvg); put(kvfo, kvf);
     }
     if (has_head) {
       std::vector<float> hw, hv;
@@ -469,6 +523,7 @@
       w.front_wst_h2 = at(fronth); w.ctx_wst_h2 = at(ctxh); w.attn_wst_h2 = at(attnh); w.ff_wst_h2 = at(ffh);
       w.f1_ctx_wst_h2 = at(f1h[0]); w.f1_attn_wst_h2 = at(f1h[1]); w.f1_ff_wst_h2 = at(f1h[2]);
       w.tail_wst_h2 = at(tailh);
+      if (ckv.ok) w.kv_fold = at(kvfo);
     }
   } catch (const PackError& e) {
     delete p;
@@ -594,7 +649,7 @@
   const float** ptrs[] = {&w.f1_ctx_wst, &w.f1_ctx_vec, &w.f1_attn_wst, &w.f1_attn_vec, &w.f1_ff_wst, &w.f1_ff_vec, &w.ctx_wst, &w.ctx_vec,
                           &w.attn_wst, &w.attn_vec, &w.ff_wst, &w.ff_vec, &w.front_wst, &w.front_vec, &w.tail_wst, &w.tail_vec, &w.head_wst,
                           &w.head_vec, &w.front_wst_h2, &w.ctx_wst_h2, &w.attn_wst_h2, &w.ff_wst_h2, &w.f1_ctx_wst_h2, &w.f1_attn_wst_h2,
-                          &w.f1_ff_wst_h2, &w.tail_wst_h2, &w.pv_guard};
+                          &w.f1_ff_wst_h2, &w.tail_wst_h2, &w.pv_guard, &w.kv_fold};
   for (const float** q : ptrs) rebase_ptr(*q, from, n, to);
   p->placed = to;
   return GMF_OK;
diff --git a/gmf_amd/csrc/launchers.hpp b/gmf_amd/csrc/launchers.hpp
--- a/gmf_amd/csrc/launchers.hpp
+++ b/gmf_amd/csrc/launchers.hpp
@@ -28,6 +28,7 @@
   const float* qw_wst = nullptr;
   const float* qw_bias = nullptr;
   PvGuard guard;
+  const float* kvf_vec = nullptr;
 };
 
 struct Tuning {
@@ -48,6 +49,7 @@
   int nms_binned = 1;
   bool topk_select = true;
   int mid_grid_roles = 512;
+  bool kv_fold = true;
   bool q_in_attention = true;
   int pv_fp8 = 1;
   int compat_format = 0;
@@ -96,7 +98,8 @@
 hipError_t launch_linear_h2(bool roles, const float* f, const float* front_wst, const float* front_vec, const float* ctx_img,
                             const float* attn_wst, const float* attn_vec, const float* ff_wst, const float* ff_vec, float* q,
                             float* k, float* v, float* x2, int B, int N, int tiles, int T, int ttiles, hipStream_t s, bool one_product = false,
-                            const PairTab* ptab = nullptr, unsigned* v_scale = nullptr, PvGuard guard = {});
+                            const PairTab* ptab = nullptr, unsigned* v_scale = nullptr, PvGuard guard = {}, const float* kvf_wst = nullptr,
+                            const float* kvf_bias = nullptr);
 hipError_t launch_small_front_fattn(const float* f, const float* front_wst, const float* front_vec, const float* ctx_img,
                                     const float* attn_wst, const float* attn_vec, float* q, float* k, float* v, float* x1, int B,
                                     int N, int tiles, int T, int ttiles, hipStream_t s, unsigned* v_scale = nullptr, PvGuard guard = {},
diff --git a/include/gmf_hip.h b/include/gmf_hip.h
--- a/include/gmf_hip.h
+++ b/include/gmf_hip.h
@@ -82,7 +82,9 @@
   const float* f1_ctx_wst_h2; const float* f1_attn_wst_h2; const float* f1_ff_wst_h2;
   const float* tail_wst_h2;
   const float* pv_guard;
+  const float* kv_fold;
 } gmf_encoder_weights;
+#define GMF_KV_FOLD_STRIDE 37504
 
 typedef struct gmf_tensor {
   const char* name;
```
